# killerwhile/kafka-assignment-optimizer

Hardware: AMD Instinct MI355X
Metric: candidate assignments/sec (+ time_to_optimal_s), 10k-partition reassign (higher is better)
Workload: dtype int32

## Files before the change

include/kao.h:

```cpp
#ifndef KAO_H
#define KAO_H

#include <stdint.h>

#ifdef __cplusplus
extern "C" {
#endif

#define KAO_VERSION 103
#define KAO_NONE 0xFFFFu
#define KAO_MAX_RF 8
#define KAO_MAX_RACKS 255

enum {
    KAO_OK = 0,
    KAO_ERR_INVALID = -1,
    KAO_ERR_UNSUPPORTED = -2,
    KAO_ERR_NO_DEVICE = -3,
    KAO_ERR_HIP = -4,
    KAO_ERR_NOMEM = -5,
    KAO_ERR_NOT_INIT = -6
};

enum {
    KAO_STATUS_OPTIMAL_PROVEN = 0,
    KAO_STATUS_FEASIBLE_BOUND_GAP = 1,
    KAO_STATUS_NO_FEASIBLE = 2,
    KAO_STATUS_TIME_LIMIT = 3,
    KAO_STATUS_INFEASIBLE_PROVEN = 4
};

typedef struct kao_topic {
    int32_t n_brokers;
    int32_t n_racks;
    int32_t n_partitions;
    int32_t rf;
    int32_t rf_cur;
    const uint8_t *rack_of;
    const uint16_t *current;
    int32_t w[2][2];
    int32_t rep_lo, rep_hi;
    int32_t lead_lo, lead_hi;
    int32_t rack_lo, rack_hi;
    int32_t prack_lo, prack_hi;
    const int32_t *broker_w;
    const int32_t *broker_wl;
} kao_topic;

typedef struct kao_opts {
    uint64_t seed;
    double time_limit_s;
    int32_t restarts;
    int32_t iters_per_launch;
    int32_t max_launches;
    int32_t obj_scale;
    int32_t lam_min, lam_max;
    int32_t period_log2;
    int32_t stop_at_bound;
    int32_t profile;
    int32_t dual_iters;
    int32_t elite_period;
    int32_t use_prices;
    int32_t use_cycles;
    int32_t islands;
    int32_t schedule;
    int32_t team;
    const int64_t *target_objective;
} kao_opts;

typedef struct kao_result {
    int32_t status;
    int32_t best_restart;
    int64_t objective;
    int64_t upper_bound;
    int32_t violations[8];
    double seconds_to_best;
    uint16_t *assignment;
} kao_result;

typedef struct kao_stats {
    uint64_t launches;
    uint64_t delta_candidates;
    uint64_t full_candidates;
    double ms_search;
    double ms_eval;
    uint64_t search_bytes_algo;
    uint64_t eval_bytes_algo;
    int32_t n_restarts_total;
    int32_t lds_bytes_search;
    int32_t blocks_search;
    int32_t drift;
    int32_t launch_groups;
    int32_t search_rf3_launches;
} kao_stats;

typedef struct kao_session kao_session;
typedef struct kao_eval_plan kao_eval_plan;

int kao_init(int device);
void kao_shutdown(void);
int kao_version(void);
const char *kao_strerror(int code);
const char *kao_last_error(void);
int kao_device_name(char *buf, int len);

int kao_derive_bounds(const kao_topic *t, int32_t out[8]);
int kao_upper_bound(const kao_topic *t, int64_t *ub);
int kao_check_infeasible(const kao_topic *t, char *why, int why_len);
int kao_canonicalize(const kao_topic *t, uint16_t *assignment);

int kao_evaluate(const kao_topic *t, const uint16_t *assignment, int64_t *objective, int32_t violations[8]);
int kao_evaluate_batch(const kao_topic *t, const uint16_t *candidates, int64_t n, int32_t *objective,
                       int32_t *violations);
int kao_eval_plan_create(const kao_topic *t, kao_eval_plan **out);
int kao_eval_plan_run(kao_eval_plan *p, const void *d_candidates, int64_t n, void *d_objective ,
                      void *d_violations , void *d_best_key );
int kao_eval_plan_sync(kao_eval_plan *p, double *ms_last );
void kao_eval_plan_destroy(kao_eval_plan *p);

int kao_session_create(const kao_topic *topics, int32_t n_topics, const kao_opts *opts, kao_session **out);
int kao_session_step(kao_session *s);
int kao_session_sync(kao_session *s);
int kao_session_new_generation(kao_session *s);
int kao_session_best(kao_session *s, kao_result *results);
int kao_session_best_keys(kao_session *s, uint64_t *keys);
int kao_session_device_keys(kao_session *s, void **d_keys);
int kao_session_stats(kao_session *s, kao_stats *out);
int kao_session_bound_step(kao_session *s, const int64_t *target, int32_t iters);
int kao_session_set_prices(kao_session *s, int32_t topic, const int32_t *a, const int32_t *l, const int32_t *g);
int kao_session_adopt_prices(kao_session *s);
int kao_session_prices(kao_session *s, int32_t topic, int32_t *a, int32_t *l, int32_t *g);
int kao_session_bound_busy(kao_session *s);
int kao_session_bounds(kao_session *s, int64_t *upper_bound, int32_t *flags, int32_t *iters);
int kao_session_dual_state(kao_session *s, int32_t topic, int32_t *a, int32_t *l, int32_t *g, int64_t *best_dual);
int kao_session_set_dual_state(kao_session *s, int32_t topic, const int32_t *a, const int32_t *l, const int32_t *g);
int kao_lp_bound(const kao_topic *t, double tol, int32_t max_iters, int64_t *bound, int64_t *best_dual, int32_t *multipliers, double stats[8]);
int kao_lp_trace(const kao_topic *t, double tol, int32_t max_iters, double *trace, double stats[8], int32_t *multipliers);
int kao_lp_round(const kao_topic *t, double pert, uint32_t salt, double tol, int32_t max_iters, int32_t use_fallback, uint16_t *assignment,
                 int64_t *objective, int32_t violations[8], double stats[8]);
int kao_lp_round_host(const kao_topic *t, const uint8_t *q, const int32_t *zq, int32_t use_fallback, uint16_t *assignment, int32_t rep[4]);
int kao_dense_spd_test(const double *A, int32_t n, const double *rhs, double *factor, double *linv, double *x, double ms[2]);
int kao_lp_sharded_test(const kao_topic *t, const int32_t *devices, int32_t n_dev, double pert, uint32_t salt, double tol, int32_t max_iters,
                        int64_t *bound, uint16_t *assignment, int64_t *objective, int32_t violations[8], double stats[8]);
int kao_dual_bound(const kao_topic *t, int64_t target, int32_t iters, int32_t launches, int64_t *bound,
                   int64_t *best_dual, int32_t *iters_done, int32_t *flags, int32_t *multipliers);
int kao_session_restart_state(kao_session *s, int32_t topic, int32_t restart, uint16_t *final_state,
                              uint16_t *best_state, int32_t info[4]);
void kao_session_destroy(kao_session *s);

int kao_solve(const kao_topic *topics, int32_t n_topics, const kao_opts *opts, kao_result *results);
int kao_solve_multi(const kao_topic *topics, int32_t n_topics, const int32_t *devices, int32_t n_dev, const kao_opts *opts,
                    kao_result *results);
int kao_solve_capped(const kao_topic *topics, int32_t n_topics, const int32_t *replica_cap, const int32_t *devices, int32_t n_dev,
                     const kao_opts *opts, int32_t max_rounds, kao_result *results, int64_t *lagrangian_bound);
int kao_improve_cycles(const kao_topic *t, uint16_t *assignment, int32_t max_rounds, int64_t *objective, int32_t stats[8]);
int kao_cycle_matrices(const kao_topic *t, const uint16_t *assignment, int32_t layer, int32_t level, int32_t *dist, int32_t *mid,
                       uint32_t *slot);
int kao_cycle_seeds(const kao_topic *t, const uint16_t *assignment, int32_t *table, int32_t *n_cfg);
int kao_cycle_pair_edges(const kao_topic *t, const uint16_t *assignment, int32_t gmin, int32_t *cost, int64_t stats[4]);

int kao_plan_waves(int32_t n_brokers, int32_t n_partitions, int32_t width, const uint16_t *current, const uint16_t *target,
                   int32_t max_per_broker, uint64_t seed, int32_t *wave , int32_t *n_waves, int32_t *lower_bound);

int kao_plan_waves_sized(int32_t n_brokers, int32_t n_partitions, int32_t width, const uint16_t *current, const uint16_t *target,
                         const uint64_t *size , uint64_t max_bytes_per_broker, int32_t max_per_broker,
                         uint64_t seed, int32_t *wave , int32_t *n_waves, int32_t *lower_bound);

int kao_balance_leaders(const kao_topic *t, uint16_t *assignment , int32_t *n_changed,
                        int64_t *objective ,
                        int32_t *status, int32_t stats[8] );

#define KAO_FAILOVER_MAX_BROKERS 8000
int kao_failover_order(int32_t n_brokers, int32_t n_racks, const uint8_t *rack_of ,
                       int32_t n_partitions, int32_t width, uint16_t *rows ,
                       int32_t scope , int32_t dry_run,
                       int32_t *scen , int32_t *n_reordered, int32_t stats[8] );

int kao_rccl_selftest(const int32_t *devices, int32_t n_dev);
int kao_rccl_loopback_counts(uint64_t out[2]);
int kao_last_solve_timing(double out[16]);
int kao_last_solve_lp(double out[8]);
int kao_last_solve_profile(double out[8]);

#ifdef __cplusplus
}
#endif
#endif
```

kafka_assignment_optimizer_amd/_ffi.py:

```python
from __future__ import annotations

import ctypes as C
import os

_HERE = os.path.dirname(os.path.abspath(__file__))
LIB_PATH = os.path.join(_HERE, "libkao.so")


class KaoTopic(C.Structure):
    _fields_ = [("n_brokers", C.c_int32), ("n_racks", C.c_int32), ("n_partitions", C.c_int32),
                ("rf", C.c_int32), ("rf_cur", C.c_int32),
                ("rack_of", C.POINTER(C.c_uint8)), ("current", C.POINTER(C.c_uint16)),
                ("w", (C.c_int32 * 2) * 2),
                ("rep_lo", C.c_int32), ("rep_hi", C.c_int32), ("lead_lo", C.c_int32), ("lead_hi", C.c_int32),
                ("rack_lo", C.c_int32), ("rack_hi", C.c_int32), ("prack_lo", C.c_int32), ("prack_hi", C.c_int32),
                ("broker_w", C.POINTER(C.c_int32)), ("broker_wl", C.POINTER(C.c_int32))]


class KaoOpts(C.Structure):
    _fields_ = [("seed", C.c_uint64), ("time_limit_s", C.c_double), ("restarts", C.c_int32),
                ("iters_per_launch", C.c_int32), ("max_launches", C.c_int32), ("obj_scale", C.c_int32),
                ("lam_min", C.c_int32), ("lam_max", C.c_int32), ("period_log2", C.c_int32),
                ("stop_at_bound", C.c_int32), ("profile", C.c_int32), ("dual_iters", C.c_int32),
                ("elite_period", C.c_int32), ("use_prices", C.c_int32), ("use_cycles", C.c_int32), ("islands", C.c_int32),
                ("schedule", C.c_int32), ("team", C.c_int32),
                ("target_objective", C.POINTER(C.c_int64))]


class KaoResult(C.Structure):
    _fields_ = [("status", C.c_int32), ("best_restart", C.c_int32), ("objective", C.c_int64),
                ("upper_bound", C.c_int64), ("violations", C.c_int32 * 8), ("seconds_to_best", C.c_double),
                ("assignment", C.POINTER(C.c_uint16))]


class KaoStats(C.Structure):
    _fields_ = [("launches", C.c_uint64), ("delta_candidates", C.c_uint64), ("full_candidates", C.c_uint64),
                ("ms_search", C.c_double), ("ms_eval", C.c_double), ("search_bytes_algo", C.c_uint64),
                ("eval_bytes_algo", C.c_uint64), ("n_restarts_total", C.c_int32), ("lds_bytes_search", C.c_int32),
                ("blocks_search", C.c_int32), ("drift", C.c_int32), ("launch_groups", C.c_int32),
                ("search_rf3_launches", C.c_int32)]


_P = C.POINTER
SIGNATURES = {
    "kao_init": (C.c_int, [C.c_int]),
    "kao_shutdown": (None, []),
    "kao_version": (C.c_int, []),
    "kao_strerror": (C.c_char_p, [C.c_int]),
    "kao_last_error": (C.c_char_p, []),
    "kao_device_name": (C.c_int, [C.c_char_p, C.c_int]),
    "kao_derive_bounds": (C.c_int, [_P(KaoTopic), _P(C.c_int32)]),
    "kao_upper_bound": (C.c_int, [_P(KaoTopic), _P(C.c_int64)]),
    "kao_canonicalize": (C.c_int, [_P(KaoTopic), _P(C.c_uint16)]),
    "kao_check_infeasible": (C.c_int, [_P(KaoTopic), C.c_char_p, C.c_int]),
    "kao_evaluate": (C.c_int, [_P(KaoTopic), _P(C.c_uint16), _P(C.c_int64), _P(C.c_int32)]),
    "kao_evaluate_batch": (C.c_int, [_P(KaoTopic), _P(C.c_uint16), C.c_int64, _P(C.c_int32), _P(C.c_int32)]),
    "kao_eval_plan_create": (C.c_int, [_P(KaoTopic), _P(C.c_void_p)]),
    "kao_eval_plan_run": (C.c_int, [C.c_void_p, C.c_void_p, C.c_int64, C.c_void_p, C.c_void_p, C.c_void_p]),
    "kao_eval_plan_sync": (C.c_int, [C.c_void_p, _P(C.c_double)]),
    "kao_eval_plan_destroy": (None, [C.c_void_p]),
    "kao_session_create": (C.c_int, [_P(KaoTopic), C.c_int32, _P(KaoOpts), _P(C.c_void_p)]),
    "kao_session_step": (C.c_int, [C.c_void_p]),
    "kao_session_sync": (C.c_int, [C.c_void_p]),
    "kao_session_new_generation": (C.c_int, [C.c_void_p]),
    "kao_session_best": (C.c_int, [C.c_void_p, _P(KaoResult)]),
    "kao_session_best_keys": (C.c_int, [C.c_void_p, _P(C.c_uint64)]),
    "kao_session_device_keys": (C.c_int, [C.c_void_p, _P(C.c_void_p)]),
    "kao_session_stats": (C.c_int, [C.c_void_p, _P(KaoStats)]),
    "kao_session_restart_state": (C.c_int, [C.c_void_p, C.c_int32, C.c_int32, _P(C.c_uint16), _P(C.c_uint16),
                                            _P(C.c_int32)]),
    "kao_session_bound_step": (C.c_int, [C.c_void_p, _P(C.c_int64), C.c_int32]),
    "kao_session_set_prices": (C.c_int, [C.c_void_p, C.c_int32, _P(C.c_int32), _P(C.c_int32), _P(C.c_int32)]),
    "kao_session_adopt_prices": (C.c_int, [C.c_void_p]),
    "kao_session_prices": (C.c_int, [C.c_void_p, C.c_int32, _P(C.c_int32), _P(C.c_int32), _P(C.c_int32)]),
    "kao_session_bound_busy": (C.c_int, [C.c_void_p]),
    "kao_session_bounds": (C.c_int, [C.c_void_p, _P(C.c_int64), _P(C.c_int32), _P(C.c_int32)]),
    "kao_session_dual_state": (C.c_int, [C.c_void_p, C.c_int32, _P(C.c_int32), _P(C.c_int32), _P(C.c_int32), _P(C.c_int64)]),
    "kao_session_set_dual_state": (C.c_int, [C.c_void_p, C.c_int32, _P(C.c_int32), _P(C.c_int32), _P(C.c_int32)]),
    "kao_lp_bound": (C.c_int, [_P(KaoTopic), C.c_double, C.c_int32, _P(C.c_int64), _P(C.c_int64), _P(C.c_int32), _P(C.c_double)]),
    "kao_lp_round": (C.c_int, [_P(KaoTopic), C.c_double, C.c_uint32, C.c_double, C.c_int32, C.c_int32, _P(C.c_uint16), _P(C.c_int64), _P(C.c_int32), _P(C.c_double)]),
    "kao_lp_round_host": (C.c_int, [_P(KaoTopic), _P(C.c_uint8), _P(C.c_int32), C.c_int32, _P(C.c_uint16), _P(C.c_int32)]),
    "kao_dense_spd_test": (C.c_int, [_P(C.c_double), C.c_int32, _P(C.c_double), _P(C.c_double), _P(C.c_double), _P(C.c_double), _P(C.c_double)]),
    "kao_lp_sharded_test": (C.c_int, [_P(KaoTopic), _P(C.c_int32), C.c_int32, C.c_double, C.c_uint32, C.c_double, C.c_int32, _P(C.c_int64), _P(C.c_uint16),
                                      _P(C.c_int64), _P(C.c_int32), _P(C.c_double)]),
    "kao_lp_trace": (C.c_int, [_P(KaoTopic), C.c_double, C.c_int32, _P(C.c_double), _P(C.c_double), _P(C.c_int32)]),
    "kao_dual_bound": (C.c_int, [_P(KaoTopic), C.c_int64, C.c_int32, C.c_int32, _P(C.c_int64), _P(C.c_int64), _P(C.c_int32),
                                 _P(C.c_int32), _P(C.c_int32)]),
    "kao_session_destroy": (None, [C.c_void_p]),
    "kao_solve": (C.c_int, [_P(KaoTopic), C.c_int32, _P(KaoOpts), _P(KaoResult)]),
    "kao_solve_multi": (C.c_int, [_P(KaoTopic), C.c_int32, _P(C.c_int32), C.c_int32, _P(KaoOpts), _P(KaoResult)]),
    "kao_solve_capped": (C.c_int, [_P(KaoTopic), C.c_int32, _P(C.c_int32), _P(C.c_int32), C.c_int32, _P(KaoOpts), C.c_int32,
                                  _P(KaoResult), _P(C.c_int64)]),
    "kao_rccl_selftest": (C.c_int, [_P(C.c_int32), C.c_int32]),
    "kao_rccl_loopback_counts": (C.c_int, [_P(C.c_uint64)]),
    "kao_improve_cycles": (C.c_int, [_P(KaoTopic), _P(C.c_uint16), C.c_int32, _P(C.c_int64), _P(C.c_int32)]),
    "kao_cycle_matrices": (C.c_int, [_P(KaoTopic), _P(C.c_uint16), C.c_int32, C.c_int32, _P(C.c_int32), _P(C.c_int32), _P(C.c_uint32)]),
    "kao_cycle_seeds": (C.c_int, [_P(KaoTopic), _P(C.c_uint16), _P(C.c_int32), _P(C.c_int32)]),
    "kao_cycle_pair_edges": (C.c_int, [_P(KaoTopic), _P(C.c_uint16), C.c_int32, _P(C.c_int32), _P(C.c_int64)]),
    "kao_plan_waves": (C.c_int, [C.c_int32, C.c_int32, C.c_int32, _P(C.c_uint16), _P(C.c_uint16), C.c_int32, C.c_uint64,
                                 _P(C.c_int32), _P(C.c_int32), _P(C.c_int32)]),
    "kao_plan_waves_sized": (C.c_int, [C.c_int32, C.c_int32, C.c_int32, _P(C.c_uint16), _P(C.c_uint16), _P(C.c_uint64), C.c_uint64,
                                       C.c_int32, C.c_uint64, _P(C.c_int32), _P(C.c_int32), _P(C.c_int32)]),
    "kao_balance_leaders": (C.c_int, [_P(KaoTopic), _P(C.c_uint16), _P(C.c_int32), _P(C.c_int64), _P(C.c_int32), _P(C.c_int32)]),
    "kao_failover_order": (C.c_int, [C.c_int32, C.c_int32, _P(C.c_uint8), C.c_int32, C.c_int32, _P(C.c_uint16), C.c_int32, C.c_int32,
                                     _P(C.c_int32), _P(C.c_int32), _P(C.c_int32)]),
    "kao_last_solve_timing": (C.c_int, [_P(C.c_double)]),
    "kao_last_solve_profile": (C.c_int, [_P(C.c_double)]),
    "kao_last_solve_lp": (C.c_int, [_P(C.c_double)]),
}

_lib = None


def load():
    global _lib
    if _lib is None:
        if not os.path.exists(LIB_PATH):
            raise OSError(f"{LIB_PATH} not built: the HIP library is required (no CPU fallback); "
                          "run `make -C kafka_assignment_optimizer_amd/csrc`")
        lib = C.CDLL(LIB_PATH)
        for name, (res, args) in SIGNATURES.items():
            fn = getattr(lib, name)
            fn.restype = res
            fn.argtypes = args
        _lib = lib
    return _lib
```

kafka_assignment_optimizer_amd/csrc/kao_host.h:

```cpp
#pragma once
#include <hip/hip_runtime.h>

#include <algorithm>
#include <cstdint>
#include <cstdlib>
#include <memory>
#include <string>
#include <vector>

#include "../../include/kao.h"
#include "kao_internal.h"

namespace kao {

int fail(int code, const std::string &msg);
#define HIP_TRY(expr)                                                                          \
    do {                                                                                       \
        hipError_t e_ = (expr);                                                                \
        if (e_ != hipSuccess)                                                                  \
            return ::kao::fail(KAO_ERR_HIP, std::string(#expr) + ": " + hipGetErrorString(e_)); \
    } while (0)
double now_s();
int cur_device();
constexpr int kMaxDevices = 64;
int num_cu(int device);
int require_init();
bool is_init();
extern thread_local int t_device;
struct DeviceScope {
    const int saved = t_device;
    int rc = KAO_OK;
    DeviceScope() = default;
    explicit DeviceScope(int device) { to(device); }
    DeviceScope(const DeviceScope &) = delete;
    DeviceScope &operator=(const DeviceScope &) = delete;
    int to(int device);
    ~DeviceScope();
};
struct SolveTiming {
    double session_ready, time_to_best, results_read_back, returned, launches, delta_candidates, bound_launches, elite_exchanges,
           bound_iters, cx_calls, cx_gains, search_iters, generations, cx_further_starts, lp_solves, lp_iters;
};
struct SolveLp { double solves, iterations, rounded, adopted, fractional_partitions; };
struct SolveProfile {
    double ms_search, ms_eval, search_launches, restarts, search_bytes_algo, delta_candidates, lds_bytes_search, blocks_search;
};
struct SolveCounters { SolveTiming timing; SolveLp lp; SolveProfile profile; };
extern thread_local SolveCounters g_last;
inline const char *env_str(const char *name) { const char *e = std::getenv(name); return e && *e ? e : nullptr; }
inline int64_t env_int(const char *name, int64_t dflt) { const char *e = env_str(name); return e ? (int64_t)std::atoll(e) : dflt; }
inline double env_real(const char *name, double dflt) { const char *e = env_str(name); return e ? std::atof(e) : dflt; }
int arena_get(size_t bytes, void **out, size_t *cap);
void arena_put(void *p, size_t bytes, int device);
int stream_get(hipStream_t *out);
void stream_put(hipStream_t st, int device);
void arena_drop_all();
inline size_t align_up(size_t x, size_t a = 256) { return (x + a - 1) / a * a; }
inline uint32_t replica_word(uint16_t x, int m) { return x == KAO_NONE ? kNoneW : ((uint32_t)x | ((uint32_t)(x / m) << 16)); }

int validate(const kao_topic *t);
void derive_bounds(const kao_topic *t, int32_t o[8]);
struct PreparedTopic {
    TopicDev d{};
    std::vector<uint16_t> int_of;
    std::vector<uint16_t> ext_of;
    std::vector<int32_t> rack_size;
    std::vector<uint16_t> cur_int;
    std::vector<uint8_t> rack_of;
    std::vector<uint16_t> cur_dense;
    std::vector<uint32_t> bw_int, bw_dense;
};
int prepare(const kao_topic *t, uint64_t seed, PreparedTopic &pt);
std::string infeasible_reason(const kao_topic *t);
int64_t upper_bound(const kao_topic *t);
int64_t upper_bound_w(const kao_topic *t);
uint64_t neighbours_in_range(uint32_t it0, uint32_t iters, int rf, int n_brokers, int n_partitions, int scan2_max = kScanTwoSlots);
int auto_period_log2(int P, int RF);
bool dual_supported(const kao_topic *t, bool session_bw = false);

}

using namespace kao;

struct kao_eval_plan {
    PreparedTopic pt;
    TopicDev *d_topic = nullptr;
    uint8_t *d_rackof = nullptr;
    uint16_t *d_curd = nullptr;
    int4 *d_map = nullptr;
    uint32_t *d_bwd = nullptr;
    int32_t *d_overflow = nullptr;
    int64_t map_n = -1;
    int map_blocks = 0;
    hipStream_t stream = nullptr;
    hipEvent_t ev0 = nullptr, ev1 = nullptr;
    bool timed = false;
    int cands_per_block = 32;
    bool cur_in_lds = true;
    bool coop = false;
    int device = 0;
};

struct kao_session {
    int device = 0;
    int n_topics = 0;
    kao_opts opts{};
    std::vector<PreparedTopic> pts;
    std::vector<kao_topic> topics;
    std::vector<int64_t> ub;
    std::vector<char> topic_global;
    std::vector<char> topic_curg;
    std::vector<char> topic_infeasible;
    std::vector<char> dual_ok;
    std::vector<int64_t> h_dual_target;
    std::vector<int32_t> h_dual_ids;
    bool multi_off = false;
    std::vector<int2> h_wide_map;
    uint64_t wide_ctl_i32 = 0, wide_map_i32 = 0;
    std::vector<int32_t> dual_flags, dual_iters;
    int total_restarts = 0;
    struct LaunchGroup {
        int maxP = 0, maxBx = 0, maxB = 0, maxR = 0;
        bool wide = false;
        int waves = kWaves;
        int nw = kRFP;
        int rf_uniform = -1;
        bool rf3 = true;
        bool global_a = false;
        bool cur_global = false;
        int team = 0;
        bool cur_in_lds = true;
        bool eval_coop = false;
        int smap_off = 0, smap_n = 0, emap_off = 0, emap_n = 0;
    };
    std::vector<LaunchGroup> groups;
    int blocks_search = 0, blocks_eval = 0;
    void *arena_ro = nullptr, *arena_rw = nullptr;
    size_t arena_ro_bytes = 0, arena_rw_bytes = 0;
    TopicDev *d_topics = nullptr;
    int2 *d_smap = nullptr;
    int4 *d_emap = nullptr;
    uint32_t *d_cur = nullptr;
    uint16_t *d_ext = nullptr;
    int32_t *d_rsz = nullptr;
    uint8_t *d_rackof = nullptr;
    uint16_t *d_curd = nullptr;
    unsigned char *d_state = nullptr;
    uint16_t *d_best = nullptr;
    int32_t *d_info = nullptr;
    int32_t *d_obj = nullptr;
    int32_t *d_viol = nullptr;
    unsigned char *d_readback = nullptr;
    size_t readback_bytes = 0, rb_viol_off = 0, rb_assign_off = 0;
    int32_t *d_dual = nullptr;
    int32_t *d_price = nullptr;
    size_t price_half_i32 = 0;
    int price_read = 0;
    int price_write_last = -1;
    bool priced = false;
    bool any_bw = false;
    uint16_t *d_int = nullptr;
    uint32_t *d_bw = nullptr, *d_bwd = nullptr;
    long long *d_dual_target = nullptr;
    int32_t *d_dual_ids = nullptr;
    unsigned char *d_dual_rb = nullptr;
    size_t dual_rb_bytes = 0;
    uint64_t bound_launches = 0;
    bool dual_state_init = false;
    size_t dual_bytes = 0;
    hipStream_t stream_bound = nullptr;
    hipEvent_t ev_bound0 = nullptr, ev_bound1 = nullptr, ev_search = nullptr;
    bool bound_inflight = false;
    bool bound_no_wait = false;
    int bound_iters_last = 0;
    double bound_ms_last = 0;
    unsigned long long *d_keys = nullptr;
    unsigned long long *d_keys_glob = nullptr;
    int32_t *d_drift = nullptr;
    int32_t *d_win_viol = nullptr;
    uint16_t *d_win_assign = nullptr;
    std::vector<unsigned char> h_readback;
    hipStream_t stream = nullptr;
    uint32_t launch = 0;
    uint32_t gen = 0;
    bool reinit = false;
    size_t best_bytes = 0;
    std::vector<hipEvent_t> ev;
    int ev_pending = 0;
    double ms_search = 0, ms_eval = 0;
    uint64_t eval_bytes_per_launch = 0;
    uint64_t delta_total = 0, search_bytes_total = 0;
    uint64_t search_rf3_launches = 0;
};

namespace kao {
constexpr int64_t kDualNone = 0x7F7F7F7F7F7F7F7Fll;
inline int64_t dual_floor(int64_t best_dual) { return best_dual >= 0 ? best_dual / kDualScale : -((-best_dual + kDualScale - 1) / kDualScale); }
inline int64_t dual_bound_value(int32_t flags, int32_t iters, int64_t best_dual) { return (flags & 4) || iters == 0 ? INT64_MAX : dual_floor(best_dual); }
struct SessionDeleter { void operator()(kao_session *s) const { kao_session_destroy(s); } };
using SessionPtr = std::unique_ptr<kao_session, SessionDeleter>;
int bound_only_session(const kao_topic *t, SessionPtr &out);
int session_topic_best(kao_session *s, int i, uint16_t *out);
int session_restart_objs(kao_session *s, int i, std::vector<int32_t> &objs);
int session_restart_best(kao_session *s, int i, int restart, uint16_t *out);
int session_adopt_external(kao_session *s, int i, const uint16_t *assign, int64_t objective, uint64_t *key_out);
}
```

kafka_assignment_optimizer_amd/csrc/kao_internal.h:

```cpp
#pragma once
#include <stdint.h>

#include <unordered_map>

#include "../../include/kao.h"

namespace kao {

constexpr int kRFP = 4;
constexpr int kMaxRF = 8;
constexpr int kWaves = 4;
constexpr int kTeamMax = 8;
constexpr int kMaxRacks = 255;
constexpr int kLdsLimit = 160 * 1024;
constexpr int kRackTab = 256;
constexpr uint32_t kNoneW = 0xFFFFFFFFu;
constexpr uint32_t kKeyNull = 0xFFFFFFFFu;
constexpr int kDBias = 32768;
constexpr int kDualLog2 = 16;
constexpr int kDualScale = 1 << kDualLog2;
constexpr int kDualStage = 100;
constexpr int kDualDeflP = 2048;
constexpr int kScanTwoSlots = 24576;
constexpr int kDualClamp = 1 << 26;
constexpr int kDualQuarterLog2 = kDualLog2 - 2;
constexpr int kDualProbes = 2;
constexpr uint32_t kExternalRestart = 0xFFFFFu;
constexpr uint32_t kObjCap = 0xFFFFFFu;

struct TopicDev {
    int32_t P, RF, R, m, Bx;
    uint32_t magic;
    int32_t rep_lo, rep_hi, lead_lo, lead_hi, rack_lo, rack_hi, prack_lo, prack_hi;
    int32_t w00, w01, w10, w11;
    uint32_t seed_lo, seed_hi;
    int32_t n_restarts;
    int32_t restart_base;
    uint32_t cur_off;
    uint32_t ext_off;
    uint32_t rsz_off;
    uint64_t state_off;
    uint64_t best_off;
    int32_t B, rf_cur;
    uint32_t rackof_off;
    uint32_t curd_off;
    uint32_t win_off;
    uint32_t dual_off;
    int32_t period_log2;
    uint32_t price_off;
    uint32_t int_off;
    int32_t nw;
    int32_t has_bw;
    uint32_t bw_off;
    uint32_t bwd_off;
    uint32_t cnt_off;
    uint32_t hole_off;
    int32_t pad_[1];
};

struct SearchParams {
    int32_t obj_scale, lam_min, lam_max;
    int32_t maxR;
    int32_t wide;
    uint32_t launch;
    uint32_t iters;
    int32_t init;
    int32_t maxP, maxBx;
    int32_t bw;
    uint32_t gen;
    int32_t scan2_max;
    int32_t cur_global;
    int32_t elite;
};

struct SearchPools {
    const TopicDev *topics;
    const int2 *block_map;
    const uint32_t *cur_pool;
    const uint16_t *ext_pool;
    const int32_t *rsz_pool;
    unsigned char *state_pool;
    uint16_t *best_pool;
    int32_t *restart_info;
    int32_t *drift;
    const int32_t *price_pool;
    const uint32_t *bw_pool;
    const uint16_t *int_pool;
    const uint16_t *elite_assign;
    const unsigned long long *elite_key;
};

struct EvalPools {
    const TopicDev *topics;
    const int4 *block_map;
    const uint8_t *rackof_pool;
    const uint16_t *curd_pool;
    const uint16_t *cand;
    int32_t *objective;
    int32_t *violations;
    unsigned long long *best_key;
    int32_t maxP, maxB;
    int32_t cur_in_lds;
    int32_t coop;
    const uint32_t *bwd_pool;
    int32_t *overflow;
    int32_t rf_uniform;
};

struct BoundPools {
    const TopicDev *topics;
    const int32_t *ids;
    const uint8_t *rackof_pool;
    const uint16_t *curd_pool;
    const uint16_t *ext_pool;
    const int32_t *rsz_pool;
    int32_t *dual_pool;
    const long long *target;
    long long *best_L;
    int32_t *info;
    int32_t iters;
    int32_t maxB, maxP, maxR;
    int32_t cur_in_lds;
    int32_t *price_pool;
    int32_t export_prices;
    int32_t ne;
    const uint32_t *bwd_pool;
};

struct BoundWide {
    const int2 *map;
    int32_t *cnt_pool;
    long long *ctl;
    int32_t chunk;
};

constexpr int search_rack_tab(int maxR) { return ((maxR < 1 ? 1 : maxR) + 1 + 63) & ~63; }
size_t search_lds_bytes(int maxP, int maxBx, int waves, bool global_a, bool priced = false, int nw = 4, bool bw = false, int maxR = kRackTab - 1, int team = 0, bool cur_global = false);
size_t eval_lds_bytes(int maxP, int maxB, bool cur_in_lds, int ne = 4);
bool search_rf3_eligible(bool global_a, bool cur_global, bool priced, int nw, int team);
void launch_search(const SearchPools &pools, const SearchParams &prm, int n_blocks, int waves, bool global_a, bool priced, int nw, void *stream, int team = 0, int rft = 0);
bool launch_init(const SearchPools &pools, const SearchParams &prm, int n_blocks, int per_block, bool priced, int nw, int waves, void *stream);
void launch_eval(const EvalPools &pools, int n_blocks, int ne, void *stream);
void launch_gather(const TopicDev *topics, int n_topics, const unsigned long long *keys, const uint16_t *best_pool,
                   const int32_t *viol, uint16_t *win_assign, int32_t *win_viol, void *stream);

void launch_adopt_global(unsigned long long *keys, const unsigned long long *glob, int n, void *stream);

size_t bound_lds_bytes(int maxB, int maxP, int maxR, bool cur_in_lds, int ne = 4, bool hbw = false, bool dirs = false);
void launch_bound_center(const BoundPools &pools, int n_topics, void *stream);
void launch_bound(const BoundPools &pools, int n_blocks, int waves, void *stream);
void launch_bound_wide(const BoundPools &pools, const BoundWide &wide, int n_topics, int n_blocks, int waves, void *stream);
bool launch_bound_multi(const BoundPools &pools, const BoundWide &wide, int n_topics, int n_blocks, int waves, void *stream);

size_t canon_lds_bytes(int maxBx);
void launch_canon(const TopicDev *topic, const uint32_t *cur_words, const uint16_t *ext, const int32_t *rsz, uint32_t *A, int maxBx,
                  int nw, int32_t *status, void *stream);


struct LpCtx;
struct LpColl {
    virtual int allreduce(int rank, double *buf, size_t n, bool is_min, void *stream) = 0;
    virtual ~LpColl() {}
};
struct LpShard { int p0, p1, rank; LpColl *coll; };
struct LpFan {
    virtual int begin(double tol, int maxit, double pert, uint32_t salt) = 0;
    virtual int enqueue_mark(int k, int slot) = 0;
    virtual int poll_mark(int slot, int *status, int *iterations, double deadline) = 0;
    virtual int finish(int32_t *multipliers, double stats[8], double *trace) = 0;
    virtual int primal(uint8_t *q, int32_t *zq) = 0;
    virtual void abort() = 0;
    virtual void close() = 0;
    virtual ~LpFan() {}
};
extern thread_local bool t_lp_inner;
void lp_set_fan(LpCtx *c, LpFan *fan);
int lp_open_fan(const kao_topic *t, const int *devices, int n_dev, LpCtx **out);
int lp_open(const kao_topic *t, LpCtx **out, const LpShard *shard = nullptr);
int lp_solve(LpCtx *c, double tol, int maxit, int32_t *multipliers, double stats[8], double *trace, double pert = 0.0, uint32_t salt = 0);
int lp_begin(LpCtx *c, double tol, int maxit, double pert = 0.0, uint32_t salt = 0);
int lp_enqueue(LpCtx *c, int k);
int lp_poll(LpCtx *c, int *status, int *iterations);
int lp_enqueue_mark(LpCtx *c, int k, int slot);
int lp_poll_mark(LpCtx *c, int slot, int *status, int *iterations, double deadline = 0);
int lp_finish(LpCtx *c, int32_t *multipliers, double stats[8], double *trace);
inline double lp_default_pert(const kao_topic *t) { const double e = 100.0 / ((double)t->n_partitions * t->rf); return e < 1e-2 ? e : 1e-2; }
int lp_primal(LpCtx *c, uint8_t *q, int32_t *zq);
int lp_round_assignment(const kao_topic *t, const uint8_t *q, const int32_t *zq, const uint16_t *fallback, uint16_t *out, int32_t rep[4], int max_free = 1 << 30);
void lp_abort(LpCtx *c);
void lp_close(LpCtx *c);
void chol_enqueue(void *stream, const double *stop, double *S, int n, const double *diag0, double *Linv);
void trsv_enqueue(void *stream, double *stop, const double *gate, const double *S, int n, double *r, const double *Linv, double *xz);

bool cycle_supported(const kao_topic *t);
int cycle_improve(const kao_topic *t, uint16_t *assign, int32_t max_rounds, double deadline, int64_t *objective, int32_t stats[8]);
struct CycleCtx;
CycleCtx *cycle_open(const kao_topic *t, int *rc_out);
int cycle_run(CycleCtx *c, uint16_t *assign, int32_t max_rounds, double deadline, int64_t *objective, int32_t stats[8],
              int (*poll)(void *) = nullptr, void *poll_arg = nullptr, bool pairs = true);
void cycle_close(CycleCtx *c);
struct PairEdge { int32_t cost; int32_t set; int32_t p, q; uint16_t rowp[8], rowq[8]; };
int pair_edges(const kao_topic *t, const uint16_t *assignment, int gmin, std::unordered_map<uint32_t, PairEdge> &edges, int64_t stats[4]);
int api_fail(int code, const char *msg);
int api_require_init();
double api_now_s();

}
```

kafka_assignment_optimizer_amd/csrc/kao_search.hip:

```cpp
#include "kao_search_dev.h"

namespace kao {

template <bool kGlobalA, bool kPriced, int NW, bool kWide, bool kTeam, bool kCurG = false, int RFT = 0>
__device__ __forceinline__ void search_body(unsigned char *smem, const SearchPools &pl, const SearchParams &prm) {
    static_assert(!kTeam || kGlobalA, "teams run topics that live in global memory");
    static_assert(!kCurG || !kGlobalA, "kCurG: the working assignment is in LDS");
    static_assert(RFT == 0 || (RFT == 3 && NW == 4 && !kGlobalA && !kTeam), "RFT = 3: LDS-resident topics of four words per partition");
    constexpr int NS = RFT ? RFT : NW;
    const int lane = threadIdx.x & 63;
    const int wave = __builtin_amdgcn_readfirstlane(threadIdx.x >> 6);
    const int n_waves = kTeam ? __builtin_amdgcn_readfirstlane((int)(blockDim.x >> 6)) : 1;
    const int tid = kTeam ? (int)threadIdx.x : lane, nthr = kTeam ? (int)blockDim.x : 64;
    const int2 bm = pl.block_map[blockIdx.x];
    const TopicDev *TD = pl.topics + bm.x;

    TopicRegs T = topic_regs<RFT>(TD);
    asm volatile("" : "+v"(T.rep_lo), "+v"(T.rep_hi), "+v"(T.lead_lo), "+v"(T.lead_hi));

    const int a_bytes = kGlobalA ? 0 : prm.maxP * NW * 4;
    const int cur_bytes = (kGlobalA || kCurG) ? 0 : prm.maxP * NW * 4;
    const int bx64 = (prm.maxBx + 63) & ~63;
    const int c_bytes = bx64 * 4;
    const int krt = search_rack_tab(prm.maxR);
    int *RSZ = reinterpret_cast<int *>(smem + cur_bytes);
    uint8_t *XR = smem + cur_bytes + krt * 4;
    const uint32_t inv = (uint32_t)krt - 1u;
    uint32_t *PR = reinterpret_cast<uint32_t *>(smem + cur_bytes + krt * 4 + bx64);
    const bool hbw = kPriced && prm.bw != 0;
    const int pr_bytes = kPriced ? (hbw ? 2 : 1) * c_bytes + krt * 4 : 0;
    int *PG = reinterpret_cast<int *>(smem + cur_bytes + krt * 4 + bx64 + c_bytes);
    uint32_t *BW = reinterpret_cast<uint32_t *>(smem + cur_bytes + krt * 4 + bx64 + c_bytes + krt * 4);
    unsigned char *wb = smem + cur_bytes + krt * 4 + bx64 + pr_bytes + (kTeam ? 0 : wave * (a_bytes + c_bytes + c_bytes / 2 + krt * 8));
    const Part<NW> *cur_words = reinterpret_cast<const Part<NW> *>(pl.cur_pool + TD->cur_off);
    const Part<NW> *CUR;
    if (kGlobalA || kCurG) CUR = cur_words; else CUR = reinterpret_cast<const Part<NW> *>(smem);
    WaveLds<NW> L;
    L.C = reinterpret_cast<uint32_t *>(wb + a_bytes);
    L.W = reinterpret_cast<uint16_t *>(wb + a_bytes + c_bytes);
    L.K = reinterpret_cast<int *>(wb + a_bytes + c_bytes + c_bytes / 2);
    L.RT = L.K + krt + (kTeam ? wave * krt : 0);
    int *TR = L.K + krt + n_waves * krt;
    int *TS = TR + 2 * 16 * kTeamRec;

    if (!kGlobalA && !kCurG) {
        Part<NW> *cur_lds = reinterpret_cast<Part<NW> *>(smem);
        for (int p = threadIdx.x; p < T.P; p += blockDim.x) cur_lds[p] = cur_words[p];
    }
    for (int r = threadIdx.x; r < krt; r += blockDim.x) {
        RSZ[r] = r < T.R ? pl.rsz_pool[TD->rsz_off + r] : 0;
        if (kPriced) PG[r] = r < T.R ? price_units(pl.price_pool[TD->price_off + 2 * TD->B + r], prm.obj_scale) : 0;
    }
    __syncthreads();
    for (int x = threadIdx.x; x < ((T.Bx + 63) & ~63); x += blockDim.x) {
        const uint32_t r = mulhi((uint32_t)x, T.magic);
        const bool valid = x < T.Bx && (int)((uint32_t)x - r * (uint32_t)T.m) < RSZ[r < (uint32_t)krt ? r : 0];
        XR[x] = valid ? (uint8_t)r : (uint8_t)inv;
        if (kPriced) {
            uint32_t pr = 0;
            if (valid) {
                const int32_t *pp = pl.price_pool + TD->price_off;
                const int b = pl.ext_pool[TD->ext_off + x];
                pr = ((uint32_t)price_units(pp[b], prm.obj_scale) & 0xFFFFu) | ((uint32_t)price_units(pp[TD->B + b], prm.obj_scale) << 16);
            }
            PR[x] = pr;
            if (hbw) BW[x] = (valid && TD->has_bw) ? pl.bw_pool[TD->bw_off + x] : 0u;
        }
    }
    __syncthreads();

    const int rho = bm.y + (kTeam ? 0 : wave);
    if (rho >= TD->n_restarts) return;
    const int g = TD->restart_base + rho;
    unsigned char *state_packed = pl.state_pool + TD->state_off + (uint64_t)rho * T.P * (NW * 2);
    if (kGlobalA) L.A = reinterpret_cast<Part<NW> *>(pl.state_pool + TD->state_off) + (uint64_t)rho * T.P;
    else L.A = reinterpret_cast<Part<NW> *>(wb);
    uint16_t *best = pl.best_pool + TD->best_off + (uint64_t)rho * T.P * T.RF;
    const uint16_t *ext = pl.ext_pool + TD->ext_off;
    const uint32_t slo = TD->seed_lo, shi = TD->seed_hi;
    const int S = prm.obj_scale;

    int best_obj, accepted;
    if (prm.init) {
        if (prm.init == 1)
        for (int p = tid; p < T.P; p += nthr) {
            Part<NW> c = CUR[p];
#pragma unroll
            for (int k = 1; k < NW; ++k)
                if (k >= T.RF) c.w[k] = kNoneW;
            L.A[p] = c;
        }
        best_obj = -1; accepted = 0;
    } else {
        best_obj = pl.restart_info[g * 4 + 0];
        accepted = pl.restart_info[g * 4 + 3];
        bool reseed = false;
        if (prm.elite) {
            const unsigned long long ek = pl.elite_key[bm.x];
            const int e_obj = (int)kObjCap - (int)((ek >> 20) & 0xFFFFFFull);
            reseed = ek != ~0ull && (ek >> 44) == 0 && (int)(ek & 0xFFFFFull) != rho && best_obj < e_obj &&
                     (fmix32(slo ^ ((uint32_t)rho * 0x9E3779B1u) ^ (prm.launch * 0x85EBCA77u) ^ 0xE117Eu) & 1u);
        }
        if (reseed) {
            const uint16_t *ea = pl.elite_assign + TD->win_off;
            const uint16_t *io = pl.int_pool + TD->int_off;
            for (int p = tid; p < T.P; p += nthr) {
                Part<NW> w;
#pragma unroll
                for (int k = 0; k < NW; ++k) w.w[k] = k < T.RF ? to_word(T, io[ea[p * T.RF + k]]) : kNoneW;
                L.A[p] = w;
            }
        } else if (!kGlobalA) {
            for (int p = lane; p < T.P; p += 64) L.A[p] = load_packed<NW>(T, state_packed, p);
        }
    }
    if (kGlobalA) __builtin_amdgcn_fence(__ATOMIC_SEQ_CST, "workgroup");
    if (kTeam) __syncthreads();
    recount(T, L, tid, nthr, krt);
    if (kTeam) __syncthreads();

    if (prm.init == 1) {
        const uint32_t *HL = pl.cur_pool + TD->hole_off;
        if (!kTeam || wave == 0)
        for (int pass = 0; pass < 2; ++pass) {
            const uint32_t n_holes = HL[pass], *hl = HL + 2 + (pass ? HL[0] : 0u);
            int p_n = n_holes ? (int)hl[0] : 0;
            Part<NW> a_n = L.A[p_n], c_n = CUR[p_n];
            for (uint32_t hi = 0; hi < n_holes; ++hi) {
                const int p = p_n;
                Part<NW> a = a_n;
                const Part<NW> c = c_n;
                if (hi + 1 < n_holes) { p_n = (int)hl[hi + 1]; a_n = L.A[p_n]; c_n = CUR[p_n]; }
#pragma unroll
                for (int k = 0; k < NW; ++k) {
                    if (k >= T.RF) break;
                    if ((k == 0) != (pass == 0)) continue;
                    if (a.w[k] != kNoneW) continue;
                    const uint32_t hmix = slo ^ fmix32(shi + (uint32_t)rho * 0x9E3779B1u + (uint32_t)(p * NW + k) * 0x27D4EB2Fu + 0x5BD1E995u + prm.gen * 0x632BE5ABu);
                    const int wl = k == 0 ? T.w00 : T.w01, wf = k == 0 ? T.w10 : T.w11;
                    uint32_t key = kKeyNull, xw_l = kNoneW;
#pragma unroll 2
                    for (int base = 0; base < T.Bx; base += 64) {
                        const uint32_t x = (uint32_t)(base + lane);
                        const uint32_t r = XR[x];
                        const uint32_t xw = x | (r << 16);
                        const bool okx = (r != inv) & !in4(a, xw);
                        const uint32_t cn = L.C[x];
                        const uint32_t rk = r;
                        int dV = dinc((int)(cn & 0xFFFFu), T.rep_lo, T.rep_hi) + dinc(L.K[rk], T.rack_lo, T.rack_hi) +
                                 dinc(cnt4(a, r), T.prack_lo, T.prack_hi);
                        if (k == 0) dV += dinc((int)(cn >> 16), T.lead_lo, T.lead_hi);
                        const uint32_t tie = fmix32(hmix + x * 0x165667B1u) >> 24;
                        uint32_t keyx;
                        if (kPriced) {
                            const uint32_t prx = PR[x];
                            int dP = p_in((int)(cn & 0xFFFFu), T.rep_lo, T.rep_hi, price_rep(prx)) + p_in(L.K[rk], T.rack_lo, T.rack_hi, PG[rk]);
                            if (k == 0) dP += p_in((int)(cn >> 16), T.lead_lo, T.lead_hi, price_lead(prx));
                            keyx = okx ? make_key_tie_p(prm.lam_max, S, dV, role_w2(c, xw, wl, wf) + (hbw ? bw_of(BW[x], k == 0) : 0), dP, tie) : kKeyNull;
                        }
                        else keyx = okx ? make_key_tie(prm.lam_max, S, dV, role_w2(c, xw, wl, wf), tie) : kKeyNull;
                        if (keyx < key) { key = keyx; xw_l = xw; }
                    }
                    const uint32_t kmin = wave_umin(key);
                    const unsigned long long bal = __ballot(key == kmin);
                    const uint32_t xw_win = (uint32_t)__builtin_amdgcn_readlane((int)xw_l, __ffsll((long long)bal) - 1);
                    a.w[k] = xw_win;
                    if (lane == 0) {
                        reinterpret_cast<uint32_t *>(&L.A[p])[k] = xw_win;
                        L.C[xw_win & 0xFFFFu] += (k == 0) ? 0x10001u : 1u;
                        L.K[xw_win >> 16] += 1;
                    }
                }
            }
        }
        if (kGlobalA) __builtin_amdgcn_fence(__ATOMIC_SEQ_CST, "workgroup");
        if (kTeam) __syncthreads();
    }

    int V, obj;
    full_cost<NW, kTeam>(T, L, CUR, RSZ, tid, nthr, V, obj, hbw ? BW : nullptr, TS, wave, n_waves);
    if (V == 0 && obj > best_obj) { best_obj = obj; snapshot(T, L, ext, best, tid, nthr); }
    rebuild_band_state(T, L, XR, inv, tid, nthr);
    if (lane == 0) L.RT[krt - 1] = 0;
    if (kTeam) __syncthreads();

    uint32_t rng = fmix32(slo ^ fmix32(shi + (uint32_t)rho * 0x9E3779B1u + prm.launch * 0x85EBCA77u + (uint32_t)tid * 0xC2B2AE3Du));

    const int plog = TD->period_log2 + (rho & 3);
    const uint32_t pmask = (1u << plog) - 1u;
    const uint32_t lrange = (uint32_t)(prm.lam_max - prm.lam_min + 1);
    const uint32_t RF8 = (uint32_t)T.RF << 8, R8 = (uint32_t)T.R << 8, m8 = (uint32_t)T.m << 8;

    const int T_tour = min(64, max(4, (T.P * T.RF) >> 2));
    uint32_t tour_off = lane < T_tour ? 0u : kKeyNull;
    asm volatile("" : "+v"(tour_off));
    const int GA = min(16, max(1, (T.P * T.RF) >> 8));
    const int x_rounds_full = (T.P + 63) >> 6;
    const bool x_windowed = x_rounds_full > 8;

    int lam_lo = prm.lam_min, lam_hi = prm.lam_max;
    uint32_t n_iters = prm.iters, it_base = prm.launch * prm.iters;
    uint32_t scan_two = TD->P * TD->RF <= prm.scan2_max ? 1u : 0u;
    {
        uint32_t v0 = (uint32_t)lam_lo, v1 = (uint32_t)lam_hi, v2 = n_iters, v3 = it_base, v4 = scan_two;
        asm volatile("" : "+v"(v0), "+v"(v1), "+v"(v2), "+v"(v3), "+v"(v4));
        lam_lo = (int)__builtin_amdgcn_readfirstlane(v0); lam_hi = (int)__builtin_amdgcn_readfirstlane(v1);
        n_iters = __builtin_amdgcn_readfirstlane(v2); it_base = __builtin_amdgcn_readfirstlane(v3);
        scan_two = __builtin_amdgcn_readfirstlane(v4);
    }
    constexpr bool kFuse = !kGlobalA && !kTeam && !kPriced;
    const bool fuse_ok = kFuse && T.Bx <= 16384;
    uint32_t jmp_a = 1u, jmp_c = 0u;
    if (fuse_ok)
        for (int n = (T.Bx + 63) >> 6; n > 0; --n) { jmp_a = (jmp_a * 0x6D2B79u) & 0xFFFFFFu; jmp_c = (jmp_c * 0x6D2B79u + 0x3C6EF3u) & 0xFFFFFFu; }
    for (uint32_t i = 0; i < n_iters; ++i) {
        const uint32_t it = it_base + i;
        const int type = (int)((0x1210u >> ((it & 7u) * 2u)) & 3u);
        const uint32_t ph = it & pmask;
        const int lam = best_obj < 0 ? lam_hi : min(lam_hi, lam_lo + (int)((2u * ph * lrange) >> plog));
        const bool sampled = (type == 2) || (type == 0 && ((it >> 3) & 1u));

        auto finish = [&](auto ty, auto uni, uint32_t kmin, int win, int p, int k, int q, int j, uint32_t uw, uint32_t vw, int dV, int dObj) {
            constexpr int TY = decltype(ty)::value;
            auto of_win = [&](int v) { return decltype(uni)::value ? v : __builtin_amdgcn_readlane(v, win); };
            if (!kTeam) {
                if (kmin == kKeyNull) return;
                if ((int)(kmin >> 8) - kDBias > 0) return;
            }
            bool mine = true;
            int *rec = TR + ((i & 1u) * 16 + (uint32_t)wave) * kTeamRec;
            if (kTeam) {
                const bool ok = kmin != kKeyNull && (int)(kmin >> 8) - kDBias <= 0;
                if (lane == win) {
                    const uint32_t ro_ = uw >> 16, rn_ = vw >> 16;
                    const bool racks = ok && TY == 0 && ro_ != rn_;
                    rec[0] = ok ? 1 : 0; rec[1] = p; rec[2] = TY == 1 ? q : p;
                    rec[3] = (int)(uw & 0xFFFFu); rec[4] = (int)(vw & 0xFFFFu);
                    rec[5] = racks ? (int)ro_ : 0xFFFF; rec[6] = racks ? (int)rn_ : 0xFFFF;
                    rec[7] = dV; rec[8] = dObj;
                }
                __syncthreads();
                bool clash = false;
                if (lane < wave) {
                    const int *o = TR + ((i & 1u) * 16 + (uint32_t)lane) * kTeamRec;
                    if (o[0]) {
                        const int mp = rec[1], mq = rec[2], mb0 = rec[3], mb1 = rec[4], mr0 = rec[5], mr1 = rec[6];
                        clash = (o[1] == mp) | (o[1] == mq) | (o[2] == mp) | (o[2] == mq) | (o[3] == mb0) | (o[3] == mb1) | (o[4] == mb0) | (o[4] == mb1);
                        if (o[5] != 0xFFFF && mr0 != 0xFFFF) clash |= (o[5] == mr0) | (o[5] == mr1) | (o[6] == mr0) | (o[6] == mr1);
                    }
                }
                mine = ok && __ballot(clash) == 0ull;
            }

            if (lane == win && mine) {
                uint32_t *ap = reinterpret_cast<uint32_t *>(&L.A[p]);
                if (TY == 0) {
                    const uint32_t d = (k == 0) ? 0x10001u : 1u;
                    L.C[uw & 0xFFFFu] -= d;
                    L.C[vw & 0xFFFFu] += d;
                    if (!kTeam || (uw >> 16) != (vw >> 16)) {
                        L.K[uw >> 16] -= 1;
                        L.K[vw >> 16] += 1;
                    }
                    ap[k] = vw;
                } else if (TY == 1) {
                    uint32_t *bp = reinterpret_cast<uint32_t *>(&L.A[q]);
                    if ((k == 0) != (j == 0)) {
                        const uint32_t lose = (k == 0) ? uw : vw, gain = (k == 0) ? vw : uw;
                        L.C[lose & 0xFFFFu] -= 0x10000u;
                        L.C[gain & 0xFFFFu] += 0x10000u;
                    }
                    ap[k] = vw;
                    bp[j] = uw;
                } else {
                    L.C[uw & 0xFFFFu] -= 0x10000u;
                    L.C[vw & 0xFFFFu] += 0x10000u;
                    ap[0] = vw;
                    ap[k] = uw;
                }
            }
            if (mine) {
                int rows;
                if (TY == 0) rows = 1 | (of_win(k) == 0 ? 2 : 0);
                else if (TY == 1) rows = (of_win(k) == 0 ? 2 : 0) ^ (of_win(j) == 0 ? 2 : 0);
                else rows = 2;
                if (rows != 0) {
                    const uint32_t xo = (uint32_t)of_win((int)uw) & 0xFFFFu, xn = decltype(uni)::value ? (uint32_t)__builtin_amdgcn_readfirstlane((int)(vw & 0xFFFFu)) : (uint32_t)of_win((int)vw) & 0xFFFFu;
                    uint32_t xx = xo;
                    asm("v_writelane_b32 %0, %1, 1" : "+v"(xx) : "s"(xn));
                    int lane_w = lane;
                    asm volatile("" : "+v"(lane_w));
                    if (lane_w < 2) {
                        const uint32_t cx = L.C[xx];
                        uint32_t wx;
                        if (rows == 3) wx = band_fields(T, cx);
                        else if (rows == 1) wx = (L.W[xx] & ~kWRowR) | band_entry((int)(cx & 0xFFFFu), T.rep_lo, T.rep_hi);
                        else wx = (L.W[xx] & ~kWRowL) | (band_entry((int)(cx >> 16), T.lead_lo, T.lead_hi) << 6);
                        L.W[xx] = (uint16_t)wx;
                    }
                }
            }
            if (kGlobalA) __builtin_amdgcn_fence(__ATOMIC_SEQ_CST, "workgroup");
            if (kTeam) {
                if (lane == 0) rec[9] = mine ? 1 : 0;
                __syncthreads();
                int dVs = 0, dOs = 0, na = 0;
                if (lane < n_waves) {
                    const int *o = TR + ((i & 1u) * 16 + (uint32_t)lane) * kTeamRec;
                    if (o[9]) { dVs = o[7]; dOs = o[8]; na = 1; }
                }
                V += wave_sum(dVs);
                obj += wave_sum(dOs);
                accepted += wave_sum(na);
            } else {
                V += of_win(dV);
                obj += of_win(dObj);
                accepted++;
            }
        };
        constexpr std::integral_constant<int, 0> kReplace{};
        constexpr std::integral_constant<int, 1> kExchange{};
        constexpr std::integral_constant<int, 2> kLeaderSwap{};

        if (sampled) {
            const int p = (int)rnd24_wide(rng, (uint32_t)T.P);
            const Part<NW> a = L.A[p];
            const Part<NW> c = CUR[p];
            uint32_t key = kKeyNull, vw = 0;
            int dV = 0, dObj = 0;
            if (type == 0) {
                const int k = (int)rnd24(rng, RF8);
                const uint32_t uw = sel_slot<NS>(a, k);
                const uint32_t ro = uw >> 16;
                const bool lead = k == 0;
                const uint32_t lw = lead ? 2u : 0u;
                const int wl = lead ? T.w00 : T.w01, wf = lead ? T.w10 : T.w11;
                const int g_old = role_w2<NS>(c, uw, wl, wf) + (hbw ? bw_of(BW[uw & 0xFFFFu], lead) : 0);
                const uint32_t wo = L.W[uw & 0xFFFFu];
                const int dV_old = wfld(wo, kWDecR) + wfldw(wo, kWDecL, lw);
                const int dV_rack_old = ddec(L.K[ro], T.rack_lo, T.rack_hi) + ddec(cnt4<NS>(a, ro), T.prack_lo, T.prack_hi);
                const int rsz_ro = RSZ[ro];
                int dP_old = 0, dP_rack_old = 0;
                if (kPriced) {
                    const uint32_t pro = PR[uw & 0xFFFFu];
                    dP_old = -(wflag(wo, kWPoutR) & price_rep(pro));
                    if (lead) dP_old -= wflag(wo, kWPoutL) & price_lead(pro);
                    dP_rack_old = p_out(L.K[ro], T.rack_lo, T.rack_hi, PG[ro]);
                }
#pragma unroll
                for (int g = 0; g < 4; ++g) {
                    uint32_t r, jj;
                    bool okg;
                    if (g < 2) {
                        r = rnd24(rng, R8);
                        jj = rnd24(rng, m8);
                        okg = (int)jj < RSZ[r];
                    } else {
                        r = ro;
                        jj = rnd24(rng, (uint32_t)rsz_ro << 8);
                        okg = true;
                    }
                    const uint32_t x = __umul24(r, (uint32_t)T.m) + jj;
                    const uint32_t xw = x | (r << 16);
                    okg = okg && !in4<NS>(a, xw);
                    const uint32_t wn = L.W[x];
                    int dVg = dV_old + wfld(wn, kWIncR) + wfldw(wn, kWIncL, lw);
                    if (g < 2) {
                        if (r != ro)
                            dVg += dV_rack_old + dinc(L.K[r], T.rack_lo, T.rack_hi) + dinc(cnt4<NS>(a, r), T.prack_lo, T.prack_hi);
                    }
                    const int dObjg = role_w2<NS>(c, xw, wl, wf) + (hbw ? bw_of(BW[x], lead) : 0) - g_old;
                    uint32_t keyg;
                    if (kPriced) {
                        const uint32_t prx = PR[x];
                        int dPg = dP_old + (wflag(wn, kWPinR) & price_rep(prx));
                        if (lead) dPg += wflag(wn, kWPinL) & price_lead(prx);
                        if (g < 2 && r != ro) dPg += dP_rack_old + p_in(L.K[r], T.rack_lo, T.rack_hi, PG[r]);
                        keyg = okg ? make_key_p(lam, S, dVg, dObjg, dPg, lane) : kKeyNull;
                    }
                    else keyg = okg ? make_key(lam, S, dVg, dObjg, lane) : kKeyNull;
                    if (keyg < key) { key = keyg; vw = xw; dV = dVg; dObj = dObjg; }
                }
                const uint32_t kmin = wave_umin(key);
                finish(kReplace, std::false_type{}, kmin, (int)(kmin & 63u), p, k, 0, 0, uw, vw, dV, dObj);
            } else {
                const uint32_t uw = a.w[0];
                int k = 0;
                const int u_lead = role_w2<NS>(c, uw, T.w00, T.w10), u_fol = role_w2<NS>(c, uw, T.w01, T.w11);
                const uint32_t wu = L.W[uw & 0xFFFFu];
                const int dV_u = wfld(wu, kWDecL);
                const int dP_u = kPriced ? -(wflag(wu, kWPoutL) & price_lead(PR[uw & 0xFFFFu])) : 0;
#pragma unroll
                for (int kk = 1; kk < NS; ++kk) {
                    if (!RFT && kk >= T.RF) break;
                    const uint32_t xw = a.w[kk];
                    const int dObjg = role_w2<NS>(c, xw, T.w00, T.w10) + u_fol - u_lead - role_w2<NS>(c, xw, T.w01, T.w11) +
                                      (hbw ? (int)(BW[xw & 0xFFFFu] >> 16) - (int)(BW[uw & 0xFFFFu] >> 16) : 0);
                    const uint32_t wx = L.W[xw & 0xFFFFu];
                    const int dVg = dV_u + wfld(wx, kWIncL);
                    uint32_t keyg;
                    if (kPriced) keyg = make_key_p(lam, S, dVg, dObjg, dP_u + (wflag(wx, kWPinL) & price_lead(PR[xw & 0xFFFFu])), lane);
                    else keyg = make_key(lam, S, dVg, dObjg, lane);
                    if (keyg < key) { key = keyg; vw = xw; k = kk; dV = dVg; dObj = dObjg; }
                }
                const uint32_t kmin = wave_umin(key);
                finish(kLeaderSwap, std::false_type{}, kmin, (int)(kmin & 63u), p, k, 0, 0, uw, vw, dV, dObj);
            }
        } else {
            uint32_t keyA, oldw_l;
            int pl_, kl_, g_old_l, dvo_l = 0, dvr_l = 0;
            auto score_words = [&](auto ty, uint32_t &key_o, const Part<NW> &al, const Part<NW> &cl, int k_o, uint32_t &oldw_o, int &g_o, int &dvo_o, int &dvr_o) {
                constexpr int TY = decltype(ty)::value;
                oldw_o = sel_slot<NS>(al, k_o);
                const uint32_t rol = oldw_o >> 16;
                const bool leadl = k_o == 0;
                g_o = role_w2<NS>(cl, oldw_o, leadl ? T.w00 : T.w01, leadl ? T.w10 : T.w11);
                if (hbw && TY == 0) g_o += bw_of(BW[oldw_o & 0xFFFFu], leadl);
                const uint32_t wo = L.W[oldw_o & 0xFFFFu];
                const int dv7 = ddec(cnt4<NS>(al, rol), T.prack_lo, T.prack_hi);
                int sc;
                if (TY == 0) {
                    dvo_o = wfld(wo, kWDecR) + wfldw(wo, kWDecL, leadl ? 2u : 0u);
                    dvr_o = ddec(L.K[rol], T.rack_lo, T.rack_hi) + dv7;
                    sc = dvo_o + min(dvr_o, 0);
                } else {
                    const int dvl = wfld(wo, leadl ? kWDecL : kWIncL);
                    sc = min(dv7, 0) + min(dvl, 0);
                }
                if (kPriced) {
                    int dPs = 0;
                    if (TY == 0) {
                        const uint32_t pro = PR[oldw_o & 0xFFFFu];
                        dPs = -(wflag(wo, kWPoutR) & price_rep(pro));
                        dPs -= wflagw(wo, kWPoutL, leadl ? 1u : 0u) & price_lead(pro);
                    }
                    key_o = make_key_p(lam, S, sc, -g_o, dPs, lane) | tour_off;
                }
                else key_o = make_key(lam, S, sc, -g_o, lane) | tour_off;
            };
            auto score_slot = [&](auto ty, uint32_t &key_o, int p_o, int &k_o, uint32_t &oldw_o, int &g_o, int &dvo_o, int &dvr_o) {
                k_o = (int)rnd24(rng, RF8);
                const Part<NW> al = L.A[p_o];
                const Part<NW> cl = CUR[p_o];
                score_words(ty, key_o, al, cl, k_o, oldw_o, g_o, dvo_o, dvr_o);
            };
            auto tournament = [&](auto ty) {
                const int p0 = (int)rnd24_wide(rng, (uint32_t)T.P);
                auto part = [&](int ga) { const int q2 = p0 + ga; return q2 < T.P ? q2 : q2 - T.P; };
                pl_ = p0;
                score_slot(ty, keyA, p0, kl_, oldw_l, g_old_l, dvo_l, dvr_l);
                int ga = 1;
                for (; kWide && ga + 1 < GA; ga += 2) {
                    uint32_t kg0, ow0, kg1, ow1;
                    int kk0, gg0, d10 = 0, d20 = 0, kk1, gg1, d11 = 0, d21 = 0;
                    const int pg0 = part(ga), pg1 = part(ga + 1);
                    score_slot(ty, kg0, pg0, kk0, ow0, gg0, d10, d20);
                    score_slot(ty, kg1, pg1, kk1, ow1, gg1, d11, d21);
                    if (kg0 < keyA) { keyA = kg0; pl_ = pg0; kl_ = kk0; oldw_l = ow0; g_old_l = gg0; dvo_l = d10; dvr_l = d20; }
                    if (kg1 < keyA) { keyA = kg1; pl_ = pg1; kl_ = kk1; oldw_l = ow1; g_old_l = gg1; dvo_l = d11; dvr_l = d21; }
                }
                for (; ga < GA; ++ga) {
                    uint32_t kg, ow;
                    int kk, gg, d1 = 0, d2 = 0;
                    const int pg = part(ga);
                    score_slot(ty, kg, pg, kk, ow, gg, d1, d2);
                    if (kg < keyA) { keyA = kg; pl_ = pg; kl_ = kk; oldw_l = ow; g_old_l = gg; dvo_l = d1; dvr_l = d2; }
                }
            };
            Part<NW> a_l, c_l;
            constexpr int XB = !kGlobalA ? 1 : ((NW == 4 && !kTeam) ? 8 : 4);
            Part<NW> xb[XB], xcb[XB];
            int q0 = 0;
            auto x_partner = [&](int rd, int &qq, bool &okq) {
                qq = q0 + rd * 64 + lane; okq = true;
                if (qq >= T.P) { if (x_windowed) qq -= T.P; else okq = false; }
                return min(qq, T.P - 1);
            };
            auto tournament_global = [&](auto ty) {
                constexpr int TY = decltype(ty)::value;
                constexpr int TB = (NW == 4 && !kTeam) ? 16 : 8;
                const int p0 = (int)rnd24_wide(rng, (uint32_t)T.P);
                auto part = [&](int ga) { const int q2 = p0 + ga; return q2 < T.P ? q2 : q2 - T.P; };
                int kk[16];
#pragma unroll
                for (int g = 0; g < 16; ++g) { kk[g] = 0; if (g < GA) kk[g] = (int)rnd24(rng, RF8); }
                if (TY == 1) {
                    const int q_draw = (int)rnd24_wide(rng, (uint32_t)T.P);
                    q0 = x_windowed ? __builtin_amdgcn_readfirstlane(q_draw) : 0;
#pragma unroll
                    for (int r2 = 0; r2 < XB; ++r2) { int qq; bool okq; const int qc = x_partner(r2, qq, okq); xb[r2] = L.A[qc]; xcb[r2] = CUR[qc]; }
                }
#pragma unroll
                for (int g0 = 0; g0 < 16; g0 += TB) {
                    if (g0 > 0 && g0 >= GA) break;
                    Part<NW> tal[TB], tcl[TB];
                    int tp[TB];
#pragma unroll
                    for (int g = 0; g < TB; ++g) { tp[g] = (g0 + g) < GA ? part(g0 + g) : p0; tal[g] = L.A[tp[g]]; tcl[g] = CUR[tp[g]]; }
#pragma unroll
                    for (int g = 0; g < TB; ++g) {
                        uint32_t kg, ow;
                        int gg, d1 = 0, d2 = 0;
                        score_words(ty, kg, tal[g], tcl[g], kk[g0 + g], ow, gg, d1, d2);
                        if (g0 + g > 0) kg |= (g0 + g) < GA ? 0u : kKeyNull;
                        if (g0 + g == 0 || kg < keyA) { keyA = kg; pl_ = tp[g]; kl_ = kk[g0 + g]; oldw_l = ow; g_old_l = gg; dvo_l = d1; dvr_l = d2; a_l = tal[g]; c_l = tcl[g]; }
                    }
                }
            };
            if constexpr (kGlobalA) { if (type == 0) tournament_global(std::integral_constant<int, 0>{}); else tournament_global(std::integral_constant<int, 1>{}); }
            else if (type == 0) tournament(std::integral_constant<int, 0>{}); else tournament(std::integral_constant<int, 1>{});
            const int wA1 = (int)(wave_umin(keyA) & 63u);
            int wA2 = -1;
            if (type == 0 && scan_two) {
                const uint32_t k2 = wave_umin(lane == wA1 ? kKeyNull : keyA);
                wA2 = k2 == kKeyNull ? -1 : (int)(k2 & 63u);
            }
            if (kFuse && type == 0 && wA2 >= 0 && fuse_ok) {
                int ps[2], ks[2], gs[2], dvos[2];
                uint32_t us[2];
                int v_rk[2];
#pragma unroll
                for (int s2 = 0; s2 < 2; ++s2) {
                    const int wA = s2 == 0 ? wA1 : wA2;
                    ps[s2] = __builtin_amdgcn_readlane(pl_, wA);
                    ks[s2] = __builtin_amdgcn_readlane(kl_, wA);
                    us[s2] = (uint32_t)__builtin_amdgcn_readlane((int)oldw_l, wA);
                    gs[s2] = __builtin_amdgcn_readlane(g_old_l, wA);
                    dvos[s2] = __builtin_amdgcn_readlane(dvo_l, wA);
                    v_rk[s2] = __builtin_amdgcn_readlane(dvr_l, wA);
                }
                const Part<NW> a1 = L.A[ps[0]], c1 = CUR[ps[0]], a2 = L.A[ps[1]], c2 = CUR[ps[1]];
                const uint32_t ro1 = us[0] >> 16, ro2 = us[1] >> 16;
                for (int r = lane; r < T.R; r += 64) {
                    const int dk = dinc(L.K[r], T.rack_lo, T.rack_hi);
                    const int v1 = ((uint32_t)r != ro1) ? v_rk[0] + dk + dinc(cnt4<NS>(a1, (uint32_t)r), T.prack_lo, T.prack_hi) : 0;
                    const int v2 = ((uint32_t)r != ro2) ? v_rk[1] + dk + dinc(cnt4<NS>(a2, (uint32_t)r), T.prack_lo, T.prack_hi) : 0;
                    L.RT[r] = (int)(((uint32_t)v1 & 0xFFFFu) | ((uint32_t)v2 << 16));
                }
                int lane_v = lane;
                asm volatile("" : "+v"(lane_v));
                const int li = lane_v & (NW - 1);
                const bool l2 = lane_v >= NW;
                const int p_l = l2 ? ps[1] : ps[0];
                const uint32_t ai = reinterpret_cast<const uint32_t *>(&L.A[p_l])[li], ci = reinterpret_cast<const uint32_t *>(&CUR[p_l])[li];
                const bool holds = (lane_v < 2 * NW) & (ai != kNoneW);
                uint32_t w_keep = 0;
                if (holds) w_keep = L.W[ai & 0xFFFFu];
                if (holds & !l2) L.W[ai & 0xFFFFu] = (uint16_t)(w_keep | kWNoCand);
                if (holds & l2) L.W[ai & 0xFFFFu] = (uint16_t)(L.W[ai & 0xFFFFu] | kWNoCand2);
                const bool hc = (lane_v < 2 * NW) & (ci != kNoneW);
                uint32_t w_ci = 0;
                if (hc) w_ci = L.W[ci & 0xFFFFu];
                const bool hm_l = hc & ((w_ci & (l2 ? kWNoCand2 : kWNoCand)) == 0u);
                const int mr_l = hm_l ? (int)((ci & 0xFFFFu) >> 6) : -1;
                int mr[2 * NW];
#pragma unroll
                for (int i2 = 0; i2 < 2 * NW; ++i2) mr[i2] = (i2 & (NW - 1)) < NS ? __builtin_amdgcn_readlane(mr_l, i2) : -1;
                const bool lead1 = ks[0] == 0, lead2 = ks[1] == 0;
                const uint32_t lw1 = lead1 ? 2u : 0u, lw2 = lead2 ? 2u : 0u;
                const int wl1 = lead1 ? T.w00 : T.w01, wf1 = lead1 ? T.w10 : T.w11, wl2 = lead2 ? T.w00 : T.w01, wf2 = lead2 ? T.w10 : T.w11;
                const int K01 = __mul24(S, gs[0]) + kDBias + __mul24(lam, dvos[0]);
                const int K02 = __mul24(S, gs[1]) + kDBias + __mul24(lam, dvos[1]);
                uint32_t jc = jmp_c;
                asm volatile("" : "+v"(jc));
                uint32_t best1 = kKeyNull, best2 = kKeyNull;
                auto scan_round2 = [&](auto with_w, int base, int rd, uint32_t &key1, uint32_t &key2) {
                    const uint32_t st1 = lcg24(rng);
                    uint32_t st2;
                    asm("v_mad_u32_u24 %0, %1, %2, %3" : "=v"(st2) : "v"(st1), "s"(jmp_a), "v"(jc));
                    const int w = (int)reinterpret_cast<const short *>(L.W)[base + lane];
                    const int rt = L.RT[XR[base + lane]];
                    const int inc = wfld(w, kWIncR);
                    int d1 = __mul24(lam, inc + wfldw(w, kWIncL, lw1) + wfldw(rt, 0, 16u)) + K01;
                    int d2 = __mul24(lam, inc + wfldw(w, kWIncL, lw2) + (rt >> 16)) + K02;
                    if (decltype(with_w)::value) {
                        const uint32_t x = (uint32_t)(base + lane);
                        const uint32_t xw = x | ((uint32_t)XR[x] << 16);
                        d1 -= __mul24(S, role_w2<NS>(c1, xw, wl1, wf1));
                        d2 -= __mul24(S, role_w2<NS>(c2, xw, wl2, wf2));
                    }
                    d1 = min(max(d1, 0), 2 * kDBias - 2);
                    d2 = min(max(d2, 0), 2 * kDBias - 2) | wflag(w, 14);
                    key1 = ((uint32_t)d1 << 16) | (st1 & 0xFF00u) | (uint32_t)rd | ((uint32_t)w & 0xFFFF0000u);
                    key2 = ((uint32_t)d2 << 16) | (st2 & 0xFF00u) | (uint32_t)rd;
                };
                const int n_rd = (T.Bx + 63) >> 6;
                int rd = 0, base = 0;
                while (rd < n_rd) {
                    int nxt = n_rd;
#pragma unroll
                    for (int i2 = 0; i2 < 2 * NW; ++i2)
                        if (mr[i2] >= rd) nxt = min(nxt, mr[i2]);
                    uint32_t k1a, k2a, k1b, k2b;
                    for (; rd + 1 < nxt; rd += 2, base += 128) {
                        scan_round2(std::false_type{}, base, rd, k1a, k2a);
                        scan_round2(std::false_type{}, base + 64, rd + 1, k1b, k2b);
                        best1 = min(best1, min(k1a, k1b));
                        best2 = min(best2, min(k2a, k2b));
                    }
                    if (rd < nxt) { scan_round2(std::false_type{}, base, rd, k1a, k2a); best1 = min(best1, k1a); best2 = min(best2, k2a); ++rd; base += 64; }
                    if (rd < n_rd) { scan_round2(std::true_type{}, base, rd, k1a, k2a); best1 = min(best1, k1a); best2 = min(best2, k2a); ++rd; base += 64; }
                }
                asm("v_mad_u32_u24 %0, %0, %1, %2" : "+v"(rng) : "s"(jmp_a), "v"(jc));
                if (holds) L.W[ai & 0xFFFFu] = (uint16_t)w_keep;
                const uint32_t kw = wave_umin(min(((best1 >> 1) & ~127u) | (uint32_t)lane, ((best2 >> 1) & ~127u) | 64u | (uint32_t)lane));
                const bool two = (kw & 64u) != 0u;
                const uint32_t kmin = kw >> 7;
                const int win = (int)(kw & 63u);
                const int p = two ? ps[1] : ps[0], k = two ? ks[1] : ks[0];
                const uint32_t uw = two ? us[1] : us[0];
                if ((int)(kmin >> 8) - kDBias <= 0) {
                    const bool lead = k == 0;
                    const uint32_t bw_ = (uint32_t)__builtin_amdgcn_readlane((int)(two ? best2 : best1), win);
                    const uint32_t xs = ((bw_ & 255u) << 6) + (uint32_t)win;
                    const uint32_t rs = XR[xs];
                    const uint32_t ws = L.W[xs];
                    const int rts = L.RT[rs];
                    const uint32_t vw = xs | (rs << 16);
                    const int dV = wfld(ws, kWIncR) + wfldw(ws, kWIncL, lead ? 2u : 0u) + (two ? dvos[1] : dvos[0]) + (two ? (rts >> 16) : wfldw(rts, 0, 16u));
                    int mx1 = -1, mx2 = -1;
#pragma unroll
                    for (int i2 = 0; i2 < NW; ++i2) { mx1 = max(mx1, mr[i2]); mx2 = max(mx2, mr[NW + i2]); }
                    const bool has_missing = (two ? mx2 : mx1) >= 0;
                    const int dObj = -(two ? gs[1] : gs[0]) + (has_missing ? (two ? role_w2<NS>(c2, vw, wl2, wf2) : role_w2<NS>(c1, vw, wl1, wf1)) : 0);
                    finish(kReplace, std::true_type{}, kmin, win, p, k, 0, 0, uw, vw, dV, dObj);
                }
            } else {
            auto slot_of = [&](int wA, int &p, int &k, uint32_t &uw, int &g_old, int &dV_old, int &dV_rack_old, Part<NW> &a, Part<NW> &c) {
                p = __builtin_amdgcn_readlane(pl_, wA);
                k = __builtin_amdgcn_readlane(kl_, wA);
                uw = (uint32_t)__builtin_amdgcn_readlane((int)oldw_l, wA);
                g_old = __builtin_amdgcn_readlane(g_old_l, wA);
                dV_old = __builtin_amdgcn_readlane(dvo_l, wA);
                dV_rack_old = __builtin_amdgcn_readlane(dvr_l, wA);
                if constexpr (kGlobalA) {
#pragma unroll
                    for (int i2 = 0; i2 < NW; ++i2) { a.w[i2] = (uint32_t)__builtin_amdgcn_readlane((int)a_l.w[i2], wA); c.w[i2] = (uint32_t)__builtin_amdgcn_readlane((int)c_l.w[i2], wA); }
                } else {
                    a = L.A[p];
                    c = CUR[p];
                }
            };
            if (type == 0) {
            uint32_t b_kmin = kKeyNull, b_uw = 0, b_vw = 0;
            int b_win = 0, b_p = 0, b_k = 0, b_dV = 0, b_dObj = 0;
#pragma nounroll
            for (int si = 0; si < (wA2 >= 0 ? 2 : 1); ++si) {
                int p, k, g_old, dV_old, dV_rack_old;
                uint32_t uw;
                Part<NW> a, c;
                slot_of(si == 0 ? wA1 : wA2, p, k, uw, g_old, dV_old, dV_rack_old, a, c);
                const bool lead = k == 0;
                const uint32_t ro = uw >> 16;
                uint32_t vw = 0;
                int dV = 0, dObj = 0;
                {
                    const int dP_rack_old = kPriced ? p_out(L.K[ro], T.rack_lo, T.rack_hi, PG[ro]) : 0;
                    for (int r = lane; r < T.R; r += 64) {
                        int v = ((uint32_t)r != ro) ? dV_rack_old + dinc(L.K[r], T.rack_lo, T.rack_hi) + dinc(cnt4<NS>(a, (uint32_t)r), T.prack_lo, T.prack_hi) : 0;
                        if (kPriced)
                            v = (v & 0xFF) | ((((uint32_t)r != ro) ? dP_rack_old + p_in(L.K[r], T.rack_lo, T.rack_hi, PG[r]) : 0) * 256);
                        L.RT[r] = v;
                    }
                }
                const int wl = lead ? T.w00 : T.w01, wf = lead ? T.w10 : T.w11;
                const int li = lane & (NW - 1);
                const uint32_t ai = sel_slot<NS>(a, li), ci = sel_slot<NS>(c, li);
                const bool holds = (lane < NS) & (ai != kNoneW);
                uint32_t w_keep = 0;
                if (!kTeam && holds) {
                    w_keep = L.W[ai & 0xFFFFu];
                    L.W[ai & 0xFFFFu] = (uint16_t)(w_keep | kWNoCand);
                }
                int ar[NS];
                {
                    const int ar_l = (kTeam && holds) ? (int)((ai & 0xFFFFu) >> 6) : -1;
#pragma unroll
                    for (int i2 = 0; i2 < NS; ++i2) ar[i2] = __builtin_amdgcn_readlane(ar_l, i2);
                }
                const bool hm_l = (lane < NS) & (ci != kNoneW) & !in4<NS>(a, ci);
                const int mr_l = hm_l ? (int)((ci & 0xFFFFu) >> 6) : -1;
                int mr[NS];
#pragma unroll
                for (int i2 = 0; i2 < NS; ++i2) mr[i2] = __builtin_amdgcn_readlane(mr_l, i2);
                bool has_missing = false;
#pragma unroll
                for (int i2 = 0; i2 < NS; ++i2) has_missing |= mr[i2] >= 0;
                int K0 = __mul24(S, g_old) + kDBias + __mul24(lam, dV_old);
                if (kPriced) {
                    const uint32_t pro = PR[uw & 0xFFFFu];
                    const uint32_t wo = L.W[uw & 0xFFFFu];
                    K0 -= wflag(wo, kWPoutR) & price_rep(pro);
                    if (lead) K0 -= wflag(wo, kWPoutL) & price_lead(pro);
                }
                const uint32_t lw = lead ? 2u : 0u, lf = lead ? 1u : 0u;
                uint32_t bestA = kKeyNull;
                int chunkA = 0;
                auto scan_round = [&](auto with_w, int base, int rd) -> uint32_t {
                    const uint32_t st = lcg24(rng);
                    const int w = (int)(short)L.W[base + lane];
                    const int rt = L.RT[XR[base + lane]];
                    int dsc;
                    if (kPriced) {
                        const uint32_t prx = PR[base + lane];
                        const int dVx = wfld(w, kWIncR) + wfldw(w, kWIncL, lw) + (int)(signed char)(rt & 0xFF);
                        dsc = __mul24(lam, dVx) + K0 + (rt >> 8) + (wflag(w, kWPinR) & price_rep(prx)) + (wflagw(w, kWPinL, lf) & price_lead(prx));
                        if (hbw) dsc -= __mul24(S, bw_of(BW[base + lane], lead));
                    } else {
                        const int dVx = wfld(w, kWIncR) + wfldw(w, kWIncL, lw) + rt;
                        dsc = __mul24(lam, dVx) + K0;
                    }
                    uint32_t member = 0;
                    if (decltype(with_w)::value) {
                        const uint32_t x = (uint32_t)(base + lane);
                        const uint32_t xw = x | ((uint32_t)XR[x] << 16);
                        dsc -= __mul24(S, role_w2<NS>(c, xw, wl, wf));
                        if (kTeam && in4<NS>(a, xw)) member = 0xFFFF0000u;
                    }
                    dsc = min(max(dsc, 0), 2 * kDBias - 2);
                    return ((uint32_t)dsc << 16) | (st & 0xFF00u) | (uint32_t)rd | ((uint32_t)w & 0xFFFF0000u) | member;
                };
                auto is_weighted = [&](int rdg) {
                    bool wgt = false;
#pragma unroll
                    for (int i2 = 0; i2 < NS; ++i2) wgt |= (mr[i2] == rdg) | (kTeam && ar[i2] == rdg);
                    return wgt;
                };
                for (int cb = 0; cb < T.Bx; cb += 16384) {
                    uint32_t bestc = kKeyNull;
                    const int cend = min(T.Bx, cb + 16384);
                    int rd = 0, base = cb;
                    if (kWide) {
                        for (; base + 64 < cend; base += 128, rd += 2) {
                            const int rdg = (cb >> 6) + rd;
                            if (is_weighted(rdg) || is_weighted(rdg + 1)) {
                                bestc = min(bestc, is_weighted(rdg) ? scan_round(std::true_type{}, base, rd) : scan_round(std::false_type{}, base, rd));
                                bestc = min(bestc, is_weighted(rdg + 1) ? scan_round(std::true_type{}, base + 64, rd + 1) : scan_round(std::false_type{}, base + 64, rd + 1));
                            } else {
                                const uint32_t k0 = scan_round(std::false_type{}, base, rd);
                                const uint32_t k1 = scan_round(std::false_type{}, base + 64, rd + 1);
                                bestc = min(bestc, min(k0, k1));
                            }
                        }
                    }
                    if (kWide || kTeam) {
                        for (; base < cend; base += 64, ++rd)
                            bestc = min(bestc, is_weighted((cb >> 6) + rd) ? scan_round(std::true_type{}, base, rd) : scan_round(std::false_type{}, base, rd));
                    } else {
                        const int n_rd = (cend - cb + 63) >> 6, rd0 = cb >> 6;
                        while (rd < n_rd) {
                            int nxt = n_rd;
#pragma unroll
                            for (int i2 = 0; i2 < NS; ++i2) {
                                const int m = mr[i2] - rd0;
                                if (m >= rd) nxt = min(nxt, m);
                            }
                            for (; rd + 1 < nxt; rd += 2, base += 128) {
                                const uint32_t k0 = scan_round(std::false_type{}, base, rd);
                                const uint32_t k1 = scan_round(std::false_type{}, base + 64, rd + 1);
                                bestc = min(bestc, min(k0, k1));
                            }
                            if (rd < nxt) { bestc = min(bestc, scan_round(std::false_type{}, base, rd)); ++rd; base += 64; }
                            if (rd < n_rd) { bestc = min(bestc, scan_round(std::true_type{}, base, rd)); ++rd; base += 64; }
                        }
                    }
                    if ((bestc >> 8) < (bestA >> 8)) { bestA = bestc; chunkA = cb; }
                }
                if (!kTeam && holds) L.W[ai & 0xFFFFu] = (uint16_t)w_keep;
                const uint32_t key = bestA >> 8;
                const uint32_t kmin = wave_umin(key);
                const unsigned long long bal = __ballot(key == kmin);
                const int win = __ffsll((long long)bal) - 1;
                if ((int)(kmin >> 8) - kDBias <= 0) {
                    const uint32_t bw_ = (uint32_t)__builtin_amdgcn_readlane((int)bestA, win);
                    const uint32_t xs = (uint32_t)__builtin_amdgcn_readlane(chunkA, win) + ((bw_ & 255u) << 6) + (uint32_t)win;
                    const uint32_t rs = XR[xs];
                    const uint32_t ws = L.W[xs];
                    const int rts = L.RT[rs];
                    vw = xs | (rs << 16);
                    dV = wfld(ws, kWIncR) + wfldw(ws, kWIncL, lw) + dV_old + (kPriced ? (int)(signed char)(rts & 0xFF) : rts);
                    dObj = -g_old + (has_missing ? role_w2<NS>(c, vw, wl, wf) : 0) + (hbw ? bw_of(BW[xs], lead) : 0);
                }
                if (si == 0 || kmin < b_kmin) { b_kmin = kmin; b_win = win; b_p = p; b_k = k; b_uw = uw; b_vw = vw; b_dV = dV; b_dObj = dObj; }
            }
            finish(kReplace, std::true_type{}, b_kmin, b_win, b_p, b_k, 0, 0, b_uw, b_vw, b_dV, b_dObj);
            } else {
                int p, k, g_old, dV_old, dV_rack_old;
                uint32_t uw;
                Part<NW> a, c;
                slot_of(wA1, p, k, uw, g_old, dV_old, dV_rack_old, a, c);
                const bool lead = k == 0;
                const uint32_t ro = uw >> 16;
                uint32_t key = kKeyNull, vw = 0;
                int dV = 0, dObj = 0, q = 0, j = 0;
                const int nrp = lead ? 0 : 1;
                const int cnt_a_ru = cnt4<NS>(a, ro);
                const uint32_t wu = L.W[uw & 0xFFFFu];
                const int pl_u = kPriced ? price_lead(PR[uw & 0xFFFFu]) : 0;
                const int bwl_u = hbw ? (int)(BW[uw & 0xFFFFu] >> 16) : 0;
                if (!kGlobalA) {
                    const int q_draw = (int)rnd24_wide(rng, (uint32_t)T.P);
                    q0 = x_windowed ? __builtin_amdgcn_readfirstlane(q_draw) : 0;
                }
                const int x_rounds = x_windowed ? 8 : x_rounds_full;
                auto x_round = [&](int rd, const Part<NW> &b, const Part<NW> &cb) {
                    const uint32_t tie0 = lcg24(rng) >> 8;
                    int qq; bool okq;
                    x_partner(rd, qq, okq);
                    okq = okq & (qq != p);
                    const bool u_in_b = in4<NS>(b, uw);
                    const int u_in_q_lead = role_w2<NS>(cb, uw, T.w00, T.w10), u_in_q_fol = role_w2<NS>(cb, uw, T.w01, T.w11);
                    const int dv_ro = ddec(cnt_a_ru, T.prack_lo, T.prack_hi) + dinc(cnt4<NS>(b, ro), T.prack_lo, T.prack_hi);
                    int cnt_b_rv[3] = {0, 0, 0};
                    if constexpr (RFT == 3) {
                        const int e01 = (int)((b.w[0] >> 16) == (b.w[1] >> 16)), e02 = (int)((b.w[0] >> 16) == (b.w[2] >> 16)), e12 = (int)((b.w[1] >> 16) == (b.w[2] >> 16));
                        cnt_b_rv[0] = 1 + e01 + e02; cnt_b_rv[1] = 1 + e01 + e12; cnt_b_rv[2] = 1 + e02 + e12;
                    }
#pragma unroll
                    for (int jj = 0; jj < NS; ++jj) {
                        if (!RFT && jj >= T.RF) break;
                        const uint32_t v = b.w[jj];
                        const bool ok = okq & (v != uw) & !in4<NS>(a, v) & !u_in_b;
                        const int nrq = jj != 0;
                        int dObjx = role_w<NS>(T, c, v, nrp) + (jj == 0 ? u_in_q_lead : u_in_q_fol) - g_old - role_w<NS>(T, cb, v, nrq);
                        int dVx = 0, dPx = 0;
                        if (lead != (jj == 0)) {
                            const uint32_t wv = L.W[v & 0xFFFFu];
                            dVx += lead ? (wfld(wu, kWDecL) + wfld(wv, kWIncL)) : (wfld(wv, kWDecL) + wfld(wu, kWIncL));
                            if (kPriced) {
                                if (hbw) { const int dbl = (int)(BW[v & 0xFFFFu] >> 16) - bwl_u; dObjx += lead ? dbl : -dbl; }
                                const int plv = price_lead(PR[v & 0xFFFFu]);
                                dPx = lead ? ((wflag(wv, kWPinL) & plv) - (wflag(wu, kWPoutL) & pl_u))
                                           : ((wflag(wu, kWPinL) & pl_u) - (wflag(wv, kWPoutL) & plv));
                            }
                        }
                        const uint32_t rv = v >> 16;
                        if (rv != ro)
                            dVx += dv_ro + dinc(cnt4<NS>(a, rv), T.prack_lo, T.prack_hi) + ddec(RFT == 3 ? cnt_b_rv[jj < 3 ? jj : 0] : cnt4<NS>(b, rv), T.prack_lo, T.prack_hi);
                        uint32_t keyx;
                        if (kPriced) keyx = ok ? make_key_tie_p(lam, S, dVx, dObjx, dPx, tie0 + (uint32_t)jj * 0x55u) : kKeyNull;
                        else keyx = ok ? make_key_tie(lam, S, dVx, dObjx, tie0 + (uint32_t)jj * 0x55u) : kKeyNull;
                        if (keyx < key) { key = keyx; vw = v; q = qq; j = jj; dV = dVx; dObj = dObjx; }
                    }
                };
                if constexpr (kGlobalA) {
#pragma unroll
                    for (int r2 = 0; r2 < XB; ++r2)
                        if (r2 < x_rounds) x_round(r2, xb[r2], xcb[r2]);
                    for (int rb = XB; rb < x_rounds; rb += XB) {
                        Part<NW> yb[XB], ycb[XB];
#pragma unroll
                        for (int r2 = 0; r2 < XB; ++r2) { int qq; bool okq; const int qc = x_partner(rb + r2, qq, okq); yb[r2] = L.A[qc]; ycb[r2] = CUR[qc]; }
#pragma unroll
                        for (int r2 = 0; r2 < XB; ++r2)
                            if (rb + r2 < x_rounds) x_round(rb + r2, yb[r2], ycb[r2]);
                    }
                } else {
                    for (int rd = 0; rd < x_rounds; ++rd) {
                        int qq; bool okq;
                        const int qc = x_partner(rd, qq, okq);
                        const Part<NW> b = L.A[qc];
                        const Part<NW> cb = CUR[qc];
                        x_round(rd, b, cb);
                    }
                }
                const uint32_t kmin = wave_umin(key);
                const unsigned long long bal = __ballot(key == kmin);
                const int win = __ffsll((long long)bal) - 1;
                finish(kExchange, std::false_type{}, kmin, win, p, k, q, j, uw, vw, dV, dObj);
            }
            }
        }
        if (V == 0 && obj > best_obj) { best_obj = obj; snapshot(T, L, ext, best, tid, nthr); }
    }

    if (kTeam) __syncthreads();
    recount(T, L, tid, nthr, krt);
    if (kTeam) __syncthreads();
    int V2, obj2;
    full_cost<NW, kTeam>(T, L, CUR, RSZ, tid, nthr, V2, obj2, hbw ? BW : nullptr, TS, wave, n_waves);
    if ((V2 != V || obj2 != obj) && tid == 0) atomicAdd(pl.drift, 1);
    if (!kGlobalA)
        for (int p = lane; p < T.P; p += 64) store_packed<NW>(state_packed, p, L.A[p]);
    if (tid == 0) {
        pl.restart_info[g * 4 + 0] = best_obj;
        pl.restart_info[g * 4 + 1] = V2;
        pl.restart_info[g * 4 + 2] = obj2;
        pl.restart_info[g * 4 + 3] = accepted;
    }
}

#ifndef KAO_WPE_SMALL
#define KAO_WPE_SMALL 6
#endif
#ifndef KAO_WPE_WIDE
#define KAO_WPE_WIDE 6
#endif
template <bool kGlobalA, bool kPriced, int NW, bool kWide> constexpr int search_min_waves() { return kGlobalA ? 1 : (kWide ? KAO_WPE_WIDE : KAO_WPE_SMALL); }
template <bool kGlobalA, bool kPriced, int NW, bool kWide, int RFT = 0>
__global__ __launch_bounds__(256) __attribute__((amdgpu_waves_per_eu(search_min_waves<kGlobalA, kPriced, NW, kWide>(), 8))) void k_search(SearchPools pl, SearchParams prm) {
    extern __shared__ __attribute__((aligned(16))) unsigned char smem[];
    search_body<kGlobalA, kPriced, NW, kWide, false, false, RFT>(smem, pl, prm);
}
template <bool kPriced, int NW>
__global__ __launch_bounds__(256) void k_search_curg(SearchPools pl, SearchParams prm) {
    extern __shared__ __attribute__((aligned(16))) unsigned char smem[];
    search_body<false, kPriced, NW, true, false, true>(smem, pl, prm);
}
template <bool kPriced, int NW>
__global__ __launch_bounds__(NW == 8 ? 256 : 512) void k_team(SearchPools pl, SearchParams prm) {
    extern __shared__ __attribute__((aligned(16))) unsigned char smem[];
    search_body<true, kPriced, NW, true, true>(smem, pl, prm);
}

constexpr int kInitWaves = 16;
constexpr size_t init_lds_total(size_t maxBx, int maxR, bool priced, bool bw) {
    const size_t bx64 = (maxBx + 63) & ~(size_t)63, krt = (size_t)search_rack_tab(maxR);
    return krt * 4 + bx64 + (priced ? (bw ? 2 : 1) * bx64 * 4 + krt * 4 : 0) + bx64 * 4 + krt * 4 + (size_t)kInitWaves * krt * 4 + 3 * 8;
}
size_t init_lds_bytes(int maxBx, int maxR, bool priced, bool bw) { return init_lds_total((size_t)maxBx, maxR, priced, bw); }
static_assert(init_lds_total(500, 255, false, false) == 21016 && init_lds_total(500, 255, true, true) == 26136, "init_lds_total no longer sums the LDS carve of k_init");
template <bool kPriced, int NW>
__global__ __launch_bounds__(64 * kInitWaves) void k_init(SearchPools pl, SearchParams prm, int per_block) {
    extern __shared__ __attribute__((aligned(16))) unsigned char smem[];
    const int lane = threadIdx.x & 63;
    const int wave = __builtin_amdgcn_readfirstlane(threadIdx.x >> 6);
    const int n_waves = __builtin_amdgcn_readfirstlane((int)(blockDim.x >> 6));
    const int tid = (int)threadIdx.x, nthr = (int)blockDim.x;
    const int2 bm = pl.block_map[blockIdx.x / (unsigned)per_block];
    const TopicDev *TD = pl.topics + bm.x;
    const int rho = bm.y + (int)(blockIdx.x % (unsigned)per_block);
    if (rho >= TD->n_restarts) return;

    const TopicRegs T = topic_regs(TD);

    const int bx64 = (prm.maxBx + 63) & ~63, krt = search_rack_tab(prm.maxR);
    const bool hbw = kPriced && prm.bw != 0;
    const uint32_t inv = (uint32_t)krt - 1u;
    unsigned char *q = smem;
    int *RSZ = reinterpret_cast<int *>(q); q += krt * 4;
    uint8_t *XR = q; q += bx64;
    uint32_t *PR = reinterpret_cast<uint32_t *>(q); if (kPriced) q += bx64 * 4;
    int *PG = reinterpret_cast<int *>(q); if (kPriced) q += krt * 4;
    uint32_t *BW = reinterpret_cast<uint32_t *>(q); if (hbw) q += bx64 * 4;
    WaveLds<NW> L;
    L.C = reinterpret_cast<uint32_t *>(q); q += bx64 * 4;
    L.K = reinterpret_cast<int *>(q); q += krt * 4;
    L.W = nullptr; L.RT = nullptr;
    int *KW = reinterpret_cast<int *>(q); q += kInitWaves * krt * 4;
    unsigned long long *BEST = reinterpret_cast<unsigned long long *>(q);

    for (int r = tid; r < krt; r += nthr) {
        RSZ[r] = r < T.R ? pl.rsz_pool[TD->rsz_off + r] : 0;
        if (kPriced) PG[r] = r < T.R ? price_units(pl.price_pool[TD->price_off + 2 * TD->B + r], prm.obj_scale) : 0;
    }
    __syncthreads();
    for (int x = tid; x < ((T.Bx + 63) & ~63); x += nthr) {
        const uint32_t r = mulhi((uint32_t)x, T.magic);
        const bool valid = x < T.Bx && (int)((uint32_t)x - r * (uint32_t)T.m) < RSZ[r < (uint32_t)krt ? r : 0];
        XR[x] = valid ? (uint8_t)r : (uint8_t)inv;
        if (kPriced) {
            uint32_t pr = 0;
            if (valid) {
                const int32_t *pp = pl.price_pool + TD->price_off;
                const int b = pl.ext_pool[TD->ext_off + x];
                pr = ((uint32_t)price_units(pp[b], prm.obj_scale) & 0xFFFFu) | ((uint32_t)price_units(pp[TD->B + b], prm.obj_scale) << 16);
            }
            PR[x] = pr;
            if (hbw) BW[x] = (valid && TD->has_bw) ? pl.bw_pool[TD->bw_off + x] : 0u;
        }
    }
    const Part<NW> *CUR = reinterpret_cast<const Part<NW> *>(pl.cur_pool + TD->cur_off);
    L.A = reinterpret_cast<Part<NW> *>(pl.state_pool + TD->state_off) + (uint64_t)rho * T.P;
    const uint32_t slo = TD->seed_lo, shi = TD->seed_hi;
    const int S = prm.obj_scale;
    for (int p = tid; p < T.P; p += nthr) {
        Part<NW> c = CUR[p];
#pragma unroll
        for (int k = 1; k < NW; ++k)
            if (k >= T.RF) c.w[k] = kNoneW;
        L.A[p] = c;
    }
    __builtin_amdgcn_fence(__ATOMIC_SEQ_CST, "workgroup");
    __syncthreads();
    recount(T, L, tid, nthr, krt);
    __syncthreads();
    if (n_waves > 1) {
        for (int r = lane; r < krt; r += 64) KW[wave * krt + r] = L.K[r];
        L.K = KW + wave * krt;
        if (tid < 3) BEST[tid] = ~0ull;
        __syncthreads();
    }

    const uint32_t *HL = pl.cur_pool + TD->hole_off;
    const int n_rounds = (T.Bx + 63) >> 6;
    int par = 0;
    for (int pass = 0; pass < 2; ++pass) {
        const uint32_t n_holes = HL[pass], *hl = HL + 2 + (pass ? HL[0] : 0u);
        for (uint32_t h0 = 0; h0 < n_holes; h0 += 64) {
          const uint32_t nb = min(64u, n_holes - h0);
          const uint32_t p_l = hl[h0 + ((uint32_t)lane < nb ? (uint32_t)lane : 0u)];
          const Part<NW> a_l = L.A[p_l], c_l = CUR[p_l];
          for (uint32_t hi = 0; hi < nb; ++hi) {
            const int p = __builtin_amdgcn_readlane((int)p_l, (int)hi);
            Part<NW> a, c;
#pragma unroll
            for (int w = 0; w < NW; ++w) {
                a.w[w] = (uint32_t)__builtin_amdgcn_readlane((int)a_l.w[w], (int)hi);
                c.w[w] = (uint32_t)__builtin_amdgcn_readlane((int)c_l.w[w], (int)hi);
            }
#pragma unroll
            for (int k = 0; k < NW; ++k) {
                if (k >= T.RF) break;
                if ((k == 0) != (pass == 0)) continue;
                if (a.w[k] != kNoneW) continue;
                const uint32_t hmix = slo ^ fmix32(shi + (uint32_t)rho * 0x9E3779B1u + (uint32_t)(p * NW + k) * 0x27D4EB2Fu + 0x5BD1E995u + prm.gen * 0x632BE5ABu);
                const int wl = k == 0 ? T.w00 : T.w01, wf = k == 0 ? T.w10 : T.w11;
                uint32_t key = kKeyNull, xw_l = kNoneW;
                for (int j = wave; j < n_rounds; j += n_waves) {
                    const uint32_t x = (uint32_t)(j * 64 + lane);
                    const uint32_t r = XR[x];
                    const uint32_t xw = x | (r << 16);
                    const bool okx = (r != inv) & !in4(a, xw);
                    const uint32_t cn = L.C[x];
                    int dV = dinc((int)(cn & 0xFFFFu), T.rep_lo, T.rep_hi) + dinc(L.K[r], T.rack_lo, T.rack_hi) +
                             dinc(cnt4(a, r), T.prack_lo, T.prack_hi);
                    if (k == 0) dV += dinc((int)(cn >> 16), T.lead_lo, T.lead_hi);
                    const uint32_t tie = fmix32(hmix + x * 0x165667B1u) >> 24;
                    uint32_t keyx;
                    if (kPriced) {
                        const uint32_t prx = PR[x];
                        int dP = p_in((int)(cn & 0xFFFFu), T.rep_lo, T.rep_hi, price_rep(prx)) + p_in(L.K[r], T.rack_lo, T.rack_hi, PG[r]);
                        if (k == 0) dP += p_in((int)(cn >> 16), T.lead_lo, T.lead_hi, price_lead(prx));
                        keyx = okx ? make_key_tie_p(prm.lam_max, S, dV, role_w2(c, xw, wl, wf) + (hbw ? bw_of(BW[x], k == 0) : 0), dP, tie) : kKeyNull;
                    }
                    else keyx = okx ? make_key_tie(prm.lam_max, S, dV, role_w2(c, xw, wl, wf), tie) : kKeyNull;
                    if (keyx < key) { key = keyx; xw_l = xw; }
                }
                uint32_t kmin = wave_umin(key);
                const unsigned long long bal = __ballot(key == kmin);
                const int l_win = __ffsll((long long)bal) - 1;
                uint32_t xw_win = (uint32_t)__builtin_amdgcn_readlane((int)xw_l, l_win);
                if (n_waves > 1) {
                    if (lane == 0) atomicMin(&BEST[par], ((unsigned long long)kmin << 32) | ((unsigned long long)l_win << 24) | ((unsigned long long)((xw_win & 0xFFFFu) >> 6) << 8) | (xw_win >> 16 & 0xFFu));
                    asm volatile("s_waitcnt lgkmcnt(0)\n\ts_barrier" ::: "memory");
                    const unsigned long long bw = BEST[par];
                    const int nxt = par == 2 ? 0 : par + 1;
                    if (tid == 0) BEST[nxt == 2 ? 0 : nxt + 1] = ~0ull;
                    par = nxt;
                    const uint32_t lo = (uint32_t)bw;
                    xw_win = (((lo >> 8) & 0xFFFFu) << 6 | (lo >> 24)) | ((lo & 0xFFu) << 16);
                }
                a.w[k] = xw_win;
                if (lane == 0) {
                    const int owner = (int)(((xw_win & 0xFFFFu) >> 6) & (uint32_t)(n_waves - 1));
                    if (wave == owner) {
                        reinterpret_cast<uint32_t *>(&L.A[p])[k] = xw_win;
                        L.C[xw_win & 0xFFFFu] += (k == 0) ? 0x10001u : 1u;
                    }
                    L.K[xw_win >> 16] += 1;
                }
            }
          }
        }
        __builtin_amdgcn_fence(__ATOMIC_SEQ_CST, "workgroup");
        __syncthreads();
    }
}

constexpr size_t search_lds_total(size_t maxP, size_t maxBx, size_t waves, bool global_a, bool priced, size_t nw, bool bw, int maxR, size_t team, bool cur_global) {
    const size_t a = global_a ? 0 : maxP * 4 * nw, bx64 = (maxBx + 63) & ~(size_t)63, krt = (size_t)search_rack_tab(maxR);
    const size_t shared = (cur_global ? 0 : a) + krt * 4 + bx64 + (priced ? (bw ? 2 : 1) * bx64 * 4 + krt * 4 : 0);
    if (team > 0)
        return shared + bx64 * 6 + krt * 4 + team * krt * 4 + 2 * 16 * kTeamRec * 4 + 16 * 2 * 4;
    return shared + waves * (a + bx64 * 6 + krt * 8);
}
size_t search_lds_bytes(int maxP, int maxBx, int waves, bool global_a, bool priced, int nw, bool bw, int maxR, int team, bool cur_global) {
    return search_lds_total((size_t)maxP, (size_t)maxBx, (size_t)waves, global_a, priced, (size_t)nw, bw, maxR, (size_t)team, cur_global);
}
static_assert(search_lds_total(50, 500, 4, false, false, 4, false, 10, 0, false) == 19104 && search_lds_total(50, 500, 4, false, false, 8, false, 10, 0, false) == 23104 &&
              search_lds_total(50, 500, 4, false, true, 4, false, 10, 0, false) == 21408 && search_lds_total(50, 500, 4, false, true, 4, true, 10, 0, false) == 23456 &&
              search_lds_total(9800, 500, 1, false, false, 4, false, 10, 0, true) == 161152 && search_lds_total(100000, 500, 1, true, false, 4, false, 10, 8, false) == 7808,
              "search_lds_total no longer sums the LDS carve of search_body");

bool search_rf3_eligible(bool global_a, bool cur_global, bool priced, int nw, int team) { return !global_a && !cur_global && !priced && nw == 4 && team == 0; }

void launch_search(const SearchPools &pools, const SearchParams &prm, int n_blocks, int waves, bool global_a, bool priced, int nw, void *stream, int team, int rft) {
    const bool curg = prm.cur_global != 0 && !global_a, wide = prm.wide != 0;
    const size_t lds = search_lds_bytes(prm.maxP, prm.maxBx, waves, global_a, priced, nw, prm.bw != 0, prm.maxR, team, curg);
    hipStream_t st = static_cast<hipStream_t>(stream);
    const dim3 grid(n_blocks), block(64 * (team > 0 && !curg ? team : waves));
    if (rft == 3 && search_rf3_eligible(global_a, curg, priced, nw, team)) {
        if (wide) launch_lds<k_search<false, false, 4, true, 3>>(grid, block, lds, st, pools, prm);
        else launch_lds<k_search<false, false, 4, false, 3>>(grid, block, lds, st, pools, prm);
        return;
    }
    with_flags(priced, nw == 8, [&](auto p, auto k8) {
        constexpr bool kPriced = decltype(p)::value;
        constexpr int NW = decltype(k8)::value ? 8 : 4;
        if (curg) launch_lds<k_search_curg<kPriced, NW>>(grid, block, lds, st, pools, prm);
        else if (team > 0) launch_lds<k_team<kPriced, NW>>(grid, block, lds, st, pools, prm);
        else if (global_a) launch_lds<k_search<true, kPriced, NW, true>>(grid, block, lds, st, pools, prm);
        else if (wide) launch_lds<k_search<false, kPriced, NW, true>>(grid, block, lds, st, pools, prm);
        else launch_lds<k_search<false, kPriced, NW, false>>(grid, block, lds, st, pools, prm);
    });
}

bool launch_init(const SearchPools &pools, const SearchParams &prm, int n_blocks, int per_block, bool priced, int nw, int waves, void *stream) {
    const size_t lds = init_lds_bytes(prm.maxBx, prm.maxR, priced, prm.bw != 0);
    if (lds > 160 * 1024) return false;
    waves = waves > 0 ? std::min(kInitWaves, waves) : std::min(8, std::max(1, (prm.maxBx + 63) / 64));
    while (waves & (waves - 1)) waves &= waves - 1;
    const dim3 grid((unsigned)(n_blocks * per_block)), block((unsigned)(64 * waves));
    with_flags(priced, nw == 8, [&](auto p, auto k8) {
        launch_lds<k_init<decltype(p)::value, decltype(k8)::value ? 8 : 4>>(grid, block, lds, static_cast<hipStream_t>(stream), pools, prm, per_block);
    });
    return true;
}

}
```

kafka_assignment_optimizer_amd/csrc/kao_search_dev.h:

```cpp
#pragma once
#include <hip/hip_runtime.h>

#include <type_traits>

#include "kao_device.h"
#include "kao_internal.h"

namespace kao {

__device__ __forceinline__ uint32_t fmix32(uint32_t h) {
    h ^= h >> 16; h *= 0x85EBCA6Bu; h ^= h >> 13; h *= 0xC2B2AE35u; h ^= h >> 16;
    return h;
}
__device__ __forceinline__ uint32_t xs32(uint32_t &s) {
    s ^= s << 13; s ^= s >> 17; s ^= s << 5;
    return s;
}
__device__ __forceinline__ uint32_t mulhi(uint32_t a, uint32_t b) { return __umulhi(a, b); }
__device__ __forceinline__ int band(int c, int lo, int hi) { return max(c - hi, 0) + max(lo - c, 0); }
__device__ __forceinline__ int dinc(int c, int lo, int hi) { return (int)(c >= hi) - (int)(c < lo); }
__device__ __forceinline__ int ddec(int c, int lo, int hi) { return (int)(c <= lo) - (int)(c > hi); }

template <int NW> struct alignas(16) Part { uint32_t w[NW]; };
__device__ __forceinline__ uint32_t sel4(const Part<4> &a, int k) {
    const uint32_t lo = (k & 2) ? a.w[2] : a.w[0];
    const uint32_t hi = (k & 2) ? a.w[3] : a.w[1];
    return (k & 1) ? hi : lo;
}
__device__ __forceinline__ uint32_t sel4(const Part<8> &a, int k) {
    const uint32_t q0 = (k & 4) ? a.w[4] : a.w[0], q1 = (k & 4) ? a.w[5] : a.w[1], q2 = (k & 4) ? a.w[6] : a.w[2], q3 = (k & 4) ? a.w[7] : a.w[3];
    const uint32_t lo = (k & 2) ? q2 : q0, hi = (k & 2) ? q3 : q1;
    return (k & 1) ? hi : lo;
}
template <int NW> __device__ __forceinline__ void set_slot(Part<NW> &a, int k, uint32_t v) {
#pragma unroll
    for (int i = 0; i < NW; ++i) a.w[i] = (i == k) ? v : a.w[i];
}
__device__ __forceinline__ uint32_t lcg24(uint32_t &s) {
    asm("v_mad_u32_u24 %0, %0, %1, %2" : "+v"(s) : "s"(0x6D2B79u), "v"(0x3C6EF3u));
    return s;
}
__device__ __forceinline__ uint32_t rnd24(uint32_t &s, uint32_t n8) {
    const uint32_t v = lcg24(s);
    return (uint32_t)(((unsigned long long)(v & 0xFFFFFFu) * (unsigned long long)(n8 & 0xFFFFFFu)) >> 32);
}
__device__ __forceinline__ uint32_t rnd24_wide(uint32_t &s, uint32_t n) {
    const uint32_t v = lcg24(s);
    return __umulhi((v & 0xFFFFFFu) << 8, n);
}
__device__ __forceinline__ uint32_t key_of(int delta, uint32_t low) {
    delta = min(max(delta, -kDBias), kDBias - 2);
    return ((uint32_t)(delta + kDBias) << 8) | low;
}
__device__ __forceinline__ uint32_t make_key_p(int lam, int S, int dV, int dObj, int dP, int lane) { return key_of(__mul24(lam, dV) - __mul24(S, dObj) + dP, (uint32_t)lane); }
__device__ __forceinline__ uint32_t make_key(int lam, int S, int dV, int dObj, int lane) { return key_of(__mul24(lam, dV) - __mul24(S, dObj), (uint32_t)lane); }
__device__ __forceinline__ uint32_t make_key_tie_p(int lam, int S, int dV, int dObj, int dP, uint32_t tie) { return key_of(__mul24(lam, dV) - __mul24(S, dObj) + dP, tie & 0xFFu); }
__device__ __forceinline__ uint32_t make_key_tie(int lam, int S, int dV, int dObj, uint32_t tie) { return key_of(__mul24(lam, dV) - __mul24(S, dObj), tie & 0xFFu); }
__device__ __forceinline__ int price_rep(uint32_t pr) { return (int)(short)(pr & 0xFFFFu); }
__device__ __forceinline__ int price_lead(uint32_t pr) { return (int)pr >> 16; }
__device__ __forceinline__ int p_in(int c, int lo, int hi, int price) { return ((c >= hi) | (c < lo)) ? price : 0; }
__device__ __forceinline__ int p_out(int c, int lo, int hi, int price) { return ((c > hi) | (c <= lo)) ? -price : 0; }
__device__ __forceinline__ int bw_of(uint32_t bw, bool lead) { return (int)(bw & 0xFFFFu) + (lead ? (int)(bw >> 16) : 0); }
__device__ __forceinline__ int price_units(int v, int S) { return min(max((S * v + kDualScale / 2) >> kDualLog2, -32767), 32767); }

template <int NS = 0, int NW> __device__ __forceinline__ bool in4(const Part<NW> &a, uint32_t w) {
    bool r = false;
#pragma unroll
    for (int i = 0; i < (NS ? NS : NW); ++i) r |= a.w[i] == w;
    return r;
}
template <int NS = 0, int NW> __device__ __forceinline__ int cnt4(const Part<NW> &a, uint32_t r) {
    int n = 0;
#pragma unroll
    for (int i = 0; i < (NS ? NS : NW); ++i) n += (int)((a.w[i] >> 16) == r);
    return n;
}
template <int NS, int NW> __device__ __forceinline__ uint32_t sel_slot(const Part<NW> &a, int k) {
    if constexpr (NS == 3 && NW == 4) {
        int k1 = k & 1, k2 = k & 2;
        asm("" : "+v"(k1), "+v"(k2));
        const uint32_t w0 = a.w[0], w1 = a.w[1], w2 = a.w[2];
        return k2 ? w2 : (k1 ? w1 : w0);
    } else return sel4(a, k);
}

struct TopicRegs {
    int P, RF, R, m, Bx;
    uint32_t magic;
    int rep_lo, rep_hi, lead_lo, lead_hi, rack_lo, rack_hi, prack_lo, prack_hi;
    int w00, w01, w10, w11;
};

template <int RFT = 0> __device__ __forceinline__ TopicRegs topic_regs(const TopicDev *TD) {
    TopicRegs T;
    T.P = TD->P; T.RF = RFT ? RFT : TD->RF; T.R = TD->R; T.m = TD->m; T.Bx = TD->Bx; T.magic = TD->magic;
    T.rep_lo = TD->rep_lo; T.rep_hi = TD->rep_hi; T.lead_lo = TD->lead_lo; T.lead_hi = TD->lead_hi;
    T.rack_lo = TD->rack_lo; T.rack_hi = TD->rack_hi; T.prack_lo = TD->prack_lo; T.prack_hi = TD->prack_hi;
    T.w00 = TD->w00; T.w01 = TD->w01; T.w10 = TD->w10; T.w11 = TD->w11;
    return T;
}

template <int NS = 0, int NW> __device__ __forceinline__ int role_w2(const Part<NW> &c, uint32_t w, int wl, int wf) {
    bool fol = false;
#pragma unroll
    for (int i = 1; i < (NS ? NS : NW); ++i) fol |= c.w[i] == w;
    return (c.w[0] == w) ? wl : (fol ? wf : 0);
}
template <int NS = 0, int NW> __device__ __forceinline__ int role_w(const TopicRegs &T, const Part<NW> &c, uint32_t w, int nr) {
    return role_w2<NS>(c, w, nr ? T.w01 : T.w00, nr ? T.w11 : T.w10);
}
__device__ __forceinline__ uint32_t to_word(const TopicRegs &T, uint32_t x) {
    return x == 0xFFFFu ? kNoneW : (x | (mulhi(x, T.magic) << 16));
}
template <int NW> __device__ __forceinline__ Part<NW> load_packed(const TopicRegs &T, const unsigned char *base, int p) {
    Part<NW> a;
    if (NW == 4) {
        const uint2 s = reinterpret_cast<const uint2 *>(base)[p];
        a.w[0] = to_word(T, s.x & 0xFFFFu); a.w[1] = to_word(T, s.x >> 16); a.w[2] = to_word(T, s.y & 0xFFFFu); a.w[3] = to_word(T, s.y >> 16);
    } else {
        const uint4 s = reinterpret_cast<const uint4 *>(base)[p];
        const uint32_t v[4] = {s.x, s.y, s.z, s.w};
#pragma unroll
        for (int i = 0; i < NW / 2; ++i) { a.w[2 * i] = to_word(T, v[i & 3] & 0xFFFFu); a.w[2 * i + 1] = to_word(T, v[i & 3] >> 16); }
    }
    return a;
}
template <int NW> __device__ __forceinline__ void store_packed(unsigned char *base, int p, const Part<NW> &a) {
    if (NW == 4) reinterpret_cast<uint2 *>(base)[p] = make_uint2((a.w[0] & 0xFFFFu) | (a.w[1] << 16), (a.w[2] & 0xFFFFu) | (a.w[3] << 16));
    else reinterpret_cast<uint4 *>(base)[p] = make_uint4((a.w[0] & 0xFFFFu) | (a.w[1] << 16), (a.w[2] & 0xFFFFu) | (a.w[3] << 16),
                                                         (a.w[4 % NW] & 0xFFFFu) | (a.w[5 % NW] << 16), (a.w[6 % NW] & 0xFFFFu) | (a.w[7 % NW] << 16));
}
template <int NW> __device__ __forceinline__ int part_rack_viol(const TopicRegs &T, const Part<NW> &a) {
    int s = 0, touched = 0;
#pragma unroll
    for (int k = 0; k < NW; ++k) {
        const uint32_t rk = a.w[k] >> 16;
        bool first = a.w[k] != kNoneW;
#pragma unroll
        for (int j = 0; j < k; ++j) first &= (a.w[j] >> 16) != rk;
        if (first) { s += band(cnt4(a, rk), T.prack_lo, T.prack_hi); touched++; }
    }
    return s + (T.R - touched) * T.prack_lo;
}

constexpr int kTeamRec = 12;
template <int NW> struct WaveLds {
    Part<NW> *A;
    uint32_t *C;
    uint16_t *W;
    int *K;
    int *RT;
};

constexpr int kWIncR = 0, kWDecR = 2, kWPinR = 4, kWPoutR = 5, kWIncL = 6, kWDecL = 8, kWPinL = 10, kWPoutL = 11;
__device__ __forceinline__ int wfld(uint32_t w, int off) { return __builtin_amdgcn_sbfe((int)w, (unsigned)off, 2u); }
__device__ __forceinline__ int wfldw(uint32_t w, int off, uint32_t width) { return __builtin_amdgcn_sbfe((int)w, (unsigned)off, width); }
__device__ __forceinline__ int wflag(uint32_t w, int off) { return __builtin_amdgcn_sbfe((int)w, (unsigned)off, 1u); }
__device__ __forceinline__ int wflagw(uint32_t w, int off, uint32_t width) { return __builtin_amdgcn_sbfe((int)w, (unsigned)off, width); }
constexpr unsigned long long band_entry_of(int a, int b) {
    const int di = (b >= 0 ? 1 : 0) - (a < 0 ? 1 : 0), dd = (a <= 0 ? 1 : 0) - (b > 0 ? 1 : 0);
    const int pin = (b >= 0 || a < 0) ? 1 : 0, pout = (b > 0 || a <= 0) ? 1 : 0;
    return (unsigned long long)((di & 3) | ((dd & 3) << 2) | (pin << 4) | (pout << 5));
}
constexpr unsigned long long band_table() {
    unsigned long long t = 0;
    for (int a = -1; a <= 1; ++a) for (int b = -1; b <= 1; ++b) t |= band_entry_of(a, b) << (6 * (3 * (a + 1) + (b + 1)));
    return t;
}
constexpr unsigned long long kBandTab = band_table();
__device__ __forceinline__ int clamp_pm1(int x) {
    int r;
    asm("v_med3_i32 %0, %1, -1, 1" : "=v"(r) : "v"(x));
    return r;
}
__device__ __forceinline__ uint32_t band_entry(int c, int lo, int hi) {
    const int a = clamp_pm1(c - lo), b = clamp_pm1(c - hi);
    int t;
    asm("v_mad_i32_i24 %0, %1, 3, %2" : "=v"(t) : "v"(a), "v"(b));
    return (uint32_t)(kBandTab >> (uint32_t)(__mul24(t, 6) + 24)) & 63u;
}
__device__ __forceinline__ uint32_t band_fields(const TopicRegs &T, uint32_t c) {
    return band_entry((int)(c & 0xFFFFu), T.rep_lo, T.rep_hi) | (band_entry((int)(c >> 16), T.lead_lo, T.lead_hi) << 6);
}
constexpr uint32_t kWRowR = 0x003Fu, kWRowL = 0x0FC0u;
constexpr uint32_t kWNoCand = 0x8000u;
constexpr uint32_t kWNoCand2 = 0x4000u;
template <int NW> __device__ __forceinline__ void rebuild_band_state(const TopicRegs &T, const WaveLds<NW> &L, const uint8_t *XR, uint32_t inv, int lane, int stride = 64) {
    for (int x = lane; x < ((T.Bx + 63) & ~63); x += stride) L.W[x] = (uint16_t)(XR[x] == inv ? (kWNoCand | kWNoCand2) : band_fields(T, L.C[x]));
}

template <int NW> __device__ __forceinline__ void recount(const TopicRegs &T, const WaveLds<NW> &L, int lane, int stride, int krt) {
    for (int x = lane; x < ((T.Bx + 63) & ~63); x += stride) L.C[x] = 0;
    for (int r = lane; r < krt; r += stride) L.K[r] = 0;
    if (stride > 64) __syncthreads();
    for (int p = lane; p < T.P; p += stride) {
        const Part<NW> a = L.A[p];
#pragma unroll
        for (int k = 0; k < NW; ++k)
            if (a.w[k] != kNoneW) { atomicAdd(&L.C[a.w[k] & 0xFFFFu], k == 0 ? 0x10001u : 1u); atomicAdd(&L.K[a.w[k] >> 16], 1); }
    }
}

template <int NW, bool kTeam = false> __device__ __forceinline__ void full_cost(const TopicRegs &T, const WaveLds<NW> &L, const Part<NW> *CUR, const int *RSZ,
                                                            int lane, int stride, int &V, int &obj, const uint32_t *BW = nullptr,
                                                            int *TS = nullptr, int wave = 0, int n_waves = 1) {
    int v = 0, o = 0;
    for (int p = lane; p < T.P; p += stride) {
        const Part<NW> a = L.A[p];
        const Part<NW> c = CUR[p];
#pragma unroll
        for (int k = 0; k < NW; ++k)
            if (a.w[k] != kNoneW) o += role_w(T, c, a.w[k], k == 0 ? 0 : 1);
        v += part_rack_viol(T, a);
    }
    for (int x = lane; x < T.Bx; x += stride) {
        const int r = (int)mulhi((uint32_t)x, T.magic);
        if (x - r * T.m < RSZ[r]) {
            const uint32_t c = L.C[x];
            v += band((int)(c & 0xFFFFu), T.rep_lo, T.rep_hi) + band((int)(c >> 16), T.lead_lo, T.lead_hi);
            if (BW) { const uint32_t bw = BW[x]; o += (int)(c & 0xFFFFu) * (int)(bw & 0xFFFFu) + (int)(c >> 16) * (int)(bw >> 16); }
        }
    }
    for (int r = lane; r < T.R; r += stride) v += band(L.K[r], T.rack_lo, T.rack_hi);
    V = wave_sum(v);
    obj = wave_sum(o);
    if (kTeam) {
        __syncthreads();
        if ((lane & 63) == 0) { TS[2 * wave] = V; TS[2 * wave + 1] = obj; }
        __syncthreads();
        int tv = 0, to = 0;
        if ((lane & 63) < n_waves) { tv = TS[2 * (lane & 63)]; to = TS[2 * (lane & 63) + 1]; }
        V = wave_sum(tv);
        obj = wave_sum(to);
    }
}

template <int NW> __device__ __forceinline__ void snapshot(const TopicRegs &T, const WaveLds<NW> &L, const uint16_t *ext, uint16_t *best, int lane, int stride = 64) {
    for (int p = lane; p < T.P; p += stride) {
        const Part<NW> a = L.A[p];
        uint16_t *o = best + p * T.RF;
#pragma unroll
        for (int k = 0; k < NW; ++k)
            if (k < T.RF) o[k] = ext[a.w[k] & 0xFFFFu];
    }
}

}
```

kafka_assignment_optimizer_amd/csrc/kao_session.cpp:

```cpp
#include <cstring>

#include "kao_host.h"

namespace {

constexpr int kEvRing = 32;

template <typename Item>
std::vector<Item> xcd_order(const std::vector<Item> &items, const std::vector<int> &topic_of) {
    const size_t n = items.size();
    std::vector<std::vector<size_t>> q(8);
    for (size_t i = 0; i < n; ++i) q[(size_t)topic_of[i] % 8].push_back(i);
    std::vector<size_t> head(8, 0);
    std::vector<Item> out;
    out.reserve(n);
    for (size_t b = 0; b < n; ++b) {
        size_t x = b % 8;
        if (head[x] >= q[x].size()) {
            size_t bestx = 0, bestlen = 0;
            for (size_t y = 0; y < 8; ++y)
                if (q[y].size() - head[y] > bestlen) { bestlen = q[y].size() - head[y]; bestx = y; }
            x = bestx;
            out.push_back(items[q[x].back()]);
            q[x].pop_back();
            continue;
        }
        out.push_back(items[q[x][head[x]++]]);
    }
    return out;
}

int session_drain_events(kao_session *s) {
    for (int i = 0; i < s->ev_pending; ++i) {
        float a = 0, b = 0;
        HIP_TRY(hipEventSynchronize(s->ev[i * 3 + 2]));
        HIP_TRY(hipEventElapsedTime(&a, s->ev[i * 3 + 0], s->ev[i * 3 + 1]));
        HIP_TRY(hipEventElapsedTime(&b, s->ev[i * 3 + 1], s->ev[i * 3 + 2]));
        s->ms_search += a;
        s->ms_eval += b;
    }
    s->ev_pending = 0;
    return KAO_OK;
}

int resolve_opts(const kao_topic *topics, int n_topics, const kao_opts *opts_in, int n_cu, uint64_t device_bytes, kao_opts &o) {
    o = opts_in ? *opts_in : kao_opts{};
    if (o.team < 0 || o.team > kTeamMax || o.schedule < 0 || o.schedule > 1) return fail(KAO_ERR_INVALID, "kao_opts: team must be 0..8, schedule 0 or 1");
    if (o.iters_per_launch <= 0) o.iters_per_launch = 512;
    if (o.obj_scale <= 0) o.obj_scale = 4;
    if (o.lam_min <= 0) o.lam_min = 1;
    if (o.lam_max <= 0) o.lam_max = 40;
    if (o.lam_max < o.lam_min) o.lam_max = o.lam_min;
    if (o.period_log2 < 0) o.period_log2 = 0;
    if (o.period_log2 > 20) o.period_log2 = 20;
    if (o.time_limit_s <= 0) o.time_limit_s = 10.0;
    if (o.elite_period < 0) o.elite_period = 0;
    if (o.restarts <= 0) {
        const int want = n_cu * 32;
        int r = want / n_topics;
        r = (r / kWaves) * kWaves;
        o.restarts = std::min(std::max(r, 8), 8192);
        int64_t slots = 1;
        for (int t = 0; t < n_topics; ++t) slots = std::max<int64_t>(slots, (int64_t)topics[t].n_partitions * std::max(topics[t].rf, 1));
        const int floor_r = slots >= 32768 ? 4 * n_cu : n_cu;
        const int cap = (int)std::max<int64_t>(floor_r, (((int64_t)1 << 22) / slots) / kWaves * kWaves);
        o.restarts = std::min(o.restarts, cap);
        if (n_topics == 1 && o.restarts > n_cu && o.restarts <= n_cu + n_cu / 4 && o.team <= 1) {
            const kao_topic &t0 = topics[0];
            std::vector<int> rs((size_t)std::max(t0.n_racks, 1), 0);
            for (int b = 0; b < t0.n_brokers; ++b) if (t0.rack_of[b] < rs.size()) rs[t0.rack_of[b]]++;
            const int bx = *std::max_element(rs.begin(), rs.end()) * t0.n_racks, nw0 = (t0.rf > kRFP || t0.rf_cur > kRFP) ? 2 * kRFP : kRFP;
            const bool hbw = t0.broker_w || t0.broker_wl;
            if (search_lds_bytes(t0.n_partitions, bx, 1, false, true, nw0, hbw, t0.n_racks) > kLdsLimit &&
                search_lds_bytes(t0.n_partitions, bx, 1, false, true, nw0, hbw, t0.n_racks, 0, true) <= kLdsLimit)
                o.restarts = n_cu / kWaves * kWaves;
        }
    }
    if (o.restarts > (1 << 20) - 2) o.restarts = (1 << 20) - 2;
    uint64_t per_restart = 0;
    for (int t = 0; t < n_topics; ++t) per_restart += (uint64_t)topics[t].n_partitions * (32 + 2 * (uint64_t)std::max(topics[t].rf, 1));
    uint64_t budget = 8ull << 30;
    if (device_bytes > 0) budget = std::min<uint64_t>(budget, std::max<uint64_t>(device_bytes / 8, 256ull << 20));
    const uint64_t cap = budget / std::max<uint64_t>(per_restart, 1);
    if ((uint64_t)o.restarts > cap) o.restarts = (int)std::max<uint64_t>(cap / kWaves * kWaves, kWaves);
    return KAO_OK;
}

struct SessionPlan {
    std::vector<TopicDev> tds;
    std::vector<int2> smap;
    std::vector<int4> emap;
    std::vector<uint32_t> cur_pool, bw_pool, bwd_pool; std::vector<uint16_t> ext_pool, curd_pool, int_pool; std::vector<int32_t> rsz_pool;
    std::vector<uint8_t> rackof_pool;
    uint64_t state_bytes = 0, best_u16 = 0, win_u16 = 0, dual_i32 = 0, price_i32 = 0, wide_slices = 0;
};
template <typename T>
uint32_t append(std::vector<T> &pool, const std::vector<T> &v) { pool.insert(pool.end(), v.begin(), v.end()); return (uint32_t)(pool.size() - v.size()); }

void plan_topic(kao_session &s, int t, bool curg_on, int n_cu, SessionPlan &pl) {
    const kao_opts &o = s.opts;
    const PreparedTopic &pt = s.pts[(size_t)t];
    TopicDev &d = s.pts[(size_t)t].d;
    d.n_restarts = o.restarts;
    d.period_log2 = o.period_log2 > 0 ? o.period_log2 : auto_period_log2(d.P, d.RF);
    d.restart_base = t * o.restarts;
    std::vector<uint32_t> &cur_pool = pl.cur_pool;
    while (cur_pool.size() % 4) cur_pool.push_back(kNoneW);
    d.cur_off = (uint32_t)cur_pool.size();
    for (size_t i = 0; i < (size_t)d.P * d.nw; ++i) cur_pool.push_back(replica_word(pt.cur_int[i], d.m));
    {
        d.hole_off = (uint32_t)cur_pool.size();
        const size_t w0 = (size_t)d.cur_off;
        std::vector<uint32_t> lead, foll;
        for (int p = 0; p < d.P; ++p) {
            bool fh = false;
            for (int k = 1; k < d.RF; ++k) fh |= cur_pool[w0 + (size_t)p * d.nw + k] == kNoneW;
            if (cur_pool[w0 + (size_t)p * d.nw] == kNoneW) lead.push_back((uint32_t)p);
            if (fh) foll.push_back((uint32_t)p);
        }
        cur_pool.push_back((uint32_t)lead.size()); cur_pool.push_back((uint32_t)foll.size());
        append(cur_pool, lead);
        append(cur_pool, foll);
    }
    const bool both_fit = search_lds_bytes(d.P, d.Bx, 1, false, true, d.nw, s.any_bw, d.R) <= kLdsLimit;
    const bool curg = !both_fit && curg_on && o.team <= 1 && o.restarts <= n_cu &&
                      search_lds_bytes(d.P, d.Bx, 1, false, true, d.nw, s.any_bw, d.R, 0, true) <= kLdsLimit;
    const bool global_a = !both_fit && !curg;
    s.topic_global[(size_t)t] = global_a;
    s.topic_curg[(size_t)t] = curg;
    d.ext_off = append(pl.ext_pool, pt.ext_of);
    d.rsz_off = append(pl.rsz_pool, pt.rack_size);
    d.state_off = pl.state_bytes;
    pl.state_bytes += align_up((uint64_t)o.restarts * d.P * d.nw * (global_a ? 4 : 2));
    d.best_off = pl.best_u16;
    pl.best_u16 += (uint64_t)o.restarts * d.P * d.RF;
    d.win_off = (uint32_t)pl.win_u16;
    pl.win_u16 += (uint64_t)d.P * d.RF;
    d.rackof_off = append(pl.rackof_pool, pt.rack_of);
    d.curd_off = append(pl.curd_pool, pt.cur_dense);
    if (d.has_bw) {
        d.bw_off = append(pl.bw_pool, pt.bw_int);
        d.bwd_off = append(pl.bwd_pool, pt.bw_dense);
        s.priced = true;
        s.any_bw = true;
    }
    d.int_off = append(pl.int_pool, pt.int_of);
    d.price_off = (uint32_t)pl.price_i32;
    pl.price_i32 += 2 * (uint64_t)d.B + kRackTab;
    pl.dual_i32 = (pl.dual_i32 + 1) & ~(uint64_t)1;
    d.dual_off = (uint32_t)pl.dual_i32;
    pl.dual_i32 += 6 * (uint64_t)d.B + 3 * kRackTab + 8;
    d.cnt_off = (uint32_t)pl.dual_i32;
    pl.dual_i32 += 3 * (2 * (uint64_t)d.B + kRackTab) + 4 * (uint64_t)d.B + 2 * kRackTab;
    pl.wide_slices += (uint64_t)(d.P + 63) / 64;
    s.eval_bytes_per_launch += (uint64_t)o.restarts * (uint64_t)(2 * d.RF * d.P + 2 * d.rf_cur * d.P + d.B);
}

int plan_groups(kao_session &s, int n_cu, SessionPlan &pl) {
    const kao_opts &o = s.opts;
    const bool rft_on = env_int("KAO_SEARCH_RFT", 1) != 0;
    std::vector<int> order((size_t)s.n_topics);
    for (int t = 0; t < s.n_topics; ++t) order[(size_t)t] = t;
    auto need1 = [&](int t) {
        const TopicDev &d = s.pts[(size_t)t].d;
        const bool ga = s.topic_global[(size_t)t] != 0;
        const bool cg = s.topic_curg[(size_t)t] != 0;
        return (ga ? ((size_t)1 << 40) : 0) + (cg ? ((size_t)1 << 39) : 0) + (d.nw > kRFP ? ((size_t)1 << 41) : 0) + search_lds_bytes(d.P, d.Bx, 1, ga, true, d.nw, s.any_bw, d.R, 0, cg);
    };
    std::stable_sort(order.begin(), order.end(), [&](int x, int y) { return need1(x) < need1(y); });
    std::vector<std::vector<int>> members;
    size_t group_base = 0;
    auto kind = [&](int t) { return (s.topic_global[(size_t)t] ? 1 : 0) | (s.pts[(size_t)t].d.nw > kRFP ? 2 : 0) | (s.topic_curg[(size_t)t] ? 4 : 0); };
    int lds_groups = 0, group_kind = -1;
    for (int t : order) {
        const bool new_kind = members.empty() || kind(t) != group_kind;
        if (new_kind || (need1(t) > 2 * group_base && lds_groups < 8)) {
            members.emplace_back(); group_base = need1(t); group_kind = kind(t);
            if (new_kind) lds_groups = 1; else ++lds_groups;
        }
        members.back().push_back(t);
    }
    for (const std::vector<int> &mem : members) {
        kao_session::LaunchGroup g;
        int64_t n_cand = 0;
        for (int t : mem) n_cand += s.pts[(size_t)t].d.n_restarts;
        const int64_t fill = 4 * (int64_t)std::max(n_cu, 1);
        int cpb = 32;
        if (n_cand < fill * 32) cpb = (int)std::min<int64_t>(32, std::max<int64_t>(kWaves, ((n_cand + fill - 1) / fill + kWaves - 1) / kWaves * kWaves));
        for (int t : mem) {
            const TopicDev &d = s.pts[(size_t)t].d;
            g.rf_uniform = g.rf_uniform < 0 ? d.RF : (g.rf_uniform == d.RF ? d.RF : 0);
            g.rf3 = g.rf3 && d.RF == 3 && d.rf_cur <= 3;
            g.maxP = std::max(g.maxP, d.P); g.maxBx = std::max(g.maxBx, d.Bx); g.maxB = std::max(g.maxB, d.B); g.maxR = std::max(g.maxR, d.R); g.wide = g.wide || (int64_t)d.P * d.RF >= 512;
        }
        g.rf3 = g.rf3 && rft_on;
        g.global_a = s.topic_global[(size_t)mem[0]] != 0;
        g.cur_global = s.topic_curg[(size_t)mem[0]] != 0;
        g.nw = s.pts[(size_t)mem[0]].d.nw;
        g.eval_coop = n_cand <= fill && g.maxP >= 1024;
        if (g.eval_coop) cpb = 1;
        if (g.global_a) {
            const int tmax = g.nw > kRFP ? kTeamMax / 2 : kTeamMax;
            const int want = o.team == 0 ? 1 : o.team;
            g.team = want <= 1 ? 0 : std::min(want, tmax);
            if (g.team > 0) g.waves = 1;
        }
        auto search_lds = [&] { return search_lds_bytes(g.maxP, g.maxBx, g.waves, g.global_a, true, g.nw, s.any_bw, g.maxR, g.team, g.cur_global); };
        while (g.waves > 1 && search_lds() > kLdsLimit) g.waves /= 2;
        g.cur_in_lds = eval_lds_bytes(g.maxP, g.maxB, true, g.nw) <= kLdsLimit;
        if (search_lds() > kLdsLimit || eval_lds_bytes(g.maxP, g.maxB, g.cur_in_lds, g.nw) > kLdsLimit)
            return fail(KAO_ERR_UNSUPPORTED, "broker tables exceed 160 KiB of LDS (about 30,000 padded brokers)");
        std::vector<int2> gs; std::vector<int> gs_topic;
        std::vector<int4> ge; std::vector<int> ge_topic;
        for (int t : mem) {
            const TopicDev &d = s.pts[(size_t)t].d;
            for (int r = 0; r < d.n_restarts; r += g.waves) { gs.push_back(make_int2(t, r)); gs_topic.push_back(t); }
            for (int r = 0; r < d.n_restarts; r += cpb) {
                ge.push_back(make_int4(t, r, std::min(cpb, d.n_restarts - r), d.restart_base + r));
                ge_topic.push_back(t);
            }
        }
        gs = xcd_order(gs, gs_topic);
        ge = xcd_order(ge, ge_topic);
        g.smap_off = (int)pl.smap.size(); g.smap_n = (int)gs.size();
        g.emap_off = (int)pl.emap.size(); g.emap_n = (int)ge.size();
        pl.smap.insert(pl.smap.end(), gs.begin(), gs.end());
        pl.emap.insert(pl.emap.end(), ge.begin(), ge.end());
        s.groups.push_back(g);
    }
    s.blocks_search = (int)pl.smap.size();
    s.blocks_eval = (int)pl.emap.size();
    return KAO_OK;
}

int plan_session(kao_session &s, const kao_topic *topics, int n_cu, SessionPlan &pl) {
    const int n_topics = s.n_topics;
    s.pts.resize((size_t)n_topics);
    s.topics.assign(topics, topics + n_topics);
    s.ub.resize((size_t)n_topics);
    s.topic_global.assign((size_t)n_topics, 0);
    s.topic_curg.assign((size_t)n_topics, 0);
    for (int t = 0; t < n_topics; ++t) s.any_bw |= topics[t].broker_w || topics[t].broker_wl;
    const bool curg_on = env_int("KAO_CUR_GLOBAL", 1) != 0;
    for (int t = 0; t < n_topics; ++t) {
        const uint64_t seed = s.opts.seed ^ ((uint64_t)(t + 1) * 0x9E3779B97F4A7C15ull);
        const int rc = prepare(&topics[t], seed, s.pts[(size_t)t]);
        if (rc) return rc;
        s.ub[(size_t)t] = upper_bound_w(&topics[t]);
        s.topic_infeasible.push_back(infeasible_reason(&topics[t]).empty() ? 0 : 1);
        plan_topic(s, t, curg_on, n_cu, pl);
        s.dual_ok.push_back(dual_supported(&topics[t], s.any_bw) ? 1 : 0);
    }
    s.dual_flags.assign((size_t)n_topics, 0);
    s.dual_iters.assign((size_t)n_topics, 0);
    for (int t = 0; t < n_topics; ++t) if (!s.dual_ok[(size_t)t]) s.dual_flags[(size_t)t] = 8;
    s.total_restarts = n_topics * s.opts.restarts;
    const int rc = plan_groups(s, n_cu, pl);
    for (const PreparedTopic &pt : s.pts) pl.tds.push_back(pt.d);
    return rc;
}

struct ArenaLayout {
    struct Sec { void *slot; size_t off, bytes; const void *src; };
    std::vector<Sec> secs;
    size_t total = 0;
    template <typename T>
    void add(T *&dev_ptr, size_t bytes, const void *src = nullptr) {
        secs.push_back({&dev_ptr, total, bytes, src});
        total += align_up(bytes);
    }
    template <typename T, typename V>
    void add(T *&dev_ptr, const std::vector<V> &image) { add(dev_ptr, image.size() * sizeof(V), image.data()); }
    void stage(unsigned char *host) const {
        for (const Sec &sec : secs) if (sec.bytes && sec.src) std::memcpy(host + sec.off, sec.src, sec.bytes);
    }
    void bind(void *base) const {
        for (const Sec &sec : secs) { unsigned char *p = static_cast<unsigned char *>(base) + sec.off; std::memcpy(sec.slot, &p, sizeof p); }
    }
};

ArenaLayout layout_ro(kao_session &s, const SessionPlan &pl) {
    ArenaLayout a;
    a.add(s.d_topics, pl.tds);
    a.add(s.d_smap, pl.smap);
    a.add(s.d_emap, pl.emap);
    a.add(s.d_cur, pl.cur_pool);
    a.add(s.d_ext, pl.ext_pool);
    a.add(s.d_rsz, pl.rsz_pool);
    a.add(s.d_rackof, pl.rackof_pool);
    a.add(s.d_curd, pl.curd_pool);
    a.add(s.d_int, pl.int_pool);
    a.add(s.d_bw, pl.bw_pool);
    a.add(s.d_bwd, pl.bwd_pool);
    return a;
}

ArenaLayout layout_rw(kao_session &s, const SessionPlan &pl) {
    const size_t n_topics = (size_t)s.n_topics, n_restarts = (size_t)s.total_restarts;
    s.rb_viol_off = align_up(n_topics * 8 + 16, 16);
    s.rb_assign_off = s.rb_viol_off + n_topics * 32;
    s.readback_bytes = s.rb_assign_off + pl.win_u16 * 2;
    uint64_t dual_i32 = (pl.dual_i32 + 1) & ~(uint64_t)1;
    s.wide_ctl_i32 = dual_i32; dual_i32 += 32 * (uint64_t)n_topics;
    s.wide_map_i32 = dual_i32; dual_i32 += 2 * pl.wide_slices;
    s.dual_bytes = align_up(dual_i32 * 4);
    s.dual_rb_bytes = n_topics * 24;
    s.price_half_i32 = align_up(pl.price_i32 * 4) / 4;
    s.best_bytes = pl.best_u16 * 2 ? pl.best_u16 * 2 : 2;
    ArenaLayout a;
    a.add(s.d_state, pl.state_bytes);
    a.add(s.d_best, pl.best_u16 * 2);
    a.add(s.d_info, n_restarts * 16);
    a.add(s.d_obj, n_restarts * 4);
    a.add(s.d_viol, n_restarts * 32);
    a.add(s.d_readback, s.readback_bytes);
    a.add(s.d_dual, s.dual_bytes);
    a.add(s.d_dual_target, n_topics * 8);
    a.add(s.d_dual_ids, n_topics * 4);
    a.add(s.d_dual_rb, s.dual_rb_bytes);
    a.add(s.d_price, 2 * s.price_half_i32 * 4);
    a.add(s.d_keys_glob, n_topics * 8);
    return a;
}

}

extern "C" {

void kao_session_destroy(kao_session *s) {
    if (!s) return;
    (void)hipSetDevice(s->device);
    if (s->stream) (void)hipStreamSynchronize(s->stream);
    if (s->stream_bound) (void)hipStreamSynchronize(s->stream_bound);
    if (s->ev_bound0) (void)hipEventDestroy(s->ev_bound0);
    if (s->ev_bound1) (void)hipEventDestroy(s->ev_bound1);
    if (s->ev_search) (void)hipEventDestroy(s->ev_search);
    if (s->stream_bound) (void)hipStreamDestroy(s->stream_bound);
    arena_put(s->arena_ro, s->arena_ro_bytes, s->device);
    arena_put(s->arena_rw, s->arena_rw_bytes, s->device);
    for (hipEvent_t e : s->ev) (void)hipEventDestroy(e);
    stream_put(s->stream, s->device);
    delete s;
}

int kao_session_create(const kao_topic *topics, int32_t n_topics, const kao_opts *opts_in, kao_session **out) {
    if (!out) return fail(KAO_ERR_INVALID, "null out");
    *out = nullptr;
    if (!topics || n_topics < 1) return fail(KAO_ERR_INVALID, "no topics");
    int rc = require_init();
    if (rc) return rc;
    SessionPtr s(new kao_session());
    s->device = cur_device();
    s->n_topics = n_topics;
    const int n_cu = num_cu(s->device);
    size_t free_b = 0, total_b = 0;
    if (hipMemGetInfo(&free_b, &total_b) != hipSuccess) total_b = 0;
    if ((rc = resolve_opts(topics, n_topics, opts_in, n_cu, total_b, s->opts))) return rc;
    SessionPlan pl;
    if ((rc = plan_session(*s, topics, n_cu, pl))) return rc;

    const ArenaLayout ro = layout_ro(*s, pl), rw = layout_rw(*s, pl);
    if ((rc = arena_get(ro.total, &s->arena_ro, &s->arena_ro_bytes))) return rc;
    if ((rc = arena_get(rw.total, &s->arena_rw, &s->arena_rw_bytes))) return rc;
    ro.bind(s->arena_ro);
    rw.bind(s->arena_rw);
    s->d_keys = reinterpret_cast<unsigned long long *>(s->d_readback);
    s->d_drift = reinterpret_cast<int32_t *>(s->d_readback + (size_t)n_topics * 8);
    s->d_win_viol = reinterpret_cast<int32_t *>(s->d_readback + s->rb_viol_off);
    s->d_win_assign = reinterpret_cast<uint16_t *>(s->d_readback + s->rb_assign_off);
    s->h_readback.assign(s->readback_bytes, 0);
    std::vector<unsigned char> stage(ro.total);
    ro.stage(stage.data());

    if ((rc = stream_get(&s->stream))) return rc;
    const size_t price_b = 2 * s->price_half_i32 * 4;
    hipError_t e1 = hipMemcpyAsync(s->arena_ro, stage.data(), ro.total, hipMemcpyHostToDevice, s->stream);
    hipError_t e2 = hipMemsetAsync(s->d_best, 0xFF, s->best_bytes, s->stream);
    hipError_t e3 = hipMemsetAsync(s->d_readback, 0xFF, (size_t)n_topics * 8, s->stream);
    hipError_t e4 = hipMemsetAsync(s->d_drift, 0, 16, s->stream);
    if (e4 == hipSuccess) e4 = hipMemsetAsync(s->d_price, 0, price_b ? price_b : 4, s->stream);
    hipError_t e5 = hipStreamSynchronize(s->stream);
    if (e1 != hipSuccess || e2 != hipSuccess || e3 != hipSuccess || e4 != hipSuccess || e5 != hipSuccess) return fail(KAO_ERR_HIP, "session upload failed");
    if (s->opts.profile) {
        s->ev.resize(kEvRing * 3);
        for (auto &e : s->ev) if (hipEventCreate(&e) != hipSuccess) return fail(KAO_ERR_HIP, "hipEventCreate");
    }
    *out = s.release();
    return KAO_OK;
}

int kao_session_step(kao_session *s) {
    if (!s) return fail(KAO_ERR_INVALID, "null session");
    HIP_TRY(hipSetDevice(s->device));
    const bool prof = s->opts.profile != 0;
    if (prof && s->ev_pending == kEvRing) {
        int rc = session_drain_events(s);
        if (rc) return rc;
    }
    SearchPools sp{};
    sp.topics = s->d_topics; sp.block_map = s->d_smap; sp.cur_pool = s->d_cur; sp.ext_pool = s->d_ext; sp.rsz_pool = s->d_rsz;
    sp.state_pool = s->d_state; sp.best_pool = s->d_best; sp.restart_info = s->d_info; sp.drift = s->d_drift;
    SearchParams prm{};
    prm.obj_scale = s->opts.obj_scale; prm.lam_min = s->opts.lam_min; prm.lam_max = s->opts.lam_max;
    prm.launch = s->launch; prm.iters = (uint32_t)s->opts.iters_per_launch; prm.init = (s->launch == 0 || s->reinit) ? 1 : 0;
    prm.gen = s->gen;
    s->reinit = false;
    const int eper = s->opts.elite_period;
    prm.bw = s->any_bw ? 1 : 0;
    prm.scan2_max = kScanTwoSlots;
    prm.elite = (eper > 0 && s->launch > 0 && s->launch % (uint32_t)eper == 0) ? 1 : 0;
    sp.price_pool = s->d_price + (size_t)s->price_read * s->price_half_i32;
    sp.int_pool = s->d_int; sp.elite_assign = s->d_win_assign; sp.elite_key = s->d_keys; sp.bw_pool = s->d_bw;
    EvalPools ep{};
    ep.topics = s->d_topics; ep.rackof_pool = s->d_rackof; ep.curd_pool = s->d_curd;
    ep.cand = s->d_best; ep.objective = s->d_obj; ep.violations = s->d_viol; ep.best_key = s->d_keys; ep.bwd_pool = s->d_bwd;
    hipEvent_t *e = prof ? &s->ev[(size_t)s->ev_pending * 3] : nullptr;
    if (prof) HIP_TRY(hipEventRecord(e[0], s->stream));
    for (const kao_session::LaunchGroup &g : s->groups) {
        sp.block_map = s->d_smap + g.smap_off;
        prm.maxP = g.maxP; prm.maxBx = g.maxBx; prm.maxR = g.maxR; prm.wide = g.wide ? 1 : 0; prm.cur_global = g.cur_global ? 1 : 0;
        SearchParams gp = prm;
        if (gp.init && g.global_a) {
            const int init_waves = (int)env_int("KAO_INIT_WAVES", -1);
            if (init_waves != 0 && launch_init(sp, gp, g.smap_n, g.team > 0 ? 1 : g.waves, s->priced, g.nw, std::max(init_waves, 0), s->stream)) gp.init = 2;
            HIP_TRY(hipGetLastError());
        }
        const int rft = g.rf3 ? 3 : 0;
        launch_search(sp, gp, g.smap_n, g.waves, g.global_a, s->priced, g.nw, s->stream, g.team, rft);
        if (rft && search_rf3_eligible(g.global_a, g.cur_global, s->priced, g.nw, g.team)) s->search_rf3_launches++;
        HIP_TRY(hipGetLastError());
    }
    if (prof) HIP_TRY(hipEventRecord(e[1], s->stream));
    for (const kao_session::LaunchGroup &g : s->groups) {
        ep.block_map = s->d_emap + g.emap_off;
        ep.maxP = g.maxP; ep.maxB = g.maxB; ep.cur_in_lds = g.cur_in_lds ? 1 : 0; ep.coop = g.eval_coop ? 1 : 0; ep.rf_uniform = std::max(g.rf_uniform, 0);
        launch_eval(ep, g.emap_n, g.nw, s->stream);
        HIP_TRY(hipGetLastError());
    }
    if (prof) { HIP_TRY(hipEventRecord(e[2], s->stream)); s->ev_pending++; }
    if (eper > 0 && (s->launch + 1) % (uint32_t)eper == 0) {
        launch_gather(s->d_topics, s->n_topics, s->d_keys, s->d_best, s->d_viol, s->d_win_assign, s->d_win_viol, s->stream);
        HIP_TRY(hipGetLastError());
    }
    for (const PreparedTopic &pt : s->pts) {
        const uint64_t n = neighbours_in_range(prm.launch * prm.iters, prm.iters, pt.d.RF, pt.d.B, pt.d.P, prm.scan2_max) * (uint64_t)pt.d.n_restarts;
        s->delta_total += n;
        s->search_bytes_total += n * (uint64_t)(8 * pt.d.RF + 10);
    }
    s->launch++;
    return KAO_OK;
}

int kao_session_new_generation(kao_session *s) {
    if (!s) return fail(KAO_ERR_INVALID, "null session");
    HIP_TRY(hipSetDevice(s->device));
    HIP_TRY(hipMemsetAsync(s->d_best, 0xFF, s->best_bytes, s->stream));
    HIP_TRY(hipMemsetAsync(s->d_readback, 0xFF, (size_t)s->n_topics * 8, s->stream));
    s->gen++;
    s->reinit = true;
    return KAO_OK;
}

int kao_session_sync(kao_session *s) {
    if (!s) return fail(KAO_ERR_INVALID, "null session");
    HIP_TRY(hipSetDevice(s->device));
    HIP_TRY(hipStreamSynchronize(s->stream));
    if (s->opts.profile) return session_drain_events(s);
    return KAO_OK;
}

int kao_session_best_keys(kao_session *s, uint64_t *keys) {
    if (!s || !keys) return fail(KAO_ERR_INVALID, "null argument");
    HIP_TRY(hipSetDevice(s->device));
    HIP_TRY(hipMemcpyAsync(keys, s->d_keys, (size_t)s->n_topics * 8, hipMemcpyDeviceToHost, s->stream));
    HIP_TRY(hipStreamSynchronize(s->stream));
    return KAO_OK;
}

int kao_session_device_keys(kao_session *s, void **d_keys) {
    if (!s || !d_keys) return fail(KAO_ERR_INVALID, "null argument");
    *d_keys = s->d_keys;
    return KAO_OK;
}

int kao_session_best(kao_session *s, kao_result *results) {
    if (!s || !results) return fail(KAO_ERR_INVALID, "null argument");
    HIP_TRY(hipSetDevice(s->device));
    launch_gather(s->d_topics, s->n_topics, s->d_keys, s->d_best, s->d_viol, s->d_win_assign, s->d_win_viol, s->stream);
    HIP_TRY(hipGetLastError());
    HIP_TRY(hipMemcpyAsync(s->h_readback.data(), s->d_readback, s->readback_bytes, hipMemcpyDeviceToHost, s->stream));
    int rc = kao_session_sync(s);
    if (rc) return rc;
    const uint64_t *keys = reinterpret_cast<const uint64_t *>(s->h_readback.data());
    const int32_t *wv = reinterpret_cast<const int32_t *>(s->h_readback.data() + s->rb_viol_off);
    const uint16_t *wa = reinterpret_cast<const uint16_t *>(s->h_readback.data() + s->rb_assign_off);
    for (int t = 0; t < s->n_topics; ++t) {
        const TopicDev &d = s->pts[(size_t)t].d;
        kao_result &r = results[t];
        r.upper_bound = s->ub[(size_t)t];
        const uint64_t key = keys[t];
        if (key == ~0ull) {
            r.status = s->topic_infeasible[(size_t)t] ? KAO_STATUS_INFEASIBLE_PROVEN : KAO_STATUS_NO_FEASIBLE; r.best_restart = -1; r.objective = -1;
            std::memset(r.violations, 0, sizeof r.violations);
            continue;
        }
        r.best_restart = (key & 0xFFFFF) == kExternalRestart ? -1 : (int)(key & 0xFFFFF);
        r.objective = (int64_t)kObjCap - (int64_t)((key >> 20) & 0xFFFFFF);
        std::memcpy(r.violations, wv + (size_t)t * 8, 32);
        if (r.assignment) std::memcpy(r.assignment, wa + d.win_off, (size_t)d.P * d.RF * 2);
        if (r.violations[0] != 0) { r.status = s->topic_infeasible[(size_t)t] ? KAO_STATUS_INFEASIBLE_PROVEN : KAO_STATUS_NO_FEASIBLE; r.objective = -1; }
        else r.status = r.objective >= r.upper_bound ? KAO_STATUS_OPTIMAL_PROVEN : KAO_STATUS_FEASIBLE_BOUND_GAP;
    }
    return KAO_OK;
}

int kao_session_stats(kao_session *s, kao_stats *out) {
    if (!s || !out) return fail(KAO_ERR_INVALID, "null argument");
    int rc = kao_session_sync(s);
    if (rc) return rc;
    std::memset(out, 0, sizeof *out);
    out->launches = s->launch;
    out->delta_candidates = s->delta_total;
    out->full_candidates = (uint64_t)s->launch * (uint64_t)s->total_restarts;
    out->ms_search = s->ms_search; out->ms_eval = s->ms_eval;
    out->search_bytes_algo = s->search_bytes_total;
    out->eval_bytes_algo = s->eval_bytes_per_launch * s->launch;
    out->n_restarts_total = s->total_restarts;
    for (const kao_session::LaunchGroup &g : s->groups)
        out->lds_bytes_search = std::max(out->lds_bytes_search, (int32_t)search_lds_bytes(g.maxP, g.maxBx, g.waves, g.global_a, s->priced, g.nw, s->any_bw, g.maxR, g.team, g.cur_global));
    out->launch_groups = (int32_t)s->groups.size();
    out->blocks_search = s->blocks_search;
    out->search_rf3_launches = (int32_t)std::min<uint64_t>(s->search_rf3_launches, (uint64_t)INT32_MAX);
    HIP_TRY(hipMemcpy(&out->drift, s->d_drift, 4, hipMemcpyDeviceToHost));
    return KAO_OK;
}

int kao_session_restart_state(kao_session *s, int32_t topic, int32_t restart, uint16_t *final_state, uint16_t *best_state,
                              int32_t info[4]) {
    if (!s || topic < 0 || topic >= s->n_topics) return fail(KAO_ERR_INVALID, "bad topic");
    const PreparedTopic &pt = s->pts[(size_t)topic];
    const TopicDev &d = pt.d;
    if (restart < 0 || restart >= d.n_restarts) return fail(KAO_ERR_INVALID, "bad restart");
    HIP_TRY(hipSetDevice(s->device));
    int rc = kao_session_sync(s);
    if (rc) return rc;
    if (final_state) {
        const bool ga = s->topic_global[(size_t)topic] != 0;
        const int nw = d.nw;
        std::vector<uint16_t> raw((size_t)d.P * nw * (ga ? 2 : 1));
        HIP_TRY(hipMemcpy(raw.data(), s->d_state + d.state_off + (uint64_t)restart * d.P * nw * (ga ? 4 : 2), raw.size() * 2, hipMemcpyDeviceToHost));
        for (int p = 0; p < d.P; ++p)
            for (int k = 0; k < d.RF; ++k) {
                const uint16_t x = ga ? raw[((size_t)p * nw + k) * 2] : raw[(size_t)p * nw + k];
                final_state[(size_t)p * d.RF + k] = x < pt.ext_of.size() ? pt.ext_of[x] : (uint16_t)KAO_NONE;
            }
    }
    if (best_state)
        HIP_TRY(hipMemcpy(best_state, s->d_best + d.best_off + (uint64_t)restart * d.P * d.RF, (size_t)d.P * d.RF * 2, hipMemcpyDeviceToHost));
    if (info) HIP_TRY(hipMemcpy(info, s->d_info + (size_t)(d.restart_base + restart) * 4, 16, hipMemcpyDeviceToHost));
    return KAO_OK;
}

}

namespace kao {

int session_topic_best(kao_session *s, int i, uint16_t *out) {
    HIP_TRY(hipSetDevice(s->device));
    launch_gather(s->d_topics, s->n_topics, s->d_keys, s->d_best, s->d_viol, s->d_win_assign, s->d_win_viol, s->stream);
    HIP_TRY(hipGetLastError());
    const TopicDev &d = s->pts[(size_t)i].d;
    HIP_TRY(hipMemcpyAsync(out, s->d_win_assign + d.win_off, (size_t)d.P * d.RF * 2, hipMemcpyDeviceToHost, s->stream));
    HIP_TRY(hipStreamSynchronize(s->stream));
    return KAO_OK;
}
int session_restart_objs(kao_session *s, int i, std::vector<int32_t> &objs) {
    HIP_TRY(hipSetDevice(s->device));
    const TopicDev &d = s->pts[(size_t)i].d;
    std::vector<int32_t> info((size_t)d.n_restarts * 4);
    HIP_TRY(hipMemcpyAsync(info.data(), s->d_info + (size_t)d.restart_base * 4, info.size() * 4, hipMemcpyDeviceToHost, s->stream));
    HIP_TRY(hipStreamSynchronize(s->stream));
    objs.resize((size_t)d.n_restarts);
    for (int r = 0; r < d.n_restarts; ++r) objs[(size_t)r] = info[(size_t)r * 4];
    return KAO_OK;
}
int session_restart_best(kao_session *s, int i, int restart, uint16_t *out) {
    HIP_TRY(hipSetDevice(s->device));
    const TopicDev &d = s->pts[(size_t)i].d;
    if (restart < 0 || restart >= d.n_restarts) return fail(KAO_ERR_INVALID, "bad restart");
    HIP_TRY(hipMemcpyAsync(out, s->d_best + d.best_off + (uint64_t)restart * d.P * d.RF, (size_t)d.P * d.RF * 2, hipMemcpyDeviceToHost, s->stream));
    HIP_TRY(hipStreamSynchronize(s->stream));
    return KAO_OK;
}
int session_adopt_external(kao_session *s, int i, const uint16_t *assign, int64_t objective, uint64_t *key_out) {
    HIP_TRY(hipSetDevice(s->device));
    const TopicDev &d = s->pts[(size_t)i].d;
    const uint64_t key = ((uint64_t)((int64_t)kObjCap - objective) << 20) | (uint64_t)kExternalRestart;
    HIP_TRY(hipStreamSynchronize(s->stream));
    HIP_TRY(hipMemcpyAsync(s->d_win_assign + d.win_off, assign, (size_t)d.P * d.RF * 2, hipMemcpyHostToDevice, s->stream));
    HIP_TRY(hipMemcpyAsync(s->d_keys + i, &key, 8, hipMemcpyHostToDevice, s->stream));
    HIP_TRY(hipStreamSynchronize(s->stream));
    *key_out = key;
    return KAO_OK;
}

}
```

kafka_assignment_optimizer_amd/solver.py:

```python
from __future__ import annotations

import ctypes as C
from dataclasses import dataclass
from typing import List, Optional, Sequence

import numpy as np

from . import _ffi
from .model import BOUND_KEYS, Topic

STATUS_NAMES = {0: "OPTIMAL_PROVEN", 1: "FEASIBLE_BOUND_GAP", 2: "NO_FEASIBLE", 3: "TIME_LIMIT", 4: "INFEASIBLE_PROVEN"}


class KaoError(RuntimeError):
    def __init__(self, code: int, where: str):
        lib = _ffi.load()
        detail = lib.kao_last_error().decode(errors="replace")
        super().__init__(f"{where}: {lib.kao_strerror(code).decode()} ({code}) {detail}")
        self.code = code


def _check(rc: int, where: str):
    if rc != 0:
        raise KaoError(rc, where)


def library_path() -> str:
    return _ffi.LIB_PATH


def init(device: int = 0):
    _check(_ffi.load().kao_init(int(device)), "kao_init")


def device_name() -> str:
    buf = C.create_string_buffer(256)
    _check(_ffi.load().kao_device_name(buf, 256), "kao_device_name")
    return buf.value.decode()


class _CTopics:

    def __init__(self, topics: Sequence[Topic]):
        self.keep = []
        self.arr = (_ffi.KaoTopic * len(topics))()
        for i, t in enumerate(topics):
            s = self.arr[i]
            rack = np.ascontiguousarray(t.rack_of, dtype=np.uint8)
            cur = np.ascontiguousarray(t.current, dtype=np.uint16)
            self.keep += [rack, cur]
            s.n_brokers, s.n_racks, s.n_partitions = t.n_brokers, int(t.n_racks), int(t.n_partitions)
            s.rf, s.rf_cur = int(t.rf), int(cur.shape[1])
            s.rack_of = rack.ctypes.data_as(C.POINTER(C.c_uint8))
            s.current = cur.ctypes.data_as(C.POINTER(C.c_uint16))
            for a in range(2):
                for b in range(2):
                    s.w[a][b] = int(t.weights[a][b])
            for k in BOUND_KEYS:
                v = t.bounds_override.get(k, -1) if t.bounds_override else -1
                setattr(s, k, -1 if v is None else int(v))
            for name in ("broker_w", "broker_wl"):
                v = getattr(t, name, None)
                if v is not None:
                    arr = np.ascontiguousarray(v, dtype=np.int32)
                    if arr.shape != (t.n_brokers,):
                        raise ValueError(f"{name}: one weight per broker expected")
                    self.keep.append(arr)
                    setattr(s, name, arr.ctypes.data_as(C.POINTER(C.c_int32)))

    def ptr(self, i: int = 0):
        return C.byref(self.arr[i]) if i else self.arr


def derive_bounds(topic: Topic) -> dict:
    ct = _CTopics([topic])
    out = (C.c_int32 * 8)()
    _check(_ffi.load().kao_derive_bounds(ct.arr, out), "kao_derive_bounds")
    return dict(zip(BOUND_KEYS, [int(v) for v in out]))


def upper_bound(topic: Topic) -> int:
    ct = _CTopics([topic])
    ub = C.c_int64()
    _check(_ffi.load().kao_upper_bound(ct.arr, C.byref(ub)), "kao_upper_bound")
    return int(ub.value)


def check_infeasible(topic: Topic) -> str:
    ct = _CTopics([topic])
    buf = C.create_string_buffer(256)
    rc = _ffi.load().kao_check_infeasible(ct.arr, buf, 256)
    if rc < 0:
        raise KaoError(rc, "kao_check_infeasible")
    return buf.value.decode() if rc == 1 else ""


def evaluate(topic: Topic, assign) -> tuple:
    ct = _CTopics([topic])
    a = np.ascontiguousarray(assign, dtype=np.uint16).reshape(-1)
    if a.size != topic.n_partitions * topic.rf:
        raise ValueError("assignment must have P*rf entries")
    obj = C.c_int64()
    viol = (C.c_int32 * 8)()
    _check(_ffi.load().kao_evaluate(ct.arr, a.ctypes.data_as(C.POINTER(C.c_uint16)), C.byref(obj), viol),
           "kao_evaluate")
    return int(obj.value), np.array(list(viol), dtype=np.int64)


def evaluate_batch(topic: Topic, candidates) -> tuple:
    ct = _CTopics([topic])
    c = np.ascontiguousarray(candidates, dtype=np.uint16).reshape(-1, topic.n_partitions * topic.rf)
    n = c.shape[0]
    obj = np.zeros(n, dtype=np.int32)
    viol = np.zeros((n, 8), dtype=np.int32)
    _check(_ffi.load().kao_evaluate_batch(ct.arr, c.ctypes.data_as(C.POINTER(C.c_uint16)), n,
                                          obj.ctypes.data_as(C.POINTER(C.c_int32)),
                                          viol.ctypes.data_as(C.POINTER(C.c_int32))), "kao_evaluate_batch")
    return obj, viol


def canonicalize(topic: Topic, assign) -> np.ndarray:
    ct = _CTopics([topic])
    a = np.ascontiguousarray(assign, dtype=np.uint16).reshape(-1).copy()
    _check(_ffi.load().kao_canonicalize(ct.arr, a.ctypes.data_as(C.POINTER(C.c_uint16))), "kao_canonicalize")
    return a.reshape(topic.n_partitions, topic.rf)


def improve_cycles(topic: Topic, assign, max_rounds: int = 0) -> tuple:
    ct = _CTopics([topic])
    a = np.ascontiguousarray(assign, dtype=np.uint16).reshape(-1).copy()
    if a.size != topic.n_partitions * topic.rf:
        raise ValueError("assignment must have P*rf entries")
    obj = C.c_int64()
    st = (C.c_int32 * 8)()
    _check(_ffi.load().kao_improve_cycles(ct.arr, a.ctypes.data_as(C.POINTER(C.c_uint16)), int(max_rounds), C.byref(obj), st),
           "kao_improve_cycles")
    names = ("rounds", "improving_rounds", "realisations", "improving", "candidates", "merged", "objective_before", "objective_after")
    return a.reshape(topic.n_partitions, topic.rf), int(obj.value), dict(zip(names, (int(v) for v in st)))


def cycle_matrices(topic: Topic, assign, layer: int, level: int) -> tuple:
    ct = _CTopics([topic])
    a = np.ascontiguousarray(assign, dtype=np.uint16).reshape(-1)
    n = len(topic.broker_ids) + int(topic.n_racks) + 1
    dist = np.zeros((n, n), dtype=np.int32)
    mid = np.zeros((n, n), dtype=np.int32)
    slot = np.zeros((n, n), dtype=np.uint32)
    _check(_ffi.load().kao_cycle_matrices(ct.arr, a.ctypes.data_as(C.POINTER(C.c_uint16)), layer, level,
                                          dist.ctypes.data_as(C.POINTER(C.c_int32)), mid.ctypes.data_as(C.POINTER(C.c_int32)),
                                          slot.ctypes.data_as(C.POINTER(C.c_uint32))), "kao_cycle_matrices")
    return dist, mid, slot


def cycle_seeds(topic: Topic, assign) -> np.ndarray:
    ct = _CTopics([topic])
    a = np.ascontiguousarray(assign, dtype=np.uint16).reshape(-1)
    ncfg = C.c_int32()
    _check(_ffi.load().kao_cycle_seeds(ct.arr, a.ctypes.data_as(C.POINTER(C.c_uint16)), None, C.byref(ncfg)), "kao_cycle_seeds")
    tab = np.zeros((topic.n_partitions, ncfg.value, 2), dtype=np.int32)
    _check(_ffi.load().kao_cycle_seeds(ct.arr, a.ctypes.data_as(C.POINTER(C.c_uint16)), tab.ctypes.data_as(C.POINTER(C.c_int32)), C.byref(ncfg)),
           "kao_cycle_seeds")
    return tab


def cycle_pair_edges(topic: Topic, assign, gmin: int = -2):
    ct = _CTopics([topic])
    a = np.ascontiguousarray(assign, dtype=np.uint16).reshape(-1)
    B = topic.n_brokers
    cost = np.zeros((B, B), dtype=np.int32)
    st = (C.c_int64 * 4)()
    _check(_ffi.load().kao_cycle_pair_edges(ct.arr, a.ctypes.data_as(C.POINTER(C.c_uint16)), int(gmin), cost.ctypes.data_as(C.POINTER(C.c_int32)), st),
           "kao_cycle_pair_edges")
    return cost, dict(half_moves=int(st[0]), pairs=int(st[1]), edges=int(st[2]), closed_improving=int(st[3]))


class EvalPlan:

    def __init__(self, topic: Topic):
        self.topic = topic
        self._ct = _CTopics([topic])
        self._h = C.c_void_p()
        _check(_ffi.load().kao_eval_plan_create(self._ct.arr, C.byref(self._h)), "kao_eval_plan_create")

    def run(self, d_candidates: int, n: int, d_objective: int, d_violations: int = 0, d_best_key: int = 0):
        _check(_ffi.load().kao_eval_plan_run(self._h, C.c_void_p(d_candidates), int(n), C.c_void_p(d_objective),
                                             C.c_void_p(d_violations or None), C.c_void_p(d_best_key or None)),
               "kao_eval_plan_run")

    def sync(self) -> float:
        ms = C.c_double()
        _check(_ffi.load().kao_eval_plan_sync(self._h, C.byref(ms)), "kao_eval_plan_sync")
        return float(ms.value)

    def close(self):
        if self._h:
            _ffi.load().kao_eval_plan_destroy(self._h)
            self._h = C.c_void_p()

    def __del__(self):
        try:
            self.close()
        except Exception:
            pass


@dataclass
class Result:
    status: str
    objective: int
    upper_bound: int
    violations: np.ndarray
    assignment: np.ndarray
    best_restart: int
    seconds_to_best: float


def _make_opts(**kw) -> _ffi.KaoOpts:
    o = _ffi.KaoOpts()
    for k, v in kw.items():
        if not hasattr(o, k):
            raise TypeError(f"unknown option {k}")
        setattr(o, k, v)
    return o


def _results_buffers(topics: Sequence[Topic]):
    res = (_ffi.KaoResult * len(topics))()
    bufs = []
    for i, t in enumerate(topics):
        b = np.full(t.n_partitions * t.rf, 0xFFFF, dtype=np.uint16)
        bufs.append(b)
        res[i].assignment = b.ctypes.data_as(C.POINTER(C.c_uint16))
    return res, bufs


def _unpack(topics, res, bufs) -> List[Result]:
    out = []
    for i, t in enumerate(topics):
        r = res[i]
        out.append(Result(STATUS_NAMES.get(r.status, str(r.status)), int(r.objective), int(r.upper_bound),
                          np.array(list(r.violations), dtype=np.int64), bufs[i].reshape(t.n_partitions, t.rf).copy(),
                          int(r.best_restart), float(r.seconds_to_best)))
    return out


class Session:

    def __init__(self, topics: Sequence[Topic], **opts):
        self.topics = list(topics)
        self._ct = _CTopics(self.topics)
        self._opts = _make_opts(**opts)
        self._h = C.c_void_p()
        _check(_ffi.load().kao_session_create(self._ct.arr, len(self.topics), C.byref(self._opts), C.byref(self._h)),
               "kao_session_create")

    def step(self, n: int = 1):
        lib = _ffi.load()
        for _ in range(n):
            _check(lib.kao_session_step(self._h), "kao_session_step")

    def sync(self):
        _check(_ffi.load().kao_session_sync(self._h), "kao_session_sync")

    def new_generation(self):
        _check(_ffi.load().kao_session_new_generation(self._h), "kao_session_new_generation")

    def best(self) -> List[Result]:
        res, bufs = _results_buffers(self.topics)
        _check(_ffi.load().kao_session_best(self._h, res), "kao_session_best")
        return _unpack(self.topics, res, bufs)

    def device_keys_ptr(self) -> int:
        p = C.c_void_p()
        _check(_ffi.load().kao_session_device_keys(self._h, C.byref(p)), "kao_session_device_keys")
        return int(p.value)

    def best_keys(self) -> np.ndarray:
        keys = np.zeros(len(self.topics), dtype=np.uint64)
        _check(_ffi.load().kao_session_best_keys(self._h, keys.ctypes.data_as(C.POINTER(C.c_uint64))),
               "kao_session_best_keys")
        return keys

    def stats(self) -> dict:
        st = _ffi.KaoStats()
        _check(_ffi.load().kao_session_stats(self._h, C.byref(st)), "kao_session_stats")
        return {k: getattr(st, k) for k, _ in _ffi.KaoStats._fields_}

    def restart_state(self, topic: int, restart: int) -> dict:
        t = self.topics[topic]
        n = t.n_partitions * t.rf
        fin = np.zeros(n, dtype=np.uint16)
        best = np.zeros(n, dtype=np.uint16)
        info = (C.c_int32 * 4)()
        _check(_ffi.load().kao_session_restart_state(self._h, topic, restart, fin.ctypes.data_as(C.POINTER(C.c_uint16)),
                                                     best.ctypes.data_as(C.POINTER(C.c_uint16)), info),
               "kao_session_restart_state")
        return dict(final=fin.reshape(t.n_partitions, t.rf), best=best.reshape(t.n_partitions, t.rf),
                    best_obj=int(info[0]), V=int(info[1]), obj=int(info[2]), n_accept=int(info[3]))

    def bound_step(self, targets: Sequence[int], iters: int = 512):
        tg = np.ascontiguousarray(targets, dtype=np.int64)
        if tg.shape != (len(self.topics),):
            raise ValueError("one target per topic")
        _check(_ffi.load().kao_session_bound_step(self._h, tg.ctypes.data_as(C.POINTER(C.c_int64)), int(iters)),
               "kao_session_bound_step")

    def set_prices(self, topic: int, a, l, g):
        t = self.topics[topic]
        a = np.ascontiguousarray(a, dtype=np.int32); l = np.ascontiguousarray(l, dtype=np.int32); g = np.ascontiguousarray(g, dtype=np.int32)
        if a.shape != (t.n_brokers,) or l.shape != (t.n_brokers,) or g.shape[0] < t.n_racks:
            raise ValueError("a[n_brokers], l[n_brokers], g[n_racks] expected")
        p32 = C.POINTER(C.c_int32)
        _check(_ffi.load().kao_session_set_prices(self._h, topic, a.ctypes.data_as(p32), l.ctypes.data_as(p32), g.ctypes.data_as(p32)),
               "kao_session_set_prices")

    def prices(self, topic: int) -> tuple:
        t = self.topics[topic]
        a = np.zeros(t.n_brokers, dtype=np.int32); l = np.zeros(t.n_brokers, dtype=np.int32); g = np.zeros(t.n_racks, dtype=np.int32)
        p32 = C.POINTER(C.c_int32)
        _check(_ffi.load().kao_session_prices(self._h, topic, a.ctypes.data_as(p32), l.ctypes.data_as(p32), g.ctypes.data_as(p32)),
               "kao_session_prices")
        return a, l, g

    def adopt_prices(self):
        _check(_ffi.load().kao_session_adopt_prices(self._h), "kao_session_adopt_prices")

    def bounds(self) -> dict:
        n = len(self.topics)
        ub = np.zeros(n, dtype=np.int64)
        fl = np.zeros(n, dtype=np.int32)
        it = np.zeros(n, dtype=np.int32)
        _check(_ffi.load().kao_session_bounds(self._h, ub.ctypes.data_as(C.POINTER(C.c_int64)),
                                              fl.ctypes.data_as(C.POINTER(C.c_int32)), it.ctypes.data_as(C.POINTER(C.c_int32))),
               "kao_session_bounds")
        return dict(upper_bound=ub, flags=fl, iters=it)

    def set_dual_state(self, topic: int, a, l, g):
        a, l, g = (np.ascontiguousarray(v, dtype=np.int32) for v in (a, l, g))
        p32 = C.POINTER(C.c_int32)
        _check(_ffi.load().kao_session_set_dual_state(self._h, topic, a.ctypes.data_as(p32), l.ctypes.data_as(p32), g.ctypes.data_as(p32)),
               "kao_session_set_dual_state")

    def dual_state(self, topic: int) -> dict:
        t = self.topics[topic]
        a = np.zeros(t.n_brokers, dtype=np.int32)
        l = np.zeros(t.n_brokers, dtype=np.int32)
        g = np.zeros(t.n_racks, dtype=np.int32)
        best = C.c_int64()
        p32 = C.POINTER(C.c_int32)
        _check(_ffi.load().kao_session_dual_state(self._h, topic, a.ctypes.data_as(p32), l.ctypes.data_as(p32),
                                                  g.ctypes.data_as(p32), C.byref(best)), "kao_session_dual_state")
        return dict(a=a, l=l, g=g, best_dual=int(best.value))

    def close(self):
        if self._h:
            _ffi.load().kao_session_destroy(self._h)
            self._h = C.c_void_p()

    def __enter__(self):
        return self

    def __exit__(self, *exc):
        self.close()

    def __del__(self):
        try:
            self.close()
        except Exception:
            pass


def dual_bound(topic: Topic, target: int, iters: int = 512, launches: int = 1) -> dict:
    ct = _CTopics([topic])
    bound, best = C.c_int64(), C.c_int64()
    itn, fl = C.c_int32(), C.c_int32()
    mult = np.zeros(2 * topic.n_brokers + topic.n_racks, dtype=np.int32)
    _check(_ffi.load().kao_dual_bound(ct.ptr(0), int(target), int(iters), int(launches), C.byref(bound), C.byref(best),
                                      C.byref(itn), C.byref(fl), mult.ctypes.data_as(C.POINTER(C.c_int32))), "kao_dual_bound")
    B = topic.n_brokers
    return dict(bound=int(bound.value), best_dual=int(best.value), iters=int(itn.value), flags=int(fl.value),
                a=mult[:B].copy(), l=mult[B:2 * B].copy(), g=mult[2 * B:].copy())


def lp_bound(topic: Topic, tol: float = 0.0, max_iters: int = 0) -> dict:
    ct = _CTopics([topic])
    bound, best = C.c_int64(), C.c_int64()
    B = topic.n_brokers
    mult = np.zeros(2 * B + topic.n_racks, dtype=np.int32)
    st = np.zeros(8)
    _check(_ffi.load().kao_lp_bound(ct.ptr(0), float(tol), int(max_iters), C.byref(bound), C.byref(best),
                                    mult.ctypes.data_as(C.POINTER(C.c_int32)), st.ctypes.data_as(C.POINTER(C.c_double))), "kao_lp_bound")
    return dict(bound=int(bound.value), best_dual=int(best.value), a=mult[:B].copy(), l=mult[B:2 * B].copy(), g=mult[2 * B:].copy(),
                iterations=int(st[0]), primal=float(st[1]), dual=float(st[2]), status=int(st[3]), mu=float(st[4]), pinf=float(st[5]),
                dinf=float(st[6]), ms=float(st[7]))


def lp_round(topic: Topic, pert: float = 0.0, salt: int = 0, tol: float = 0.0, max_iters: int = 0, fallback=None) -> dict:
    ct = _CTopics([topic])
    n = topic.n_partitions * topic.rf
    a = np.zeros(n, dtype=np.uint16) if fallback is None else np.ascontiguousarray(np.asarray(fallback).reshape(-1), dtype=np.uint16).copy()
    if a.shape != (n,):
        raise ValueError("fallback: [P, rf] expected")
    obj = C.c_int64()
    viol = (C.c_int32 * 8)()
    st = np.zeros(8)
    _check(_ffi.load().kao_lp_round(ct.ptr(0), float(pert), int(salt) & 0xFFFFFFFF, float(tol), int(max_iters), 0 if fallback is None else 1,
                                    a.ctypes.data_as(C.POINTER(C.c_uint16)), C.byref(obj), viol, st.ctypes.data_as(C.POINTER(C.c_double))), "kao_lp_round")
    return dict(assignment=a.reshape(topic.n_partitions, topic.rf), objective=int(obj.value), violations=[int(v) for v in viol],
                iterations=int(st[0]), status=int(st[1]), fractional=int(st[2]), over_inflow=int(st[3]), from_fallback=int(st[4]),
                ms_lp=float(st[5]), ms_round=float(st[6]), pert=float(st[7]))


def lp_round_host(topic: Topic, q, zq, fallback=None) -> dict:
    ct = _CTopics([topic])
    n = topic.n_partitions * topic.rf
    q = np.ascontiguousarray(q, dtype=np.uint8); zq = np.ascontiguousarray(zq, dtype=np.int32)
    a = np.zeros(n, dtype=np.uint16) if fallback is None else np.ascontiguousarray(np.asarray(fallback).reshape(-1), dtype=np.uint16).copy()
    rep = (C.c_int32 * 4)()
    _check(_ffi.load().kao_lp_round_host(ct.ptr(0), q.ctypes.data_as(C.POINTER(C.c_uint8)), zq.ctypes.data_as(C.POINTER(C.c_int32)),
                                         0 if fallback is None else 1, a.ctypes.data_as(C.POINTER(C.c_uint16)), rep), "kao_lp_round_host")
    return dict(assignment=a.reshape(topic.n_partitions, topic.rf), fractional=int(rep[0]), over_inflow=int(rep[1]), unplaced=int(rep[2]), from_fallback=int(rep[3]))


def lp_repair_host(topic: Topic, assignment) -> np.ndarray:
    ct = _CTopics([topic])
    a = np.ascontiguousarray(np.asarray(assignment).reshape(-1), dtype=np.uint16).copy()
    rep = (C.c_int32 * 4)()
    _check(_ffi.load().kao_lp_round_host(ct.ptr(0), None, None, 2, a.ctypes.data_as(C.POINTER(C.c_uint16)), rep), "kao_lp_round_host")
    return a.reshape(topic.n_partitions, topic.rf)


def lp_trace(topic: Topic, tol: float = 0.0, max_iters: int = 80) -> dict:
    ct = _CTopics([topic])
    B = topic.n_brokers
    mult = np.zeros(2 * B + topic.n_racks, dtype=np.int32)
    st = np.zeros(8)
    max_iters = int(max_iters) if int(max_iters) > 0 else 80
    tr = np.zeros(5 * (max_iters + 2))
    pd = C.POINTER(C.c_double)
    _check(_ffi.load().kao_lp_trace(ct.ptr(0), float(tol), int(max_iters), tr.ctypes.data_as(pd), st.ctypes.data_as(pd),
                                    mult.ctypes.data_as(C.POINTER(C.c_int32))), "kao_lp_trace")
    it = int(st[0])
    return dict(a=mult[:B].copy(), l=mult[B:2 * B].copy(), g=mult[2 * B:].copy(), iterations=it, primal=float(st[1]), dual=float(st[2]),
                status=int(st[3]), ms=float(st[7]), trace=tr[:5 * (it + 1)].reshape(-1, 5))


def lp_sharded(topic: Topic, devices: Sequence[int], pert: float = 0.0, salt: int = 0, tol: float = 0.0, max_iters: int = 0) -> dict:
    ct = _CTopics([topic])
    dv = np.asarray(list(devices), dtype=np.int32)
    A = np.full((topic.n_partitions, topic.rf), 0xFFFF, dtype=np.uint16)
    bound = C.c_int64(0); obj = C.c_int64(0)
    viol = np.zeros(8, dtype=np.int32); st = np.zeros(8)
    _check(_ffi.load().kao_lp_sharded_test(ct.ptr(0), dv.ctypes.data_as(C.POINTER(C.c_int32)), len(dv), float(pert), int(salt), float(tol), int(max_iters),
                                           C.byref(bound), A.ctypes.data_as(C.POINTER(C.c_uint16)), C.byref(obj), viol.ctypes.data_as(C.POINTER(C.c_int32)),
                                           st.ctypes.data_as(C.POINTER(C.c_double))), "kao_lp_sharded_test")
    return dict(bound=int(bound.value), assignment=A, objective=int(obj.value), violations=viol.tolist(), iterations=int(st[0]), status=int(st[1]),
                fractional=int(st[2]), collectives=int(st[3]), dual=float(st[4]), ms_lp=float(st[5]), ms_rest=float(st[6]), pert=float(st[7]))


def dense_spd_test(A: np.ndarray, rhs: Optional[np.ndarray] = None) -> dict:
    A = np.ascontiguousarray(A, dtype=np.float64)
    n = A.shape[0]
    assert A.shape == (n, n)
    f = np.zeros((n, n)); li = np.zeros((n // 64, 64, 64)); x = np.zeros(n); ms = np.zeros(2)
    pd = C.POINTER(C.c_double)
    r = None if rhs is None else np.ascontiguousarray(rhs, dtype=np.float64)
    _check(_ffi.load().kao_dense_spd_test(A.ctypes.data_as(pd), n, None if r is None else r.ctypes.data_as(pd), f.ctypes.data_as(pd),
                                          li.ctypes.data_as(pd), x.ctypes.data_as(pd), ms.ctypes.data_as(pd)), "kao_dense_spd_test")
    return dict(factor=f, linv=li, x=x, ms_factor=float(ms[0]), ms_solve=float(ms[1]))


def decode_key(key: int) -> tuple:
    key = int(key)
    return key >> 44, 0xFFFFFF - ((key >> 20) & 0xFFFFFF), key & 0xFFFFF


def solve(topics: Sequence[Topic], target_objective: Optional[Sequence[int]] = None, **opts) -> List[Result]:
    topics = list(topics)
    ct = _CTopics(topics)
    opts.setdefault("stop_at_bound", 1)
    o = _make_opts(**opts)
    if target_objective is not None:
        tgt = (C.c_int64 * len(topics))(*[int(v) for v in target_objective])
        o.target_objective = tgt
    res, bufs = _results_buffers(topics)
    _check(_ffi.load().kao_solve(ct.arr, len(topics), C.byref(o), res), "kao_solve")
    return _unpack(topics, res, bufs)


def solve_multi(topics: Sequence[Topic], devices: Sequence[int], target_objective: Optional[Sequence[int]] = None, **opts) -> List[Result]:
    topics = list(topics)
    ct = _CTopics(topics)
    opts.setdefault("stop_at_bound", 1)
    o = _make_opts(**opts)
    if target_objective is not None:
        tgt = (C.c_int64 * len(topics))(*[int(v) for v in target_objective])
        o.target_objective = tgt
    dev = (C.c_int32 * len(devices))(*[int(d) for d in devices])
    res, bufs = _results_buffers(topics)
    _check(_ffi.load().kao_solve_multi(ct.arr, len(topics), dev, len(devices), C.byref(o), res), "kao_solve_multi")
    return _unpack(topics, res, bufs)


def solve_capped(topics: Sequence[Topic], replica_cap: Sequence[int], devices: Optional[Sequence[int]] = None, max_rounds: int = 0, **opts):
    topics = list(topics)
    ct = _CTopics(topics)
    o = _make_opts(**opts)
    cap = np.ascontiguousarray(replica_cap, dtype=np.int32)
    if cap.shape != (topics[0].n_brokers,):
        raise ValueError("one cap per broker expected")
    dev = (C.c_int32 * len(devices))(*[int(d) for d in devices]) if devices else None
    res, bufs = _results_buffers(topics)
    lb = C.c_int64()
    _check(_ffi.load().kao_solve_capped(ct.arr, len(topics), cap.ctypes.data_as(C.POINTER(C.c_int32)), dev, len(devices) if devices else 0,
                                        C.byref(o), int(max_rounds), res, C.byref(lb)), "kao_solve_capped")
    out = _unpack(topics, res, bufs)
    return out, (None if lb.value == (1 << 63) - 1 else int(lb.value))


def rccl_selftest(devices: Sequence[int]) -> None:
    dev = (C.c_int32 * len(devices))(*[int(d) for d in devices])
    _check(_ffi.load().kao_rccl_selftest(dev, len(devices)), "kao_rccl_selftest")


def rccl_loopback_counts() -> tuple:
    out = (C.c_uint64 * 2)()
    _check(_ffi.load().kao_rccl_loopback_counts(out), "kao_rccl_loopback_counts")
    return int(out[0]), int(out[1])


def last_solve_timing() -> dict:
    out = (C.c_double * 16)()
    _check(_ffi.load().kao_last_solve_timing(out), "kao_last_solve_timing")
    return dict(session_ready=out[0], time_to_best=out[1], results_read_back=out[2], returned=out[3], launches=int(out[4]),
                delta_candidates=int(out[5]), bound_launches=int(out[6]), elite_exchanges=int(out[7]), bound_iters=int(out[8]),
                cx_calls=int(out[9]), cx_gains=int(out[10]), search_iters=int(out[11]), generations=int(out[12]), cx_further_starts=int(out[13]),
                lp_solves=int(out[14]), lp_iters=int(out[15]))


def last_solve_lp() -> dict:
    out = (C.c_double * 8)()
    _check(_ffi.load().kao_last_solve_lp(out), "kao_last_solve_lp")
    return dict(solves=int(out[0]), iterations=int(out[1]), rounded=int(out[2]), adopted=int(out[3]), fractional_partitions=int(out[4]))


def last_solve_profile() -> dict:
    out = (C.c_double * 8)()
    _check(_ffi.load().kao_last_solve_profile(out), "kao_last_solve_profile")
    return dict(ms_search=out[0], ms_eval=out[1], search_launches=int(out[2]), restarts=int(out[3]), search_bytes_algo=int(out[4]),
                delta_candidates=int(out[5]), lds_bytes_search=int(out[6]), blocks_search=int(out[7]))
```

Baseline: 816.4 billion.

## Add small-cost RF-3 search kernel using packed 16-bit key arithmetic

Adds a kSmall instantiation of the unpriced RF-3 LDS search kernel, chosen at launch when lambda, objective scale and the largest weight keep every move cost within a 16-bit range. In that path move keys are built with 24-bit mad instructions and fewer ops, and the inner two-candidate scan evaluates both candidates at once with packed i16 arithmetic (v_pk_mad_i16/v_pk_add/v_pk_sub). To support this, the rack table halves are swapped and g_old is subtracted after the loop. Errors in the cost bound would break move ordering, and the env knob KAO_SEARCH_SMALL turns the path off.

```diff
diff --git a/include/kao.h b/include/kao.h
--- a/include/kao.h
+++ b/include/kao.h
@@ -126,6 +126,7 @@
 int kao_session_best_keys(kao_session *s, uint64_t *keys);
 int kao_session_device_keys(kao_session *s, void **d_keys);
 int kao_session_stats(kao_session *s, kao_stats *out);
+int kao_session_small_launches(kao_session *s, int64_t *out);
 int kao_session_bound_step(kao_session *s, const int64_t *target, int32_t iters);
 int kao_session_set_prices(kao_session *s, int32_t topic, const int32_t *a, const int32_t *l, const int32_t *g);
 int kao_session_adopt_prices(kao_session *s);
diff --git a/kafka_assignment_optimizer_amd/_ffi.py b/kafka_assignment_optimizer_amd/_ffi.py
--- a/kafka_assignment_optimizer_amd/_ffi.py
+++ b/kafka_assignment_optimizer_amd/_ffi.py
@@ -67,6 +67,7 @@
     "kao_session_best_keys": (C.c_int, [C.c_void_p, _P(C.c_uint64)]),
     "kao_session_device_keys": (C.c_int, [C.c_void_p, _P(C.c_void_p)]),
     "kao_session_stats": (C.c_int, [C.c_void_p, _P(KaoStats)]),
+    "kao_session_small_launches": (C.c_int, [C.c_void_p, _P(C.c_int64)]),
     "kao_session_restart_state": (C.c_int, [C.c_void_p, C.c_int32, C.c_int32, _P(C.c_uint16), _P(C.c_uint16),
                                             _P(C.c_int32)]),
     "kao_session_bound_step": (C.c_int, [C.c_void_p, _P(C.c_int64), C.c_int32]),
diff --git a/kafka_assignment_optimizer_amd/csrc/kao_host.h b/kafka_assignment_optimizer_amd/csrc/kao_host.h
--- a/kafka_assignment_optimizer_amd/csrc/kao_host.h
+++ b/kafka_assignment_optimizer_amd/csrc/kao_host.h
@@ -125,6 +125,7 @@
         int waves = kWaves;
         int nw = kRFP;
         int rf_uniform = -1;
+        int w_abs_max = 0;
         bool rf3 = true;
         bool global_a = false;
         bool cur_global = false;
@@ -191,6 +192,8 @@
     uint64_t eval_bytes_per_launch = 0;
     uint64_t delta_total = 0, search_bytes_total = 0;
     uint64_t search_rf3_launches = 0;
+    uint64_t search_small_launches = 0;
+    bool small_on = true;
 };
 
 namespace kao {
diff --git a/kafka_assignment_optimizer_amd/csrc/kao_internal.h b/kafka_assignment_optimizer_amd/csrc/kao_internal.h
--- a/kafka_assignment_optimizer_amd/csrc/kao_internal.h
+++ b/kafka_assignment_optimizer_amd/csrc/kao_internal.h
@@ -138,7 +138,9 @@
 size_t search_lds_bytes(int maxP, int maxBx, int waves, bool global_a, bool priced = false, int nw = 4, bool bw = false, int maxR = kRackTab - 1, int team = 0, bool cur_global = false);
 size_t eval_lds_bytes(int maxP, int maxB, bool cur_in_lds, int ne = 4);
 bool search_rf3_eligible(bool global_a, bool cur_global, bool priced, int nw, int team);
-void launch_search(const SearchPools &pools, const SearchParams &prm, int n_blocks, int waves, bool global_a, bool priced, int nw, void *stream, int team = 0, int rft = 0);
+constexpr int kSmallCostMax = 16384;
+bool search_small_cost(int lam_min, int lam_max, int obj_scale, int w_abs_max, bool priced);
+void launch_search(const SearchPools &pools, const SearchParams &prm, int n_blocks, int waves, bool global_a, bool priced, int nw, void *stream, int team = 0, int rft = 0, bool small = false);
 bool launch_init(const SearchPools &pools, const SearchParams &prm, int n_blocks, int per_block, bool priced, int nw, int waves, void *stream);
 void launch_eval(const EvalPools &pools, int n_blocks, int ne, void *stream);
 void launch_gather(const TopicDev *topics, int n_topics, const unsigned long long *keys, const uint16_t *best_pool,
diff --git a/kafka_assignment_optimizer_amd/csrc/kao_search.hip b/kafka_assignment_optimizer_amd/csrc/kao_search.hip
--- a/kafka_assignment_optimizer_amd/csrc/kao_search.hip
+++ b/kafka_assignment_optimizer_amd/csrc/kao_search.hip
@@ -2,11 +2,12 @@
 
 namespace kao {
 
-template <bool kGlobalA, bool kPriced, int NW, bool kWide, bool kTeam, bool kCurG = false, int RFT = 0>
+template <bool kGlobalA, bool kPriced, int NW, bool kWide, bool kTeam, bool kCurG = false, int RFT = 0, bool kSmall = false>
 __device__ __forceinline__ void search_body(unsigned char *smem, const SearchPools &pl, const SearchParams &prm) {
     static_assert(!kTeam || kGlobalA, "teams run topics that live in global memory");
     static_assert(!kCurG || !kGlobalA, "kCurG: the working assignment is in LDS");
     static_assert(RFT == 0 || (RFT == 3 && NW == 4 && !kGlobalA && !kTeam), "RFT = 3: LDS-resident topics of four words per partition");
+    static_assert(!kSmall || (RFT == 3 && !kPriced && !kCurG), "kSmall: the unpriced RF-3 instantiation");
     constexpr int NS = RFT ? RFT : NW;
     const int lane = threadIdx.x & 63;
     const int wave = __builtin_amdgcn_readfirstlane(threadIdx.x >> 6);
@@ -347,6 +348,7 @@
                     if (lead) dP_old -= wflag(wo, kWPoutL) & price_lead(pro);
                     dP_rack_old = p_out(L.K[ro], T.rack_lo, T.rack_hi, PG[ro]);
                 }
+                const int base_s = kSmall ? mad24s(S, g_old, kDBias) : 0;
 #pragma unroll
                 for (int g = 0; g < 4; ++g) {
                     uint32_t r, jj;
@@ -369,9 +371,10 @@
                         if (r != ro)
                             dVg += dV_rack_old + dinc(L.K[r], T.rack_lo, T.rack_hi) + dinc(cnt4<NS>(a, r), T.prack_lo, T.prack_hi);
                     }
-                    const int dObjg = role_w2<NS>(c, xw, wl, wf) + (hbw ? bw_of(BW[x], lead) : 0) - g_old;
+                    const int dObjg = role_w2<NS>(c, xw, wl, wf) + (hbw ? bw_of(BW[x], lead) : 0) - (kSmall ? 0 : g_old);
                     uint32_t keyg;
-                    if (kPriced) {
+                    if constexpr (kSmall) keyg = okg ? key_small(mad24s(-S, dObjg, mad24(lam, dVg, base_s)), (uint32_t)lane) : kKeyNull;
+                    else if (kPriced) {
                         const uint32_t prx = PR[x];
                         int dPg = dP_old + (wflag(wn, kWPinR) & price_rep(prx));
                         if (lead) dPg += wflag(wn, kWPinL) & price_lead(prx);
@@ -381,6 +384,7 @@
                     else keyg = okg ? make_key(lam, S, dVg, dObjg, lane) : kKeyNull;
                     if (keyg < key) { key = keyg; vw = xw; dV = dVg; dObj = dObjg; }
                 }
+                if constexpr (kSmall) dObj -= g_old;
                 const uint32_t kmin = wave_umin(key);
                 finish(kReplace, std::false_type{}, kmin, (int)(kmin & 63u), p, k, 0, 0, uw, vw, dV, dObj);
             } else {
@@ -399,7 +403,8 @@
                     const uint32_t wx = L.W[xw & 0xFFFFu];
                     const int dVg = dV_u + wfld(wx, kWIncL);
                     uint32_t keyg;
-                    if (kPriced) keyg = make_key_p(lam, S, dVg, dObjg, dP_u + (wflag(wx, kWPinL) & price_lead(PR[xw & 0xFFFFu])), lane);
+                    if constexpr (kSmall) keyg = key_small(mad24(lam, dVg, mad24s(-S, dObjg, kDBias)), (uint32_t)lane);
+                    else if (kPriced) keyg = make_key_p(lam, S, dVg, dObjg, dP_u + (wflag(wx, kWPinL) & price_lead(PR[xw & 0xFFFFu])), lane);
                     else keyg = make_key(lam, S, dVg, dObjg, lane);
                     if (keyg < key) { key = keyg; vw = xw; k = kk; dV = dVg; dObj = dObjg; }
                 }
@@ -427,7 +432,8 @@
                     const int dvl = wfld(wo, leadl ? kWDecL : kWIncL);
                     sc = min(dv7, 0) + min(dvl, 0);
                 }
-                if (kPriced) {
+                if constexpr (kSmall) key_o = key_small(mad24(lam, sc, mad24s(S, g_o, kDBias)), (uint32_t)lane) | tour_off;
+                else if (kPriced) {
                     int dPs = 0;
                     if (TY == 0) {
                         const uint32_t pro = PR[oldw_o & 0xFFFFu];
@@ -535,7 +541,7 @@
                     const int dk = dinc(L.K[r], T.rack_lo, T.rack_hi);
                     const int v1 = ((uint32_t)r != ro1) ? v_rk[0] + dk + dinc(cnt4<NS>(a1, (uint32_t)r), T.prack_lo, T.prack_hi) : 0;
                     const int v2 = ((uint32_t)r != ro2) ? v_rk[1] + dk + dinc(cnt4<NS>(a2, (uint32_t)r), T.prack_lo, T.prack_hi) : 0;
-                    L.RT[r] = (int)(((uint32_t)v1 & 0xFFFFu) | ((uint32_t)v2 << 16));
+                    L.RT[r] = kSmall ? (int)(((uint32_t)v2 & 0xFFFFu) | ((uint32_t)v1 << 16)) : (int)(((uint32_t)v1 & 0xFFFFu) | ((uint32_t)v2 << 16));
                 }
                 int lane_v = lane;
                 asm volatile("" : "+v"(lane_v));
@@ -561,6 +567,10 @@
                 const int wl1 = lead1 ? T.w00 : T.w01, wf1 = lead1 ? T.w10 : T.w11, wl2 = lead2 ? T.w00 : T.w01, wf2 = lead2 ? T.w10 : T.w11;
                 const int K01 = __mul24(S, gs[0]) + kDBias + __mul24(lam, dvos[0]);
                 const int K02 = __mul24(S, gs[1]) + kDBias + __mul24(lam, dvos[1]);
+                const uint32_t leadp = (lead2 ? 1u : 0u) | (lead1 ? 0x10000u : 0u);
+                const uint32_t K0p = ((uint32_t)K02 & 0xFFFFu) | ((uint32_t)K01 << 16);
+                const int wl1h = (int)((uint32_t)(S * wl1) << 16), wf1h = (int)((uint32_t)(S * wf1) << 16);
+                const int wl2s = (int)((uint32_t)(S * wl2) & 0xFFFFu), wf2s = (int)((uint32_t)(S * wf2) & 0xFFFFu);
                 uint32_t jc = jmp_c;
                 asm volatile("" : "+v"(jc));
                 uint32_t best1 = kKeyNull, best2 = kKeyNull;
@@ -571,6 +581,27 @@
                     const int w = (int)reinterpret_cast<const short *>(L.W)[base + lane];
                     const int rt = L.RT[XR[base + lane]];
                     const int inc = wfld(w, kWIncR);
+                    if constexpr (kSmall) {
+                        uint32_t d = pk_mad_s(pk_add(pk_mad_lo((uint32_t)wfld(w, kWIncL), leadp, (uint32_t)inc), (uint32_t)rt), (uint32_t)lam, K0p);
+                        if (decltype(with_w)::value) {
+                            const uint32_t x = (uint32_t)(base + lane);
+                            const uint32_t xw = x | ((uint32_t)XR[x] << 16);
+                            auto mask_of = [](bool b) { uint32_t m = b ? ~0u : 0u; asm("" : "+v"(m)); return m; };
+                            const bool l1 = c1.w[0] == xw, l2 = c2.w[0] == xw;
+                            bool f1 = false, f2 = false;
+#pragma unroll
+                            for (int i2 = 1; i2 < NS; ++i2) { f1 |= c1.w[i2] == xw; f2 |= c2.w[i2] == xw; }
+                            auto and_or = [](uint32_t m, uint32_t w, uint32_t acc) { uint32_t r; asm("v_and_or_b32 %0, %1, %2, %3" : "=v"(r) : "v"(m), "s"(w), "v"(acc)); return r; };
+                            uint32_t ws = mask_of(l1) & (uint32_t)wl1h;
+                            ws = and_or(mask_of(f1), (uint32_t)wf1h, ws);
+                            ws = and_or(mask_of(l2), (uint32_t)wl2s, ws);
+                            ws = and_or(mask_of(f2), (uint32_t)wf2s, ws);
+                            d = pk_sub(d, ws);
+                        }
+                        key1 = ((d | (uint32_t)w) & 0xFFFF0000u) | (st1 & 0xFF00u) | (uint32_t)rd;
+                        key2 = ((d | (uint32_t)wflag(w, 14)) << 16) | (st2 & 0xFF00u) | (uint32_t)rd;
+                        return;
+                    }
                     int d1 = __mul24(lam, inc + wfldw(w, kWIncL, lw1) + wfldw(rt, 0, 16u)) + K01;
                     int d2 = __mul24(lam, inc + wfldw(w, kWIncL, lw2) + (rt >> 16)) + K02;
                     if (decltype(with_w)::value) {
@@ -617,7 +648,7 @@
                     const uint32_t ws = L.W[xs];
                     const int rts = L.RT[rs];
                     const uint32_t vw = xs | (rs << 16);
-                    const int dV = wfld(ws, kWIncR) + wfldw(ws, kWIncL, lead ? 2u : 0u) + (two ? dvos[1] : dvos[0]) + (two ? (rts >> 16) : wfldw(rts, 0, 16u));
+                    const int dV = wfld(ws, kWIncR) + wfldw(ws, kWIncL, lead ? 2u : 0u) + (two ? dvos[1] : dvos[0]) + ((two != kSmall) ? (rts >> 16) : wfldw(rts, 0, 16u));
                     int mx1 = -1, mx2 = -1;
 #pragma unroll
                     for (int i2 = 0; i2 < NW; ++i2) { mx1 = max(mx1, mr[i2]); mx2 = max(mx2, mr[NW + i2]); }
@@ -838,7 +869,8 @@
                         if (rv != ro)
                             dVx += dv_ro + dinc(cnt4<NS>(a, rv), T.prack_lo, T.prack_hi) + ddec(RFT == 3 ? cnt_b_rv[jj < 3 ? jj : 0] : cnt4<NS>(b, rv), T.prack_lo, T.prack_hi);
                         uint32_t keyx;
-                        if (kPriced) keyx = ok ? make_key_tie_p(lam, S, dVx, dObjx, dPx, tie0 + (uint32_t)jj * 0x55u) : kKeyNull;
+                        if constexpr (kSmall) keyx = ok ? key_small(mad24(lam, dVx, mad24s(-S, dObjx, kDBias)), (tie0 + (uint32_t)jj * 0x55u) & 0xFFu) : kKeyNull;
+                        else if (kPriced) keyx = ok ? make_key_tie_p(lam, S, dVx, dObjx, dPx, tie0 + (uint32_t)jj * 0x55u) : kKeyNull;
                         else keyx = ok ? make_key_tie(lam, S, dVx, dObjx, tie0 + (uint32_t)jj * 0x55u) : kKeyNull;
                         if (keyx < key) { key = keyx; vw = v; q = qq; j = jj; dV = dVx; dObj = dObjx; }
                     }
@@ -897,10 +929,10 @@
 #define KAO_WPE_WIDE 6
 #endif
 template <bool kGlobalA, bool kPriced, int NW, bool kWide> constexpr int search_min_waves() { return kGlobalA ? 1 : (kWide ? KAO_WPE_WIDE : KAO_WPE_SMALL); }
-template <bool kGlobalA, bool kPriced, int NW, bool kWide, int RFT = 0>
+template <bool kGlobalA, bool kPriced, int NW, bool kWide, int RFT = 0, bool kSmall = false>
 __global__ __launch_bounds__(256) __attribute__((amdgpu_waves_per_eu(search_min_waves<kGlobalA, kPriced, NW, kWide>(), 8))) void k_search(SearchPools pl, SearchParams prm) {
     extern __shared__ __attribute__((aligned(16))) unsigned char smem[];
-    search_body<kGlobalA, kPriced, NW, kWide, false, false, RFT>(smem, pl, prm);
+    search_body<kGlobalA, kPriced, NW, kWide, false, false, RFT, kSmall>(smem, pl, prm);
 }
 template <bool kPriced, int NW>
 __global__ __launch_bounds__(256) void k_search_curg(SearchPools pl, SearchParams prm) {
@@ -1085,13 +1117,22 @@
 
 bool search_rf3_eligible(bool global_a, bool cur_global, bool priced, int nw, int team) { return !global_a && !cur_global && !priced && nw == 4 && team == 0; }
 
-void launch_search(const SearchPools &pools, const SearchParams &prm, int n_blocks, int waves, bool global_a, bool priced, int nw, void *stream, int team, int rft) {
+bool search_small_cost(int lam_min, int lam_max, int obj_scale, int w_abs_max, bool priced) {
+    if (priced || lam_min < 0 || lam_max < lam_min || obj_scale < 1 || w_abs_max < 0) return false;
+    return 8 * (int64_t)lam_max + 4 * (int64_t)obj_scale * (int64_t)w_abs_max <= (int64_t)kSmallCostMax;
+}
+
+void launch_search(const SearchPools &pools, const SearchParams &prm, int n_blocks, int waves, bool global_a, bool priced, int nw, void *stream, int team, int rft, bool small) {
     const bool curg = prm.cur_global != 0 && !global_a, wide = prm.wide != 0;
     const size_t lds = search_lds_bytes(prm.maxP, prm.maxBx, waves, global_a, priced, nw, prm.bw != 0, prm.maxR, team, curg);
     hipStream_t st = static_cast<hipStream_t>(stream);
     const dim3 grid(n_blocks), block(64 * (team > 0 && !curg ? team : waves));
     if (rft == 3 && search_rf3_eligible(global_a, curg, priced, nw, team)) {
-        if (wide) launch_lds<k_search<false, false, 4, true, 3>>(grid, block, lds, st, pools, prm);
+        if (small) {
+            if (wide) launch_lds<k_search<false, false, 4, true, 3, true>>(grid, block, lds, st, pools, prm);
+            else launch_lds<k_search<false, false, 4, false, 3, true>>(grid, block, lds, st, pools, prm);
+        }
+        else if (wide) launch_lds<k_search<false, false, 4, true, 3>>(grid, block, lds, st, pools, prm);
         else launch_lds<k_search<false, false, 4, false, 3>>(grid, block, lds, st, pools, prm);
         return;
     }
diff --git a/kafka_assignment_optimizer_amd/csrc/kao_search_dev.h b/kafka_assignment_optimizer_amd/csrc/kao_search_dev.h
--- a/kafka_assignment_optimizer_amd/csrc/kao_search_dev.h
+++ b/kafka_assignment_optimizer_amd/csrc/kao_search_dev.h
@@ -56,6 +56,37 @@
 __device__ __forceinline__ uint32_t make_key(int lam, int S, int dV, int dObj, int lane) { return key_of(__mul24(lam, dV) - __mul24(S, dObj), (uint32_t)lane); }
 __device__ __forceinline__ uint32_t make_key_tie_p(int lam, int S, int dV, int dObj, int dP, uint32_t tie) { return key_of(__mul24(lam, dV) - __mul24(S, dObj) + dP, tie & 0xFFu); }
 __device__ __forceinline__ uint32_t make_key_tie(int lam, int S, int dV, int dObj, uint32_t tie) { return key_of(__mul24(lam, dV) - __mul24(S, dObj), tie & 0xFFu); }
+__device__ __forceinline__ int mad24(int a, int b, int c) {
+    int r;
+    asm("v_mad_i32_i24 %0, %1, %2, %3" : "=v"(r) : "v"(a), "v"(b), "v"(c));
+    return r;
+}
+__device__ __forceinline__ int mad24s(int s, int b, int c) {
+    int r;
+    asm("v_mad_i32_i24 %0, %1, %2, %3" : "=v"(r) : "s"(s), "v"(b), "v"(c));
+    return r;
+}
+__device__ __forceinline__ uint32_t key_small(int biased_cost, uint32_t low) { return ((uint32_t)biased_cost << 8) | low; }
+__device__ __forceinline__ uint32_t pk_mad_lo(uint32_t a, uint32_t b, uint32_t c) {
+    uint32_t r;
+    asm("v_pk_mad_i16 %0, %1, %2, %3 op_sel_hi:[0,1,0]" : "=v"(r) : "v"(a), "v"(b), "v"(c));
+    return r;
+}
+__device__ __forceinline__ uint32_t pk_mad_s(uint32_t a, uint32_t s, uint32_t c) {
+    uint32_t r;
+    asm("v_pk_mad_i16 %0, %1, %2, %3 op_sel_hi:[1,0,1]" : "=v"(r) : "v"(a), "v"(s), "v"(c));
+    return r;
+}
+__device__ __forceinline__ uint32_t pk_add(uint32_t a, uint32_t b) {
+    uint32_t r;
+    asm("v_pk_add_i16 %0, %1, %2" : "=v"(r) : "v"(a), "v"(b));
+    return r;
+}
+__device__ __forceinline__ uint32_t pk_sub(uint32_t a, uint32_t b) {
+    uint32_t r;
+    asm("v_pk_sub_i16 %0, %1, %2" : "=v"(r) : "v"(a), "v"(b));
+    return r;
+}
 __device__ __forceinline__ int price_rep(uint32_t pr) { return (int)(short)(pr & 0xFFFFu); }
 __device__ __forceinline__ int price_lead(uint32_t pr) { return (int)pr >> 16; }
 __device__ __forceinline__ int p_in(int c, int lo, int hi, int price) { return ((c >= hi) | (c < lo)) ? price : 0; }
diff --git a/kafka_assignment_optimizer_amd/csrc/kao_session.cpp b/kafka_assignment_optimizer_amd/csrc/kao_session.cpp
--- a/kafka_assignment_optimizer_amd/csrc/kao_session.cpp
+++ b/kafka_assignment_optimizer_amd/csrc/kao_session.cpp
@@ -159,6 +159,7 @@
 int plan_groups(kao_session &s, int n_cu, SessionPlan &pl) {
     const kao_opts &o = s.opts;
     const bool rft_on = env_int("KAO_SEARCH_RFT", 1) != 0;
+    s.small_on = env_int("KAO_SEARCH_SMALL", 1) != 0;
     std::vector<int> order((size_t)s.n_topics);
     for (int t = 0; t < s.n_topics; ++t) order[(size_t)t] = t;
     auto need1 = [&](int t) {
@@ -190,6 +191,7 @@
         for (int t : mem) {
             const TopicDev &d = s.pts[(size_t)t].d;
             g.rf_uniform = g.rf_uniform < 0 ? d.RF : (g.rf_uniform == d.RF ? d.RF : 0);
+            for (const int w : {d.w00, d.w01, d.w10, d.w11}) g.w_abs_max = std::max(g.w_abs_max, w < 0 ? (w == INT32_MIN ? INT32_MAX : -w) : w);
             g.rf3 = g.rf3 && d.RF == 3 && d.rf_cur <= 3;
             g.maxP = std::max(g.maxP, d.P); g.maxBx = std::max(g.maxBx, d.Bx); g.maxB = std::max(g.maxB, d.B); g.maxR = std::max(g.maxR, d.R); g.wide = g.wide || (int64_t)d.P * d.RF >= 512;
         }
@@ -426,8 +428,11 @@
             HIP_TRY(hipGetLastError());
         }
         const int rft = g.rf3 ? 3 : 0;
-        launch_search(sp, gp, g.smap_n, g.waves, g.global_a, s->priced, g.nw, s->stream, g.team, rft);
-        if (rft && search_rf3_eligible(g.global_a, g.cur_global, s->priced, g.nw, g.team)) s->search_rf3_launches++;
+        const bool rf3_runs = rft && search_rf3_eligible(g.global_a, g.cur_global, s->priced, g.nw, g.team);
+        const bool small = rf3_runs && s->small_on && search_small_cost(gp.lam_min, gp.lam_max, gp.obj_scale, g.w_abs_max, s->priced);
+        launch_search(sp, gp, g.smap_n, g.waves, g.global_a, s->priced, g.nw, s->stream, g.team, rft, small);
+        if (rf3_runs) s->search_rf3_launches++;
+        if (small) s->search_small_launches++;
         HIP_TRY(hipGetLastError());
     }
     if (prof) HIP_TRY(hipEventRecord(e[1], s->stream));
@@ -535,6 +540,12 @@
     return KAO_OK;
 }
 
+int kao_session_small_launches(kao_session *s, int64_t *out) {
+    if (!s || !out) return fail(KAO_ERR_INVALID, "null argument");
+    *out = (int64_t)s->search_small_launches;
+    return KAO_OK;
+}
+
 int kao_session_restart_state(kao_session *s, int32_t topic, int32_t restart, uint16_t *final_state, uint16_t *best_state,
                               int32_t info[4]) {
     if (!s || topic < 0 || topic >= s->n_topics) return fail(KAO_ERR_INVALID, "bad topic");
diff --git a/kafka_assignment_optimizer_amd/solver.py b/kafka_assignment_optimizer_amd/solver.py
--- a/kafka_assignment_optimizer_amd/solver.py
+++ b/kafka_assignment_optimizer_amd/solver.py
@@ -286,6 +286,11 @@
         _check(_ffi.load().kao_session_stats(self._h, C.byref(st)), "kao_session_stats")
         return {k: getattr(st, k) for k, _ in _ffi.KaoStats._fields_}
 
+    def small_launches(self) -> int:
+        n = C.c_int64(0)
+        _check(_ffi.load().kao_session_small_launches(self._h, C.byref(n)), "kao_session_small_launches")
+        return int(n.value)
+
     def restart_state(self, topic: int, restart: int) -> dict:
         t = self.topics[topic]
         n = t.n_partitions * t.rf
```

Result: faster. 849.7 billion, median of 6 (+4.1%).
